# lvxianwei/DeepMerge

Measured on AMD Instinct MI355X. Metric: superpixel-pairs/sec (train step), higher is better.
Workload: dtype bf16; 1 GPU; ShfitScaleFormer_v3 depth [3, 2, 1], scales [32, 64, 128, 256] x 4ch (256x256x4 patches), 32 pairs/GPU/step, fwd+loss+bwd+allreduce+Adam (BASELINE configs[1]); pairs_per_gpu=32, global_batch=32, parallelism=dp1

## Files before the change

deepmerge_amd/_lib.py:

```python
from __future__ import annotations

import ctypes as C
import os
import re
import threading

HERE = os.path.dirname(os.path.abspath(__file__))
ROOT = os.path.dirname(HERE)
LIB_PATH = os.path.join(HERE, "libdeepmerge_hip.so")
HEADER_PATH = os.path.join(ROOT, "include", "deepmerge_hip.h")

DM_F32, DM_BF16 = 0, 1
DM_NT, DM_NN, DM_TN = 0, 1, 2
DM_BF16_PAIR = 2
DM_F64 = 3
DM_EPI_NONE, DM_EPI_GELU, DM_EPI_DGELU, DM_EPI_GELU_GRAD, DM_EPI_MUL = 0, 1, 2, 3, 4

_STATUS = {-1: "bad shape", -2: "bad dtype", -3: "bad alignment", -4: "workspace", -5: "HIP error", -6: "unsupported"}


class DeepMergeLibraryError(RuntimeError):
    pass


class DmGemmArgs(C.Structure):
    _fields_ = [
        ("layout", C.c_int32), ("ab_dtype", C.c_int32), ("c_dtype", C.c_int32), ("aux_dtype", C.c_int32),
        ("M", C.c_int32), ("N", C.c_int32), ("K", C.c_int32),
        ("epilogue", C.c_int32), ("accumulate", C.c_int32), ("split_k", C.c_int32),
        ("A", C.c_void_p), ("lda", C.c_int64),
        ("B", C.c_void_p), ("ldb", C.c_int64),
        ("C", C.c_void_p), ("ldc", C.c_int64),
        ("bias", C.c_void_p),
        ("residual", C.c_void_p), ("ldr", C.c_int64),
        ("aux", C.c_void_p), ("ldaux", C.c_int64),
        ("rows_per_group", C.c_int32), ("group_stride", C.c_int64),
        ("workspace", C.c_void_p), ("workspace_bytes", C.c_int64),
        ("colsum_a", C.c_void_p), ("colsum_accumulate", C.c_int32),
        ("k_fold", C.c_int32), ("a_fold", C.c_int64 * 3), ("b_fold", C.c_int64 * 3),
        ("c_plane", C.c_int64),
    ]


class DmReduceItem(C.Structure):
    _fields_ = [("partial", C.c_void_p), ("out0", C.c_void_p), ("out1", C.c_void_p),
                ("nrows", C.c_int32), ("width", C.c_int32), ("split", C.c_int32), ("accumulate", C.c_int32)]


class DmPairDraw(C.Structure):
    _fields_ = [("pairs", C.c_void_p), ("pair_flag", C.c_void_p), ("poly_off", C.c_void_p), ("poly_pts", C.c_void_p),
                ("pt_tile", C.c_void_p), ("pt_xy", C.c_void_p), ("pt_inner", C.c_void_p), ("pt_obj", C.c_void_p),
                ("pt_region", C.c_void_p),
                ("tile_id", C.c_void_p), ("xy", C.c_void_p), ("inner", C.c_void_p), ("obj", C.c_void_p),
                ("region", C.c_void_p), ("flag", C.c_void_p),
                ("point_id", C.c_void_p),
                ("seed", C.c_uint64),
                ("n_pairs", C.c_int32), ("n_poly", C.c_int32), ("n_poly_pts", C.c_int32), ("n_pts", C.c_int32),
                ("epoch", C.c_int32), ("batch", C.c_int32)]


class DmMergeFold(C.Structure):
    _fields_ = [("ptr", C.c_void_p), ("idx", C.c_void_p), ("edges", C.c_void_p), ("root", C.c_void_p), ("pick", C.c_void_p),
                ("rep", C.c_void_p), ("region_of", C.c_void_p),
                ("simi", C.c_void_p), ("weights", C.c_void_p),
                ("count", C.c_void_p), ("sum", C.c_void_p), ("sumsq", C.c_void_p), ("bbox", C.c_void_p), ("peri", C.c_void_p),
                ("new_id", C.c_void_p), ("hist_rank", C.c_void_p), ("new_ptr", C.c_void_p), ("new_idx", C.c_void_p),
                ("new_rep", C.c_void_p), ("new_region_of", C.c_void_p), ("n_regions", C.c_void_p),
                ("new_count", C.c_void_p), ("new_sum", C.c_void_p), ("new_sumsq", C.c_void_p), ("new_bbox", C.c_void_p),
                ("new_peri", C.c_void_p),
                ("history", C.c_void_p), ("history_simi", C.c_void_p),
                ("C", C.c_int32), ("P", C.c_int32), ("E", C.c_int32), ("S0", C.c_int32), ("bands", C.c_int32), ("round", C.c_int32),
                ("hist_base", C.c_int32), ("hist_cap", C.c_int32)]


class DmVectorTrace(C.Structure):
    _fields_ = [("dart", C.c_void_p), ("next", C.c_void_p), ("lab", C.c_void_p), ("other", C.c_void_p), ("flags", C.c_void_p),
                ("key", C.c_void_p), ("sum", C.c_void_p), ("ring_of_slot", C.c_void_p), ("ring_ptr", C.c_void_p),
                ("arc_base", C.c_void_p), ("xy", C.c_void_p), ("area2", C.c_void_p),
                ("arc_first", C.c_void_p), ("arc_left", C.c_void_p), ("arc_right", C.c_void_p), ("arc_vstart", C.c_void_p),
                ("arc_count", C.c_void_p), ("arc_pos", C.c_void_p), ("arc_ptr", C.c_void_p), ("arc_xy", C.c_void_p),
                ("W", C.c_int32), ("D", C.c_int32), ("R", C.c_int32), ("n_arcs", C.c_int32)]


class DmSceneVectorTrace(C.Structure):
    _fields_ = [("dart", C.c_void_p), ("next", C.c_void_p), ("lab", C.c_void_p), ("other", C.c_void_p), ("flags", C.c_void_p),
                ("key", C.c_void_p), ("sum", C.c_void_p), ("ring_of_slot", C.c_void_p), ("ring_ptr", C.c_void_p),
                ("arc_base", C.c_void_p), ("xy", C.c_void_p), ("area2", C.c_void_p),
                ("arc_first", C.c_void_p), ("arc_left", C.c_void_p), ("arc_right", C.c_void_p), ("arc_vstart", C.c_void_p),
                ("arc_count", C.c_void_p), ("arc_pos", C.c_void_p), ("arc_ptr", C.c_void_p), ("arc_xy", C.c_void_p),
                ("W", C.c_int64), ("D", C.c_int32), ("R", C.c_int32), ("n_arcs", C.c_int32)]


class DmProfRow(C.Structure):
    _fields_ = [("name", C.c_char * 64), ("launches", C.c_int64), ("total_ms", C.c_double),
                ("total_flops", C.c_double), ("total_bytes", C.c_double)]


_P, _I, _L, _F, _D = C.c_void_p, C.c_int32, C.c_int64, C.c_float, C.c_double

SIGNATURES = {
    "dm_abi_version": (_I, []),
    "dm_last_error": (C.c_char_p, []),
    "dm_arch": (C.c_char_p, []),
    "dm_gemm": (_I, [C.POINTER(DmGemmArgs), _P]),
    "dm_gemm_workspace_bytes": (_L, [_I, _I, _I, _I]),
    "dm_gemm_grouped": (_I, [C.POINTER(DmGemmArgs), _I, _P]),
    "dm_attention_fwd": (_I, [_P, _P, _P, _P, _I, _I, _I, _I, _F, _I, _P]),
    "dm_attention_relpos_inkernel": (_I, [_I, _I, _I, _I, _I, _I, _I, _I]),
    "dm_attention_fwd_relpos": (_I, [_P, _P, _I, _I, _I, _P, _P, _I, _I, _I, _I, _F, _I, _P]),
    "dm_attention_split_ok": (_I, [_I, _I, _I, _I, _I, _I, _I, _I]),
    "dm_attention_split_fwd": (_I, [_P, _P, _P, _P, _I, _I, _I, _P, _P, _I, _I, _I, _I, _F, _P]),
    "dm_attention_split_fwd_pair": (_I, [_P, _P, _P, _P, _I, _I, _I, _P, _P, _P, _I, _I, _I, _I, _F, _P]),
    "dm_attention_split_bwd_chunks": (_I, [_I, _I, _I]),
    "dm_attention_split_bwd": (_I, [_P, _P, _P, _I, _I, _I, _P, _P, _P, _P, _P, _P, _P, _P, _I, _I, _I, _I, _F, _P]),
    "dm_attention_split_bwd_pair": (_I, [_P, _P, _P, _I, _I, _I, _P, _P, _P, _P, _P, _P, _P, _P, _I, _I, _I, _I, _F, _P]),
    "dm_attention_bwd_relpos": (_I, [_P, _P, _I, _I, _I, _P, _P, _P, _P, _P, _P, _P, _P, _I, _I, _I, _I, _F, _I, _P]),
    "dm_attention_bwd": (_I, [_P, _P, _P, _P, _P, _P, _P, _P, _P, _I, _I, _I, _I, _F, _I, _P]),
    "dm_attention_bwd_batch_chunks": (_I, [_I, _I, _I, _I]),
    "dm_relpos_bias_gather": (_I, [_P, _P, _P, _P, _I, _I, _I, _P]),
    "dm_relpos_bias_reduce": (_I, [_P, _P, _P, _P, _I, _I, _I, _I, _I, _P]),
    "dm_layernorm_fwd": (_I, [_P, _P, _P, _P, _I, _P, _P, _I, _I, _F, _P]),
    "dm_layernorm_bwd": (_I, [_P, _I, _P, _P, _P, _P, _P, _P, _P, _P, _P, _I, _P, _I, _I, _P]),
    "dm_layernorm_bwd_partials": (_I, [_P, _I, _P, _P, _P, _P, _P, _P, _P, _P, _I, _I, C.POINTER(C.c_int32), _P]),
    "dm_layernorm_bwd_partials_pair": (_I, [_P, _I, _P, _P, _P, _P, _P, _P, _P, _P, _I, _I, C.POINTER(C.c_int32), _P]),
    "dm_partial_reduce_batch": (_I, [C.POINTER(DmReduceItem), _I, _P]),
    "dm_layernorm_bwd_partial_floats": (_L, [_I]),
    "dm_token_pool_fwd": (_I, [_P, _P, _I, _I, _I, _I, _P]),
    "dm_token_pool_bwd": (_I, [_P, _P, _I, _I, _I, _I, _P]),
    "dm_group_mean_fwd": (_I, [_P, _P, _I, _I, _I, _P]),
    "dm_group_mean_bwd": (_I, [_P, _P, _I, _I, _I, _P]),
    "dm_colsum": (_I, [_P, _I, _L, _P, _I, _I, _I, _P, _P]),
    "dm_colsum_partial_floats": (_L, [_I]),
    "dm_cast": (_I, [_P, _P, _I, _L, _P]),
    "dm_split_bf16": (_I, [_P, _L, _L, _L, _P, _I, _I, _P]),
    "dm_split_colsum_partial_floats": (_L, [_L, _L]),
    "dm_split_bf16_colsum": (_I, [_P, _L, _L, _L, _P, _I, _I, _P, _P, _P]),
    "dm_split_bf16_planes": (_I, [_P, _L, _L, _L, _P, _P, _P, _P]),
    "dm_patchify": (_I, [_P, _P, _I, _I, _I, _I, _I, _P]),
    "dm_contrastive_loss": (_I, [_P, _P, _P, _F, _F, _P, _P, _P, _I, _I, _P]),
    "dm_cross_entropy": (_I, [_P, _P, _P, _F, _P, _P, _I, _I, _P]),
    "dm_batchnorm_workspace_bytes": (_L, [_I, _I]),
    "dm_batchnorm_fwd": (_I, [_P, _P, _P, _P, _P, _P, _I, _P, _P, _P, _I, _I, _F, _F, _I, _I, _P, _P]),
    "dm_batchnorm_bwd": (_I, [_P, _P, _P, _P, _P, _I, _P, _P, _P, _P, _P, _I, _I, _I, _I, _I, _P, _P]),
    "dm_adam_step": (_I, [_P, _P, _P, _P, _P, _L, _I, _D, _D, _D, _D, _D, _P]),
    "dm_adam_hyper": (_I, [_I, _D, _D, _D, _P]),
    "dm_adam_step_dev": (_I, [_P, _P, _P, _P, _P, _L, _P, _D, _D, _D, _D, _P]),
    "dm_adam_step_dev_pair": (_I, [_P, _P, _P, _P, _P, _P, _L, _P, _D, _D, _D, _D, _P]),
    "dm_segment_mean": (_I, [_P, _P, _P, _P, _I, _I, _P]),
    "dm_edge_similarity": (_I, [_P, _P, _P, _P, _I, _I, _F, _P]),
    "dm_pairwise_distance": (_I, [_P, _P, _P, _I, _I, _I, _I, _P]),
    "dm_patch_pyramid": (_I, [_P, _I, _I, _I, _P, _P, _I, _I, _I, _I, _P, _P]),
    "dm_patch_pyramid_cols": (_I, [_P, _I, _I, _I, _P, _P, _I, _I, _I, _I, _I, _P, _I, _P]),
    "dm_pair_batch_gather": (_I, [_P, _I, _I, _I, _I, _P, _P, _P, _P, _I, _I, _I, _I, _I, _I, _P, _I, _P, _P, _P, _P]),
    "dm_pair_epoch_draw": (_I, [C.POINTER(DmPairDraw), _P]),
    "dm_contrastive_terms": (_I, [_P, _P, _P, _F, _P, _P, _I, _I, _P]),
    "dm_pair_eval_workspace_bytes": (_L, [_L, _I]),
    "dm_pair_eval_summary": (_I, [_P, _P, _P, _L, _P, _I, _P, _P, _P, _P, _P]),
    "dm_label_stats": (_I, [_P, _P, _I, _I, _I, _I, _P, _P, _P, _P, _P, _P]),
    "dm_label_features": (_I, [_P, _P, _P, _P, _P, _I, _I, _P, _P]),
    "dm_rag_edges": (_I, [_P, _I, _I, _I, _P, _P, _I, _P, _P, _I, _P, _P, _P]),
    "dm_seam_stitch": (_I, [_P, _P, _L, _L, _P, _P, _P, _I, _P, _P, _I, _P, _P, _P]),
    "dm_merge_round": (_I, [_P, _P, _I, _I, _P, _P, _I, _P]),
    "dm_merge_best": (_I, [_P, _P, _I, _I, _F, _P, _P]),
    "dm_merge_match": (_I, [_P, _P, _I, _I, _P, _P, _P, _P, _P]),
    "dm_merge_fold_regions": (_I, [C.POINTER(DmMergeFold), _P]),
    "dm_merge_edge_keys": (_I, [_P, _P, _P, _I, _I, _P, _P]),
    "dm_merge_fold_edges": (_I, [_P, _P, _P, _I, _P, _P, _P, _P]),
    "dm_relabel_raster": (_I, [_P, _P, _P, _L, _I, _P]),
    "dm_region_merge_cost": (_I, [_P, _P, _P, _P, _P, _P, _P, _I, _I, _I, _D, _D, _D, _D, _D, _P, _P]),
    "dm_pixel_regions": (_I, [_P, _I, _I, _I, _P, _P, _P, _P, _P, _P, _P, _P]),
    "dm_label_clearance": (_I, [_P, _I, _I, _I, _P, _P, _P, _P]),
    "dm_point_select_round": (_I, [_P, _P, _I, _I, _I, _I, _I, _P, _P, _P, _P, _P, _P]),
    "dm_point_emit": (_I, [_P, _P, _P, _P, _I, _I, _I, _I, _P, _P, _P, _P, _P, _P, _P]),
    "dm_label_overlap": (_I, [_P, _P, _I, _I, _L, _L, _P, _P, _I, _P, _P, _I, _P, _P, _P]),
    "dm_overlap_reduce": (_I, [_P, _P, _I, _L, _L, _P, _P, _P, _P, _P, _P, _P, _P, _P]),
    "dm_pair_flags": (_I, [_P, _I, _P, _P, _P, _I, _I, _P, _P]),
    "dm_slic_iterate": (_I, [_P, _I, _I, _I, _I, _I, _I, _P, _P, _P, _P]),
    "dm_connected_labels": (_I, [_P, _I, _I, _I, _I, _P, _P, _P, _P, _P]),
    "dm_label_area": (_I, [_P, _I, _I, _I, _P, _P]),
    "dm_slic_absorb_pick": (_I, [_P, _P, _I, _P, _I, _I, _P, _P, _P, _P]),
    "dm_vector_count": (_I, [_P, _I, _I, _P, _P, _P, _P]),
    "dm_vector_emit": (_I, [_P, _P, _I, _I, _P, _P, _P]),
    "dm_vector_link": (_I, [_P, _P, _P, _P, _I, _I, _I, _P, _P, _P, _P, _P, _P]),
    "dm_vector_head_round": (_I, [_P, _P, _P, _P, _I, _P, _P]),
    "dm_vector_rank_init": (_I, [_P, _P, _P, _P, _I, _P, _P, _P, _P, _P, _I, _P]),
    "dm_vector_rank_round": (_I, [_P, _P, _P, _P, _I, _P, _P]),
    "dm_vector_ring_emit": (_I, [C.POINTER(DmVectorTrace), _P]),
    "dm_vector_arc_emit": (_I, [C.POINTER(DmVectorTrace), _P]),
    "dm_scene_vector_count": (_I, [_P, _I, _I, _I, _I, _I, _I, _P, _P, _P, _P, _P]),
    "dm_scene_vector_link": (_I, [_P, _P, _P, _I, _I, _I, _L, _L, _L, _L, _P, _P, _P, _P, _P, _P]),
    "dm_scene_vector_ring_emit": (_I, [C.POINTER(DmSceneVectorTrace), _P]),
    "dm_scene_vector_arc_emit": (_I, [C.POINTER(DmSceneVectorTrace), _P]),
    "dm_rasterize_count": (_I, [_P, _P, _P, _I, _I, _I, _I, _P, _P]),
    "dm_rasterize_emit": (_I, [_P, _P, _P, _P, _P, _I, _I, _L, _I, _I, _L, _P, _P]),
    "dm_rasterize_fill": (_I, [_P, _L, _I, _I, _I, _P, _P, _P]),
    "dm_simplify_nodes": (_I, [_P, _I, _I, _P, _P]),
    "dm_simplify_chains": (_I, [_P, _P, _I, _L, _I, _I, _I, _P, _P, _P]),
    "dm_simplify_arc_count": (_I, [_P, _P, _I, _L, _I, _I, _P, _P, _P]),
    "dm_simplify_arc_emit": (_I, [_P, _P, _P, _I, _L, _L, _I, _I, _P, _P, _P]),
    "dm_simplify_ring_count": (_I, [_P, _P, _P, _I, _I, _I, _I, _P, _P, _P]),
    "dm_simplify_ring_emit": (_I, [_P, _P, _P, _P, _P, _I, _I, _L, _I, _I, _P, _P, _P, _P]),
    "dm_gru_cell_fwd": (_I, [_P, _L, _P, _P, _P, _P, _I, _I, _P]),
    "dm_gru_cell_bwd": (_I, [_P, _P, _P, _P, _P, _P, _I, _I, _P]),
    "dm_prof_enable": (_I, [_I]),
    "dm_prof_collect": (_I, [C.POINTER(DmProfRow), _I]),
}

_lock = threading.Lock()
_lib = None


def declared_symbols(header_path: str = HEADER_PATH):
    text = open(header_path).read()
    text = re.sub(r"/\*.*?\*/", "", text, flags=re.S)
    return sorted(set(re.findall(r"\b(dm_[a-z0-9_]+)\s*\(", text)))


def lib() -> C.CDLL:
    global _lib
    if _lib is not None:
        return _lib
    with _lock:
        if _lib is not None:
            return _lib
        if not os.path.exists(LIB_PATH):
            raise DeepMergeLibraryError(
                f"{LIB_PATH} not found: build the HIP kernels first "
                f"(`python -c 'import __graft_entry__ as g; g.build()'` or `make -C deepmerge_amd/csrc`). "
                f"deepmerge_amd has no CPU fallback.")
        try:
            handle = C.CDLL(LIB_PATH)
        except OSError as e:
            raise DeepMergeLibraryError(f"cannot load {LIB_PATH}: {e}") from e
        for name, (res, args) in SIGNATURES.items():
            try:
                fn = getattr(handle, name)
            except AttributeError as e:
                raise DeepMergeLibraryError(f"{LIB_PATH} does not export {name}") from e
            fn.restype = res
            fn.argtypes = args
        if handle.dm_abi_version() != 7:
            raise DeepMergeLibraryError(f"ABI version mismatch: library {handle.dm_abi_version()} != 7")
        _lib = handle
        return _lib


def check(rc: int, what: str):
    if rc == 0:
        return
    msg = lib().dm_last_error().decode("utf-8", "replace")
    text = f"{what} failed ({_STATUS.get(rc, rc)}): {msg}"
    if rc in (-1, -2, -3, -6):
        raise ValueError(text)
    raise RuntimeError(text)
```

deepmerge_amd/csrc/dm_attention.hip:

```cpp
#include "dm_common.h"
#include "dm_mfma.h"
#include "dm_attention_pipe.h"
#include "dm_attention_x3.h"
#include "dm_prof.h"

namespace {

constexpr int HD = 64;
constexpr int QB = 64;

template <typename T> struct AL {
  static constexpr int RB = HD * (int)sizeof(T);
  static constexpr int CPRW = RB / 16;
  static constexpr int KBD = RB / 64;
  static constexpr int EPC = 16 / (int)sizeof(T);
  static constexpr int TPB = (sizeof(T) == 2) ? 2 : 1;
};

template <typename T> __device__ __forceinline__ int swz(int row);
template <> __device__ __forceinline__ int swz<bf16_t>(int row) {
  const int t0 = (row >> 1) & 1, t1 = (row >> 2) & 1, t2 = (row >> 3) & 1;
  return ((t1 ^ t2) << 2) | (t0 << 1) | t1;
}
template <> __device__ __forceinline__ int swz<float>(int row) { return row & 15; }

template <typename T> __device__ __forceinline__ int img_off(int row, int chunk) {
  return row * AL<T>::RB + ((chunk ^ swz<T>(row)) << 4);
}

template <typename T>
__device__ __forceinline__ void tile_to_lds(char *lds, const T *g, long long ld, int nvalid, int nrows, int t) {
  using L = AL<T>;
  const int c = t % L::CPRW;
  constexpr int RPI = 256 / L::CPRW;
  for (int row = t / L::CPRW; row < nrows; row += RPI) {
    u32x4 v = {0u, 0u, 0u, 0u};
    if (row < nvalid) v = *reinterpret_cast<const u32x4 *>(g + (long long)row * ld + c * L::EPC);
    *reinterpret_cast<u32x4 *>(lds + img_off<T>(row, c)) = v;
  }
}

template <typename T> __device__ __forceinline__ u32x4 frag_row(const char *lds, int row, int kb, int lane) {
  return *reinterpret_cast<const u32x4 *>(lds + img_off<T>(row, kb * 4 + (lane >> 4)));
}
template <typename T> __device__ __forceinline__ u32x4 frag_tr(const char *lds, int d0, int m, int lane);
template <> __device__ __forceinline__ u32x4 frag_tr<bf16_t>(const char *lds, int d0, int m, int lane) {
  const int g = lane >> 4, q = (lane >> 2) & 3, p = lane & 3;
  const int d = d0 + 4 * p;
  u32x4 out;
#pragma unroll
  for (int half = 0; half < 2; ++half) {
    const int k = 32 * m + 4 * g + 16 * half + q;
    const u32x2 w = dm_ds_read_tr16(lds + img_off<bf16_t>(k, d >> 3) + ((d & 7) << 1));
    out[2 * half] = w[0];
    out[2 * half + 1] = w[1];
  }
  return out;
}
template <> __device__ __forceinline__ u32x4 frag_tr<float>(const char *lds, int d0, int m, int lane) {
  const int g = lane >> 4, d = d0 + (lane & 15);
  u32x4 out;
#pragma unroll
  for (int j = 0; j < 4; ++j) {
    const int k = 16 * m + 4 * g + j;
    out[j] = *reinterpret_cast<const unsigned int *>(lds + img_off<float>(k, d >> 2) + ((d & 3) << 2));
  }
  return out;
}
template <typename T> __device__ __forceinline__ u32x4 gl_frag(const T *rowp, bool valid, int kb, int lane) {
  u32x4 v = {0u, 0u, 0u, 0u};
  if (valid) v = *reinterpret_cast<const u32x4 *>(rowp + (kb * 4 + (lane >> 4)) * AL<T>::EPC);
  return v;
}

template <typename T, int NKT> __device__ __forceinline__ u32x4 acc_frag(const f32x4 (&s)[NKT], int m) {
  if constexpr (sizeof(T) == 2) {
    const f32x4 lo = s[2 * m], hi = s[2 * m + 1];
    bf16x8 r = {(bf16_t)lo[0], (bf16_t)lo[1], (bf16_t)lo[2], (bf16_t)lo[3], (bf16_t)hi[0], (bf16_t)hi[1], (bf16_t)hi[2], (bf16_t)hi[3]};
    return __builtin_bit_cast(u32x4, r);
  } else {
    return __builtin_bit_cast(u32x4, s[m]);
  }
}

template <typename T, int NKT>
__device__ __forceinline__ void contract_tokens(f32x4 (&o)[4], const f32x4 (&s)[NKT], const char *img, int lane) {
#pragma unroll
  for (int m = 0; m < NKT / AL<T>::TPB; ++m) {
    const u32x4 fp = acc_frag<T, NKT>(s, m);
#pragma unroll
    for (int dt = 0; dt < 4; ++dt) mma<T>(o[dt], fp, frag_tr<T>(img, dt * 16, m, lane));
    if ((m & 1) == 1) __builtin_amdgcn_sched_barrier(0);
  }
}

__device__ __forceinline__ float row_max(float v) {
  v = fmaxf(v, __shfl_xor(v, 16, 64));
  return fmaxf(v, __shfl_xor(v, 32, 64));
}
__device__ __forceinline__ float row_sum(float v) {
  v += __shfl_xor(v, 16, 64);
  return v + __shfl_xor(v, 32, 64);
}

template <typename T> __device__ __forceinline__ float fast_exp(float x);
template <> __device__ __forceinline__ float fast_exp<float>(float x) { return expf(x); }
template <> __device__ __forceinline__ float fast_exp<bf16_t>(float x) { return __expf(x); }

__device__ __forceinline__ f32x4 load4_guard(const float *p, int i, int n, bool vec) {
  if (vec) return (i < n) ? dm_load4(p + i) : (f32x4){0.f, 0.f, 0.f, 0.f};
  f32x4 r;
#pragma unroll
  for (int e = 0; e < 4; ++e) r[e] = (i + e < n) ? p[i + e] : 0.f;
  return r;
}

struct AttnParams {
  const void *qkv;
  const float *bias;
  const float *bias_t;
  const void *out;
  const void *dout;
  float *lse;
  float *delta;
  void *dqkv;
  float *slab;
  int B, N, H, bchunk;
  float scale;
};

template <bool FAST, bool STRIDED>
__device__ __forceinline__ f32x4 bias_tile(const float *bias_rows, int N, int row, int lane, int kt) {
  const int col = kt * 16 + 4 * (lane >> 4);
  f32x4 bv = {0.f, 0.f, 0.f, 0.f};
  if (bias_rows && row < N) {
    if constexpr (!STRIDED) {
      bv = load4_guard(bias_rows + (long long)row * N, col, N, FAST);
    } else {
#pragma unroll
      for (int r = 0; r < 4; ++r) bv[r] = (col + r < N) ? bias_rows[(long long)(col + r) * N + row] : 0.f;
    }
  }
  return bv;
}
template <typename T>
__device__ __forceinline__ f32x4 score_tile(const u32x4 (&fa)[AL<T>::KBD], const char *img, const f32x4 bv,
                                            int N, int row, float scale, int lane, int kt) {
  using L = AL<T>;
  const int g = lane >> 4, li = lane & 15;
  f32x4 a = {0.f, 0.f, 0.f, 0.f};
#pragma unroll
  for (int kb = 0; kb < L::KBD; ++kb) mma<T>(a, fa[kb], frag_row<T>(img, kt * 16 + li, kb, lane));
  const int col = kt * 16 + 4 * g;
#pragma unroll
  for (int r = 0; r < 4; ++r) a[r] = (row < N && col + r < N) ? a[r] * scale + bv[r] : -INFINITY;
  return a;
}

template <typename T> __device__ __forceinline__ u32x4 pack_tiles(const f32x4 (&tl)[AL<T>::TPB]) {
  if constexpr (sizeof(T) == 2) {
    bf16x8 r = {(bf16_t)tl[0][0], (bf16_t)tl[0][1], (bf16_t)tl[0][2], (bf16_t)tl[0][3],
                (bf16_t)tl[1][0], (bf16_t)tl[1][1], (bf16_t)tl[1][2], (bf16_t)tl[1][3]};
    return __builtin_bit_cast(u32x4, r);
  } else {
    return __builtin_bit_cast(u32x4, tl[0]);
  }
}

template <typename T, int NB>
__device__ __forceinline__ void contract_frags(f32x4 (&o)[4], const u32x4 (&f)[NB], const char *img, int lane) {
#pragma unroll
  for (int m = 0; m < NB; ++m) {
#pragma unroll
    for (int dt = 0; dt < 4; ++dt) mma<T>(o[dt], f[m], frag_tr<T>(img, dt * 16, m, lane));
    if ((m & 1) == 1) __builtin_amdgcn_sched_barrier(0);
  }
}

template <typename T, int NKT, bool FAST>
__global__ __launch_bounds__(256, 2) void attn_fwd_kernel(const AttnParams p) {
  using L = AL<T>;
  constexpr int NK = NKT * 16;
  constexpr int IMG = NK * L::RB;
  __shared__ __attribute__((aligned(16))) char smem[2 * IMG];
  char *kimg = smem, *vimg = smem + IMG;
  const int t = threadIdx.x, lane = t & 63, wave = t >> 6, g = lane >> 4, li = lane & 15;
  const int qblk = blockIdx.x, h = blockIdx.y, b = blockIdx.z;
  const int N = p.N, H = p.H;

  const long long tok_stride = 3LL * H * HD;
  const T *base = reinterpret_cast<const T *>(p.qkv) + (long long)b * N * tok_stride + (long long)h * HD;
  const int q = qblk * QB + wave * 16 + li;

  tile_to_lds<T>(kimg, base + (long long)H * HD, tok_stride, N, NK, t);
  tile_to_lds<T>(vimg, base + 2LL * H * HD, tok_stride, N, NK, t);
  u32x4 fq[L::KBD];
#pragma unroll
  for (int kb = 0; kb < L::KBD; ++kb) fq[kb] = gl_frag<T>(base + (long long)q * tok_stride, q < N, kb, lane);
  __syncthreads();

  f32x4 s[NKT];
  const float *brows = p.bias ? p.bias + (long long)h * N * N : nullptr;
#pragma unroll
  for (int kt = 0; kt < NKT; ++kt) s[kt] = score_tile<T>(fq, kimg, bias_tile<FAST, false>(brows, N, q, lane, kt), N, q, p.scale, lane, kt);

  float m = -INFINITY;
#pragma unroll
  for (int kt = 0; kt < NKT; ++kt)
#pragma unroll
    for (int r = 0; r < 4; ++r) m = fmaxf(m, s[kt][r]);
  m = row_max(m);
  const float msafe = (m == -INFINITY) ? 0.f : m;
  float l = 0.f;
#pragma unroll
  for (int kt = 0; kt < NKT; ++kt)
#pragma unroll
    for (int r = 0; r < 4; ++r) {
      const float e = fast_exp<T>(s[kt][r] - msafe);
      s[kt][r] = e;
      l += e;
    }
  l = row_sum(l);
  const float inv = (l > 0.f) ? 1.f / l : 0.f;
  if (g == 0 && q < N) p.lse[((long long)b * H + h) * N + q] = msafe + logf(l);
#pragma unroll
  for (int kt = 0; kt < NKT; ++kt) s[kt] *= inv;

  f32x4 o[4];
#pragma unroll
  for (int dt = 0; dt < 4; ++dt) o[dt] = (f32x4){0.f, 0.f, 0.f, 0.f};
  contract_tokens<T, NKT>(o, s, vimg, lane);
  if (q < N) {
    T *orow = reinterpret_cast<T *>(const_cast<void *>(p.out)) + ((long long)b * N + q) * H * HD + (long long)h * HD;
#pragma unroll
    for (int dt = 0; dt < 4; ++dt) dm_store4(orow + dt * 16 + 4 * g, o[dt]);
  }
}

template <typename T, int NKT, bool FAST>
__global__ __launch_bounds__(256, 2) void attn_bwd_dq_kernel(const AttnParams p) {
  using L = AL<T>;
  constexpr int NK = NKT * 16;
  constexpr int IMG = NK * L::RB;
  constexpr int NB = NKT / L::TPB;
  __shared__ __attribute__((aligned(16))) char smem[2 * IMG];
  char *kimg = smem, *vimg = smem + IMG;
  const int t = threadIdx.x, lane = t & 63, wave = t >> 6, g = lane >> 4, li = lane & 15;
  const int qblk = blockIdx.x, h = blockIdx.y, chunk = blockIdx.z;
  const int N = p.N, H = p.H;
  const long long tok_stride = 3LL * H * HD;
  const int q = qblk * QB + wave * 16 + li;
  const bool qok = q < N;
  const float *brows = p.bias ? p.bias + (long long)h * N * N : nullptr;
  const bool want_bins = p.slab != nullptr;
  f32x4 hacc[NKT];
#pragma unroll
  for (int kt = 0; kt < NKT; ++kt) hacc[kt] = (f32x4){0.f, 0.f, 0.f, 0.f};

  const int b_end = min(p.B, (chunk + 1) * p.bchunk);
  for (int b = chunk * p.bchunk; b < b_end; ++b) {
    const T *base = reinterpret_cast<const T *>(p.qkv) + (long long)b * N * tok_stride + (long long)h * HD;
    const long long orow = ((long long)b * N + q) * H * HD + (long long)h * HD;
    const T *Og = reinterpret_cast<const T *>(p.out) + orow;
    const T *dOg = reinterpret_cast<const T *>(p.dout) + orow;
    __syncthreads();
    tile_to_lds<T>(kimg, base + (long long)H * HD, tok_stride, N, NK, t);
    tile_to_lds<T>(vimg, base + 2LL * H * HD, tok_stride, N, NK, t);
    u32x4 fq[L::KBD], fdo[L::KBD];
#pragma unroll
    for (int kb = 0; kb < L::KBD; ++kb) {
      fq[kb] = gl_frag<T>(base + (long long)q * tok_stride, qok, kb, lane);
      fdo[kb] = gl_frag<T>(dOg, qok, kb, lane);
    }
    float dl = 0.f;
    if (qok) {
#pragma unroll
      for (int c = 0; c < 4; ++c) {
        const f32x4 a = dm_load4(Og + 16 * g + 4 * c), d = dm_load4(dOg + 16 * g + 4 * c);
        dl += (a[0] * d[0] + a[1] * d[1]) + (a[2] * d[2] + a[3] * d[3]);
      }
    }
    dl = row_sum(dl);
    const long long rowid = ((long long)b * H + h) * N + q;
    if (g == 0 && qok) p.delta[rowid] = dl;
    const float lse = qok ? p.lse[rowid] : 0.f;
    __syncthreads();

    u32x4 fds[NB];
    f32x4 bnext[L::TPB];
#pragma unroll
    for (int u = 0; u < L::TPB; ++u) bnext[u] = bias_tile<FAST, false>(brows, N, q, lane, u);
#pragma unroll
    for (int m = 0; m < NB; ++m) {
      f32x4 bcur[L::TPB];
#pragma unroll
      for (int u = 0; u < L::TPB; ++u) bcur[u] = bnext[u];
      if (m + 1 < NB) {
#pragma unroll
        for (int u = 0; u < L::TPB; ++u) bnext[u] = bias_tile<FAST, false>(brows, N, q, lane, (m + 1) * L::TPB + u);
      }
      f32x4 tl[L::TPB];
#pragma unroll
      for (int u = 0; u < L::TPB; ++u) {
        const int kt = m * L::TPB + u;
        const f32x4 sc = score_tile<T>(fq, kimg, bcur[u], N, q, p.scale, lane, kt);
        f32x4 a = {0.f, 0.f, 0.f, 0.f};
#pragma unroll
        for (int kb = 0; kb < L::KBD; ++kb) mma<T>(a, fdo[kb], frag_row<T>(vimg, kt * 16 + li, kb, lane));
        f32x4 dsv;
#pragma unroll
        for (int r = 0; r < 4; ++r) dsv[r] = fast_exp<T>(sc[r] - lse) * (a[r] - dl);
        if (want_bins) hacc[kt] += dsv;
        tl[u] = dsv;
      }
      fds[m] = pack_tiles<T>(tl);
      asm volatile("" : "+v"(fds[m]));
      __builtin_amdgcn_sched_barrier(0);
    }

    f32x4 o[4];
#pragma unroll
    for (int dt = 0; dt < 4; ++dt) o[dt] = (f32x4){0.f, 0.f, 0.f, 0.f};
    contract_frags<T, NB>(o, fds, kimg, lane);
    if (qok) {
      T *dq = reinterpret_cast<T *>(p.dqkv) + ((long long)b * N + q) * tok_stride + (long long)h * HD;
#pragma unroll
      for (int dt = 0; dt < 4; ++dt) dm_store4(dq + dt * 16 + 4 * g, o[dt] * p.scale);
    }
  }

  if (want_bins && qok) {
    float *srow = p.slab + (((long long)chunk * H + h) * N + q) * N;
#pragma unroll
    for (int kt = 0; kt < NKT; ++kt) {
      const int key = kt * 16 + 4 * g;
      if constexpr (FAST) {
        if (key < N) dm_store4(srow + key, hacc[kt]);
      } else {
#pragma unroll
        for (int r = 0; r < 4; ++r)
          if (key + r < N) srow[key + r] = hacc[kt][r];
      }
    }
  }
}

template <typename T, int NKT, bool FAST>
__global__ __launch_bounds__(256, 2) void attn_bwd_dkv_kernel(const AttnParams p) {
  using L = AL<T>;
  constexpr int NK = NKT * 16;
  constexpr int IMG = NK * L::RB;
  __shared__ __attribute__((aligned(16))) char smem[2 * IMG];
  char *qimg = smem, *doimg = smem + IMG;
  const int t = threadIdx.x, lane = t & 63, wave = t >> 6, g = lane >> 4, li = lane & 15;
  const int kblk = blockIdx.x, h = blockIdx.y, b = blockIdx.z;
  const int N = p.N, H = p.H;

  const long long tok_stride = 3LL * H * HD;
  const T *base = reinterpret_cast<const T *>(p.qkv) + (long long)b * N * tok_stride + (long long)h * HD;
  const long long o_stride = (long long)H * HD;
  const T *dOg = reinterpret_cast<const T *>(p.dout) + (long long)b * N * o_stride + (long long)h * HD;
  const int key = kblk * QB + wave * 16 + li;
  const bool kok = key < N;
  const T *krow = base + (long long)key * tok_stride + (long long)H * HD;
  const T *vrow = krow + (long long)H * HD;
  const float *lse = p.lse + ((long long)b * H + h) * N;
  const float *delta = p.delta + ((long long)b * H + h) * N;

  tile_to_lds<T>(qimg, base, tok_stride, N, NK, t);
  tile_to_lds<T>(doimg, dOg, o_stride, N, NK, t);
  u32x4 fk[L::KBD], fvv[L::KBD];
#pragma unroll
  for (int kb = 0; kb < L::KBD; ++kb) {
    fk[kb] = gl_frag<T>(krow, kok, kb, lane);
    fvv[kb] = gl_frag<T>(vrow, kok, kb, lane);
  }
  __syncthreads();

  constexpr int NB = NKT / L::TPB;
  u32x4 fpt[NB], fds[NB];
  const float *bsrc = FAST ? p.bias_t : p.bias;
  const float *brows = bsrc ? bsrc + (long long)h * N * N : nullptr;
  f32x4 bnext[L::TPB], lnext[L::TPB], dnext[L::TPB];
  auto fetch = [&](int m) {
#pragma unroll
    for (int u = 0; u < L::TPB; ++u) {
      const int qt = m * L::TPB + u;
      bnext[u] = bias_tile<FAST, !FAST>(brows, N, key, lane, qt);
      lnext[u] = load4_guard(lse, qt * 16 + 4 * g, N, FAST);
      dnext[u] = load4_guard(delta, qt * 16 + 4 * g, N, FAST);
    }
  };
  fetch(0);
#pragma unroll
  for (int m = 0; m < NB; ++m) {
    f32x4 bcur[L::TPB], lcur[L::TPB], dcur[L::TPB];
#pragma unroll
    for (int u = 0; u < L::TPB; ++u) { bcur[u] = bnext[u]; lcur[u] = lnext[u]; dcur[u] = dnext[u]; }
    if (m + 1 < NB) fetch(m + 1);
    f32x4 tp[L::TPB], td[L::TPB];
#pragma unroll
    for (int u = 0; u < L::TPB; ++u) {
      const int qt = m * L::TPB + u;
      const int q0 = qt * 16 + 4 * g;
      const f32x4 sc = score_tile<T>(fk, qimg, bcur[u], N, key, p.scale, lane, qt);
      f32x4 a = {0.f, 0.f, 0.f, 0.f};
#pragma unroll
      for (int kb = 0; kb < L::KBD; ++kb) mma<T>(a, fvv[kb], frag_row<T>(doimg, qt * 16 + li, kb, lane));
#pragma unroll
      for (int r = 0; r < 4; ++r) {
        const float pv = (q0 + r < N) ? fast_exp<T>(sc[r] - lcur[u][r]) : 0.f;
        tp[u][r] = pv;
        td[u][r] = pv * (a[r] - dcur[u][r]);
      }
    }
    fpt[m] = pack_tiles<T>(tp);
    fds[m] = pack_tiles<T>(td);
    asm volatile("" : "+v"(fpt[m]), "+v"(fds[m]));
    __builtin_amdgcn_sched_barrier(0);
  }
  f32x4 o[4];
  T *dk = reinterpret_cast<T *>(p.dqkv) + ((long long)b * N + key) * tok_stride + (long long)H * HD + (long long)h * HD;
  T *dvp = dk + (long long)H * HD;
#pragma unroll
  for (int dt = 0; dt < 4; ++dt) o[dt] = (f32x4){0.f, 0.f, 0.f, 0.f};
  contract_frags<T, NB>(o, fpt, doimg, lane);
  if (kok) {
#pragma unroll
    for (int dt = 0; dt < 4; ++dt) dm_store4(dvp + dt * 16 + 4 * g, o[dt]);
  }
#pragma unroll
  for (int dt = 0; dt < 4; ++dt) o[dt] = (f32x4){0.f, 0.f, 0.f, 0.f};
  contract_frags<T, NB>(o, fds, qimg, lane);
  if (kok) {
#pragma unroll
    for (int dt = 0; dt < 4; ++dt) dm_store4(dk + dt * 16 + 4 * g, o[dt] * p.scale);
  }
}

template <typename T, int NKT, bool FAST> void launch3(int which, const AttnParams &p, dim3 grid, hipStream_t s) {
  if (which == 0) hipLaunchKernelGGL((attn_fwd_kernel<T, NKT, FAST>), grid, dim3(256), 0, s, p);
  else if (which == 1) hipLaunchKernelGGL((attn_bwd_dq_kernel<T, NKT, FAST>), grid, dim3(256), 0, s, p);
  else hipLaunchKernelGGL((attn_bwd_dkv_kernel<T, NKT, FAST>), grid, dim3(256), 0, s, p);
}
template <typename T, bool FAST> void dispatch_nkt(int which, const AttnParams &p, hipStream_t s) {
  const dim3 grid((p.N + QB - 1) / QB, p.H, which == 1 ? (p.B + p.bchunk - 1) / p.bchunk : p.B);
  const int nkt = (p.N + 15) / 16;
  if (nkt <= 2) launch3<T, 2, FAST>(which, p, grid, s);
  else if (nkt <= 4) launch3<T, 4, FAST>(which, p, grid, s);
  else if (nkt <= 8) launch3<T, 8, FAST>(which, p, grid, s);
  else if (nkt <= 12) launch3<T, 12, FAST>(which, p, grid, s);
  else if (nkt <= 14) launch3<T, 14, FAST>(which, p, grid, s);
  else launch3<T, 16, FAST>(which, p, grid, s);
}
template <typename T> int dispatch(int which, const AttnParams &p, hipStream_t s) {
  const bool fast = (p.N % 4 == 0) && (which != 2 || p.bias == nullptr || p.bias_t != nullptr);
  if (fast) dispatch_nkt<T, true>(which, p, s);
  else dispatch_nkt<T, false>(which, p, s);
  return 0;
}

int check_common(const char *who, int B, int N, int H, int D, int dtype) {
  DM_REQUIRE(B > 0 && H > 0 && N > 0 && N <= 256, DM_ERR_BAD_SHAPE, "%s: need 0 < N <= 4096 tokens and head dim <= 256 (got N=%d, D=%d, B=%d, H=%d)", who, N, D, B, H);
  DM_REQUIRE(D == HD, DM_ERR_BAD_SHAPE, "%s: head dim must be in 1..256 (got %d)", who, D);
  DM_REQUIRE(dtype == DM_F32 || dtype == DM_BF16, DM_ERR_BAD_DTYPE, "%s: bad dtype %d", who, dtype);
  DM_REQUIRE(H <= 65535 && B <= 65535, DM_ERR_BAD_SHAPE, "%s: grid too large", who);
  return DM_OK;
}

}

static int batch_chunk(int B, int N, int H) {
  const int per_sample = ((N + QB - 1) / QB) * H;
  for (int c = 8; c > 1; c >>= 1)
    if ((long long)per_sample * ((B + c - 1) / c) >= 300) return c;
  return 1;
}

const AttnSwitches &attn_switches() {
  static const AttnSwitches sw = [] {
    AttnSwitches v;
    if (const char *e = getenv("DM_ATTN_PIPE")) v.pipe = atoi(e);
    if (const char *e = getenv("DM_ATTN_Q32")) v.q32 = atoi(e);
    if (const char *e = getenv("DM_ATTN_Q32_BWD")) v.q32_bwd = atoi(e);
    if (const char *e = getenv("DM_ATTN_Q32_TABKV")) v.q32_tabkv = atoi(e) != 0;
    if (const char *e = getenv("DM_ATTN_Q32_W8")) v.q32_w8 = atoi(e) != 0;
    if (const char *e = getenv("DM_ATTN_Q32_TABW")) v.q32_tabw = atoi(e);
    if (const char *e = getenv("DM_ATTN_PF")) v.pf = atoi(e) != 0;
    if (const char *e = getenv("DM_ATTN_XCD")) v.xcd = atoi(e) != 0;
    if (const char *e = getenv("DM_ATTN_X3")) v.x3 = atoi(e) != 0;
    if (const char *e = getenv("DM_ATTN_X3_W8")) v.x3_w8 = atoi(e) != 0;
    return v;
  }();
  return sw;
}

namespace {

bool tokens32(const AttnCall &c) { return c.N > 128 && c.N <= 256; }
bool cube_fits(const AttnCall &c) { return c.N == 64 * c.cube_s && (c.cube_s == 3 || c.cube_s == 4); }
bool persistent_gate(const AttnCall &c, int mode) {
  return mode != 0 && (long long)c.N * 3 * c.H * 64 * 2 < (1LL << 31) && (mode == 2 || c.B * c.H >= 96);
}

AttnPass pass32(const AttnCall &c, AttnFamily f, AttnBias bias, int waves, int rows) {
  AttnPass g{f, (c.N + 31) / 32, c.N % 32 != 0, bias, waves, 0, 0, 0};
  attn_chunks(c.B, c.N, c.H, rows, g.nblk, g.chunks, g.bchunk);
  return g;
}
bool ragged16(const AttnCall &c) { return !(c.N == 128 || c.N == 192 || c.N == 256); }
AttnPass pass_pipe16(const AttnCall &c, AttnBias bias) {
  const int nkt = (c.N + 15) / 16;
  AttnPass g{ATTN_PIPE16, ragged16(c) ? (nkt + 1) / 2 * 2 : nkt, ragged16(c), bias, 8, 0, 0, 0};
  attn_chunks(c.B, c.N, c.H, 128, g.nblk, g.chunks, g.bchunk);
  return g;
}
AttnPass pass_reg16(const AttnCall &c, int bchunk) {
  return AttnPass{ATTN_REG16, (c.N + 15) / 16, c.N % 16 != 0, c.dense ? ATTN_BIAS_DENSE : ATTN_BIAS_NONE, 4, (c.N + QB - 1) / QB, (c.B + bchunk - 1) / bchunk, bchunk};
}
int waves32(const AttnCall &c, const AttnSwitches &sw) { return (c.N + 31) / 32 <= 7 && sw.q32_w8 ? 8 : 4; }

bool split_shape(const AttnCall &c, const AttnSwitches &sw) {
  return sw.x3 && c.D == HD && tokens32(c) && c.B > 0 && c.H > 0 && persistent_gate(c, 2) && (!c.table || cube_fits(c));
}

}

AttnFwdPlan attn_plan_fwd(const AttnCall &c, const AttnSwitches &sw) {
  AttnFwdPlan pl{};
  pl.pf = sw.pf;
  pl.xcd = sw.xcd;
  if (c.split) {
    if (!split_shape(c, sw)) pl.refused = ATTN_SHAPE_NOT_TAKEN;
    else pl.pass = pass32(c, ATTN_X3, c.table ? ATTN_BIAS_TABLE : ATTN_BIAS_NONE, sw.x3_w8 ? 8 : 4, 128);
    return pl;
  }
  pl.pass = pass_reg16(c, 1);
  if (c.D != HD || c.N > 256) {
    pl.pass.family = ATTN_GENERIC;
  } else if (c.dtype == DM_BF16) {
    if (tokens32(c) && persistent_gate(c, sw.q32) && !(c.table && (c.dense || !cube_fits(c)))) {
      if (c.table) pl.pass = pass32(c, ATTN_Q32, ATTN_BIAS_TABLE, sw.q32_tabw == 4 ? 4 : 8, sw.q32_tabw == 4 ? 128 : 256);
      else if (c.dense) pl.pass = pass32(c, ATTN_Q32, ATTN_BIAS_DENSE, 4, 128);
      else pl.pass = pass32(c, ATTN_Q32, ATTN_BIAS_NONE, waves32(c, sw), 32 * waves32(c, sw));
    } else if (c.N >= 128 && persistent_gate(c, sw.pipe)) {
      pl.pass = pass_pipe16(c, c.dense ? ATTN_BIAS_DENSE : ATTN_BIAS_NONE);
    }
  }
  if (c.table && !c.dense && !(pl.pass.family == ATTN_Q32 && pl.pass.bias == ATTN_BIAS_TABLE)) pl.refused = ATTN_SHAPE_NOT_TAKEN;
  return pl;
}

AttnBwdPlan attn_plan_bwd(const AttnCall &c, const AttnSwitches &sw) {
  AttnBwdPlan pl{};
  pl.xcd = sw.xcd;
  if (c.split) {
    if (c.B > 0 && c.H > 0) {
      const AttnBias bias = c.table ? ATTN_BIAS_TABLE : ATTN_BIAS_NONE;
      pl.dq = pass32(c, ATTN_X3, bias, sw.x3_w8 ? 8 : 4, 128);
      pl.dkv = pass32(c, ATTN_X3, bias, 4, 128);
      pl.slab_chunks = pl.dkv.chunks;
    }
    if (!split_shape(c, sw)) pl.refused = ATTN_SHAPE_NOT_TAKEN;
    return pl;
  }
  pl.dq = pass_reg16(c, batch_chunk(c.B, c.N, c.H));
  pl.dkv = pass_reg16(c, 1);
  pl.slab_chunks = pl.dq.chunks;
  if (c.D != HD || c.N > 256) {
    pl.dq.family = pl.dkv.family = ATTN_GENERIC;
    return pl;
  }
  const bool table_only = c.table && !c.dense;
  if (c.dtype != DM_BF16) {
    if (table_only) pl.refused = ATTN_TABLE_NEEDS_BF16;
    return pl;
  }
  if (c.N >= 128 && persistent_gate(c, sw.pipe) && !(ragged16(c) && (c.dense || c.slab))) {
    pl.dq = pass_pipe16(c, c.dense ? ATTN_BIAS_DENSE : ATTN_BIAS_NONE);
    pl.dkv = pass_pipe16(c, c.dense || c.slab ? ATTN_BIAS_DENSE : ATTN_BIAS_NONE);
    if (tokens32(c) && persistent_gate(c, sw.q32_bwd) && !(c.table && !cube_fits(c))) {
      if (c.table) pl.dq = pass32(c, ATTN_Q32, ATTN_BIAS_TABLE, 8, 256);
      else if (c.dense) pl.dq = pass32(c, ATTN_Q32, ATTN_BIAS_DENSE, 4, 128);
      else pl.dq = pass32(c, ATTN_Q32, ATTN_BIAS_NONE, waves32(c, sw), 32 * waves32(c, sw));
      const int w = (c.N + 31) / 32 <= 7 ? 8 : 4;
      if (sw.q32_bwd != 3 && c.table && sw.q32_tabkv) pl.dkv = pass32(c, ATTN_Q32_TABKV, ATTN_BIAS_TABLE, 4, 128);
      else if (sw.q32_bwd != 3 && !c.dense && !c.slab) pl.dkv = pass32(c, ATTN_Q32, ATTN_BIAS_NONE, w, 32 * w);
    }
    pl.slab_chunks = pl.dkv.chunks;
  }
  if (table_only && pl.dkv.family != ATTN_Q32_TABKV) pl.refused = ATTN_TABLE_NOT_TAKEN;
  return pl;
}

extern "C" int32_t dm_attention_bwd_batch_chunks(int32_t B, int32_t N, int32_t H, int32_t dtype) {
  return attn_plan_bwd(AttnCall{B, N, H, HD, dtype == DM_BF16 ? DM_BF16 : DM_F32, true, false, 0, true, false}, attn_switches()).slab_chunks;
}

bool dm_attn_generic_shape(int N, int D);
int dm_attn_generic_fwd(const void *qkv, const float *bias, void *out, float *lse, int B, int N, int H, int D, float scale, int dtype, hipStream_t s);
int dm_attn_generic_bwd(const void *qkv, const float *bias, const void *out, const void *dout, const float *lse, void *dqkv, float *delta,
                        int B, int N, int H, int D, float scale, int dtype, hipStream_t s);

extern "C" int dm_attention_fwd(const void *qkv, const float *bias, void *out, float *lse, int32_t B, int32_t N, int32_t H,
                                int32_t D, float scale, int32_t dtype, void *stream) {
  if (dm_attn_generic_shape(N, D)) {
    DM_REQUIRE(B > 0 && H > 0 && H <= 65535 && B <= 65535 && (dtype == DM_F32 || dtype == DM_BF16) && qkv && out && lse, DM_ERR_BAD_SHAPE,
               "dm_attention_fwd: bad arguments (B=%d H=%d dtype=%d)", B, H, dtype);
    const int rc = dm_attn_generic_fwd(qkv, bias, out, lse, B, N, H, D, scale, dtype, reinterpret_cast<hipStream_t>(stream));
    DM_REQUIRE(rc == DM_OK, rc, "dm_attention_fwd: generic kernel could not be configured");
    DM_LAUNCH_CHECK("dm_attention_fwd(generic)");
    return DM_OK;
  }
  if (int rc = check_common("dm_attention_fwd", B, N, H, D, dtype)) return rc;
  DM_REQUIRE(qkv && out && lse, DM_ERR_BAD_SHAPE, "dm_attention_fwd: null pointer");
  DM_REQUIRE(dm_aligned16(qkv) && dm_aligned16(out) && dm_aligned16(bias), DM_ERR_BAD_ALIGN, "dm_attention_fwd: qkv/out/bias must be 16-byte aligned");
  const AttnFwdPlan pl = attn_plan_fwd(AttnCall{B, N, H, D, dtype, bias != nullptr, false, 0, false, false}, attn_switches());
  hipStream_t s = reinterpret_cast<hipStream_t>(stream);
  {
    const double esz = (dtype == DM_BF16) ? 2.0 : 4.0;
    DmProfScope prof(dtype == DM_BF16 ? "attn_fwd_bf16" : "attn_fwd_f32", s, 4.0 * B * H * (double)N * N * HD,
                     esz * 4.0 * B * H * (double)N * HD);
    const AttnPipeParams pp{qkv, bias, out, lse, B, N, H, scale};
    if (pl.pass.family == ATTN_Q32) {
      DM_REQUIRE(dm_attn_fwd_q32(pl, pp, s), DM_ERR_HIP, "dm_attention_fwd: kernel could not be configured");
    } else if (pl.pass.family == ATTN_PIPE16) {
      dm_attn_fwd_pipe(pl, pp, s);
    } else {
      AttnParams p{};
      p.qkv = qkv; p.bias = bias; p.out = out; p.lse = lse; p.B = B; p.N = N; p.H = H; p.scale = scale; p.bchunk = 1;
      if (dtype == DM_BF16) dispatch<bf16_t>(0, p, s); else dispatch<float>(0, p, s);
    }
  }
  DM_LAUNCH_CHECK("dm_attention_fwd");
  return DM_OK;
}

static AttnCall table_call(int32_t B, int32_t N, int32_t H, int32_t D, int32_t cube_s, int32_t cube_h, int32_t cube_w, int32_t dtype, bool split) {
  return AttnCall{B, N, H, D, dtype, false, true, cube_h == 8 && cube_w == 8 ? cube_s : 0, false, split};
}

extern "C" int32_t dm_attention_relpos_inkernel(int32_t B, int32_t N, int32_t H, int32_t D, int32_t cube_s, int32_t cube_h, int32_t cube_w,
                                                int32_t dtype) {
  if (B <= 0 || H <= 0) return 0;
  const AttnCall c = table_call(B, N, H, D, cube_s, cube_h, cube_w, dtype, false);
  return !attn_plan_fwd(c, attn_switches()).refused && !attn_plan_bwd(c, attn_switches()).refused ? 1 : 0;
}

extern "C" int dm_attention_fwd_relpos(const void *qkv, const float *table, int32_t cube_s, int32_t cube_h, int32_t cube_w, void *out,
                                       float *lse, int32_t B, int32_t N, int32_t H, int32_t D, float scale, int32_t dtype, void *stream) {
  DM_REQUIRE(dm_attention_relpos_inkernel(B, N, H, D, cube_s, cube_h, cube_w, dtype), DM_ERR_UNSUPPORTED,
             "dm_attention_fwd_relpos: shape not taken (B=%d N=%d H=%d D=%d cube=%dx%dx%d dtype=%d); gather the bias and call dm_attention_fwd",
             B, N, H, D, cube_s, cube_h, cube_w, dtype);
  DM_REQUIRE(qkv && table && out && lse, DM_ERR_BAD_SHAPE, "dm_attention_fwd_relpos: null pointer");
  DM_REQUIRE(dm_aligned16(qkv) && dm_aligned16(out), DM_ERR_BAD_ALIGN, "dm_attention_fwd_relpos: qkv/out must be 16-byte aligned");
  const AttnFwdPlan pl = attn_plan_fwd(table_call(B, N, H, D, cube_s, cube_h, cube_w, dtype, false), attn_switches());
  hipStream_t s = reinterpret_cast<hipStream_t>(stream);
  {
    DmProfScope prof("attn_fwd_bf16", s, 4.0 * B * H * (double)N * N * HD, 2.0 * 4.0 * B * H * (double)N * HD);
    AttnPipeParams pp{qkv, nullptr, out, lse, B, N, H, scale};
    pp.table = table;
    pp.cube_s = cube_s;
    DM_REQUIRE(dm_attn_fwd_q32(pl, pp, s), DM_ERR_UNSUPPORTED, "dm_attention_fwd_relpos: kernel could not be configured");
  }
  DM_LAUNCH_CHECK("dm_attention_fwd_relpos");
  return DM_OK;
}

static int attention_bwd(const void *qkv, const float *bias, const float *bias_t, const float *table, int32_t cube_s, const void *out,
                         const void *dout, const float *lse, void *dqkv, float *delta, float *dbias_slab, int32_t B, int32_t N, int32_t H,
                         int32_t D, float scale, int32_t dtype, void *stream) {
  if (dm_attn_generic_shape(N, D)) {
    DM_REQUIRE(B > 0 && H > 0 && H <= 65535 && B <= 65535 && (dtype == DM_F32 || dtype == DM_BF16) && qkv && out && dout && lse && dqkv && delta,
               DM_ERR_BAD_SHAPE, "dm_attention_bwd: bad arguments (B=%d H=%d dtype=%d)", B, H, dtype);
    DM_REQUIRE(dbias_slab == nullptr, DM_ERR_UNSUPPORTED, "dm_attention_bwd: the bias-table gradient needs head dim 64 and N <= 256 (got D=%d N=%d)", D, N);
    const int rc = dm_attn_generic_bwd(qkv, bias, out, dout, lse, dqkv, delta, B, N, H, D, scale, dtype, reinterpret_cast<hipStream_t>(stream));
    DM_REQUIRE(rc == DM_OK, rc, "dm_attention_bwd: generic kernel could not be configured");
    DM_LAUNCH_CHECK("dm_attention_bwd(generic)");
    return DM_OK;
  }
  if (int rc = check_common("dm_attention_bwd", B, N, H, D, dtype)) return rc;
  DM_REQUIRE(qkv && out && dout && lse && dqkv && delta, DM_ERR_BAD_SHAPE, "dm_attention_bwd: null pointer");
  DM_REQUIRE(dm_aligned16(qkv) && dm_aligned16(out) && dm_aligned16(dout) && dm_aligned16(dqkv) && dm_aligned16(bias) &&
             dm_aligned16(bias_t) && dm_aligned16(lse) && dm_aligned16(delta) && dm_aligned16(dbias_slab), DM_ERR_BAD_ALIGN,
             "dm_attention_bwd: tensors must be 16-byte aligned");
  const AttnBwdPlan pl = attn_plan_bwd(AttnCall{B, N, H, D, dtype, bias != nullptr, table != nullptr, cube_s, dbias_slab != nullptr, false}, attn_switches());
  DM_REQUIRE(pl.refused != ATTN_TABLE_NEEDS_BF16, DM_ERR_UNSUPPORTED, "dm_attention_bwd_relpos: the table-reading kernels are bf16 only");
  DM_REQUIRE(!pl.refused, DM_ERR_UNSUPPORTED,
             "dm_attention_bwd_relpos: the table-reading backward kernels do not take this call (B=%d N=%d H=%d, switches "
             "DM_ATTN_PIPE / DM_ATTN_Q32_BWD / DM_ATTN_Q32_TABKV) and no dense bias rows were given", B, N, H);
  hipStream_t s = reinterpret_cast<hipStream_t>(stream);
  {
    const double esz = (dtype == DM_BF16) ? 2.0 : 4.0;
    DmProfScope prof(dtype == DM_BF16 ? "attn_bwd_bf16" : "attn_bwd_f32", s, 10.0 * B * H * (double)N * N * HD,
                     esz * 8.0 * B * H * (double)N * HD);
    if (pl.dkv.family == ATTN_REG16) {
      AttnParams p{};
      p.qkv = qkv; p.bias = bias; p.bias_t = bias ? bias_t : nullptr; p.out = out; p.dout = dout; p.lse = const_cast<float *>(lse);
      p.delta = delta; p.dqkv = dqkv; p.slab = dbias_slab;
      p.B = B; p.N = N; p.H = H; p.scale = scale; p.bchunk = pl.dq.bchunk;
      if (dtype == DM_BF16) { dispatch<bf16_t>(1, p, s); dispatch<bf16_t>(2, p, s); }
      else { dispatch<float>(1, p, s); dispatch<float>(2, p, s); }
    } else {
      AttnPipeBwdParams pp{qkv, bias, out, dout, lse, delta, dqkv, dbias_slab, B, N, H, scale};
      pp.table = table;
      pp.cube_s = cube_s;
      DM_REQUIRE(pl.dq.family != ATTN_Q32 || dm_attn_bwd_dq_q32(pl, pp, s), DM_ERR_HIP, "dm_attention_bwd: the dQ kernel could not be configured");
      if (pl.dkv.family == ATTN_PIPE16) dm_attn_bwd_pipe(pl, pp, s);
      else DM_REQUIRE(dm_attn_bwd_dkv_q32(pl, pp, s), DM_ERR_HIP, "dm_attention_bwd: the dK / dV kernel could not be configured");
    }
  }
  DM_LAUNCH_CHECK("dm_attention_bwd");
  return DM_OK;
}

extern "C" int dm_attention_bwd(const void *qkv, const float *bias, const float *bias_t, const void *out, const void *dout,
                                const float *lse, void *dqkv, float *delta, float *dbias_slab, int32_t B, int32_t N, int32_t H, int32_t D, float scale, int32_t dtype,
                                void *stream) {
  return attention_bwd(qkv, bias, bias_t, nullptr, 0, out, dout, lse, dqkv, delta, dbias_slab, B, N, H, D, scale, dtype, stream);
}

extern "C" int dm_attention_bwd_relpos(const void *qkv, const float *table, int32_t cube_s, int32_t cube_h, int32_t cube_w, const float *bias,
                                       const float *bias_t, const void *out, const void *dout, const float *lse, void *dqkv, float *delta,
                                       float *dbias_slab, int32_t B, int32_t N, int32_t H, int32_t D, float scale, int32_t dtype, void *stream) {
  DM_REQUIRE(table, DM_ERR_BAD_SHAPE, "dm_attention_bwd_relpos: null table");
  DM_REQUIRE(bias || dm_attention_relpos_inkernel(B, N, H, D, cube_s, cube_h, cube_w, dtype), DM_ERR_UNSUPPORTED,
             "dm_attention_bwd_relpos: shape not taken (B=%d N=%d H=%d D=%d cube=%dx%dx%d dtype=%d); call dm_attention_bwd", B, N, H, D, cube_s,
             cube_h, cube_w, dtype);
  return attention_bwd(qkv, bias, bias_t, table, cube_s, out, dout, lse, dqkv, delta, dbias_slab, B, N, H, D, scale, dtype, stream);
}

static AttnCall split_call(int32_t B, int32_t N, int32_t H, int32_t D, bool has_table, int32_t cube_s, int32_t cube_h, int32_t cube_w, bool slab) {
  AttnCall c = table_call(B, N, H, D, cube_s, cube_h, cube_w, DM_F32, true);
  c.table = has_table;
  c.slab = slab;
  return c;
}

extern "C" int32_t dm_attention_split_ok(int32_t B, int32_t N, int32_t H, int32_t D, int32_t has_table, int32_t cube_s, int32_t cube_h,
                                         int32_t cube_w) {
  return attn_plan_fwd(split_call(B, N, H, D, has_table != 0, cube_s, cube_h, cube_w, false), attn_switches()).refused ? 0 : 1;
}

static int split_fwd_impl(const float *qkv, void *qkv_hi, void *qkv_lo, const float *table, int32_t cube_s, int32_t cube_h, int32_t cube_w, float *out,
                          void *out_pair, float *lse, int32_t B, int32_t N, int32_t H, int32_t D, float scale, void *stream);
extern "C" int dm_attention_split_fwd(const float *qkv, void *qkv_hi, void *qkv_lo, const float *table, int32_t cube_s, int32_t cube_h,
                                      int32_t cube_w, float *out, float *lse, int32_t B, int32_t N, int32_t H, int32_t D, float scale,
                                      void *stream) {
  return split_fwd_impl(qkv, qkv_hi, qkv_lo, table, cube_s, cube_h, cube_w, out, nullptr, lse, B, N, H, D, scale, stream);
}
extern "C" int dm_attention_split_fwd_pair(const float *qkv, void *qkv_hi, void *qkv_lo, const float *table, int32_t cube_s, int32_t cube_h,
                                           int32_t cube_w, float *out, void *out_pair, float *lse, int32_t B, int32_t N, int32_t H, int32_t D,
                                           float scale, void *stream) {
  DM_REQUIRE(out_pair && dm_aligned16(out_pair), DM_ERR_BAD_SHAPE, "dm_attention_split_fwd_pair: out_pair must be a 16-byte aligned pointer");
  return split_fwd_impl(qkv, qkv_hi, qkv_lo, table, cube_s, cube_h, cube_w, out, out_pair, lse, B, N, H, D, scale, stream);
}
static int split_fwd_impl(const float *qkv, void *qkv_hi, void *qkv_lo, const float *table, int32_t cube_s, int32_t cube_h, int32_t cube_w, float *out,
                          void *out_pair, float *lse, int32_t B, int32_t N, int32_t H, int32_t D, float scale, void *stream) {
  const AttnFwdPlan pl = attn_plan_fwd(split_call(B, N, H, D, table != nullptr, cube_s, cube_h, cube_w, false), attn_switches());
  DM_REQUIRE(!pl.refused, DM_ERR_UNSUPPORTED,
             "dm_attention_split_fwd: shape not taken (B=%d N=%d H=%d D=%d cube=%dx%dx%d); use dm_attention_fwd", B, N, H, D, cube_s, cube_h, cube_w);
  DM_REQUIRE(qkv_hi && qkv_lo && out && lse, DM_ERR_BAD_SHAPE, "dm_attention_split_fwd: null pointer");
  DM_REQUIRE(dm_aligned16(qkv) && dm_aligned16(qkv_hi) && dm_aligned16(qkv_lo) && dm_aligned16(out), DM_ERR_BAD_ALIGN,
             "dm_attention_split_fwd: tensors must be 16-byte aligned");
  hipStream_t s = reinterpret_cast<hipStream_t>(stream);
  {
    DmProfScope prof("attn_fwd_x3", s, 3.0 * 4.0 * B * H * (double)N * N * HD, 4.0 * 4.0 * B * H * (double)N * HD);
    if (qkv) dm_attn_x3_split(qkv, qkv_hi, qkv_lo, (long long)B * N * 3 * H * HD, s);
    AttnX3Params p{reinterpret_cast<const bf16_t *>(qkv_hi), reinterpret_cast<const bf16_t *>(qkv_lo), table, cube_s, out, lse, B, N, H, scale,
                   reinterpret_cast<bf16_t *>(out_pair)};
    DM_REQUIRE(dm_attn_fwd_x3(pl, p, s), DM_ERR_UNSUPPORTED, "dm_attention_split_fwd: kernel could not be configured");
  }
  DM_LAUNCH_CHECK("dm_attention_split_fwd");
  return DM_OK;
}

extern "C" int32_t dm_attention_split_bwd_chunks(int32_t B, int32_t N, int32_t H) {
  return attn_plan_bwd(split_call(B, N, H, HD, false, 0, 0, 0, false), attn_switches()).slab_chunks;
}

static int split_bwd_impl(const void *qkv_hi, const void *qkv_lo, const float *table, int32_t cube_s, int32_t cube_h, int32_t cube_w,
                          const float *out, const float *dout, void *dout_hi, void *dout_lo, const float *lse, float *dqkv, void *dqkv_pair,
                          float *delta, float *dbias_slab, int32_t B, int32_t N, int32_t H, int32_t D, float scale, void *stream);
extern "C" int dm_attention_split_bwd(const void *qkv_hi, const void *qkv_lo, const float *table, int32_t cube_s, int32_t cube_h, int32_t cube_w,
                                      const float *out, const float *dout, void *dout_hi, void *dout_lo, const float *lse, float *dqkv,
                                      float *delta, float *dbias_slab, int32_t B, int32_t N, int32_t H, int32_t D, float scale, void *stream) {
  DM_REQUIRE(dqkv, DM_ERR_BAD_SHAPE, "dm_attention_split_bwd: null pointer");
  return split_bwd_impl(qkv_hi, qkv_lo, table, cube_s, cube_h, cube_w, out, dout, dout_hi, dout_lo, lse, dqkv, nullptr, delta, dbias_slab, B, N, H, D, scale, stream);
}
extern "C" int dm_attention_split_bwd_pair(const void *qkv_hi, const void *qkv_lo, const float *table, int32_t cube_s, int32_t cube_h, int32_t cube_w,
                                           const float *out, const float *dout, void *dout_hi, void *dout_lo, const float *lse, void *dqkv_pair,
                                           float *delta, float *dbias_slab, int32_t B, int32_t N, int32_t H, int32_t D, float scale, void *stream) {
  DM_REQUIRE(dqkv_pair, DM_ERR_BAD_SHAPE, "dm_attention_split_bwd_pair: null pointer");
  return split_bwd_impl(qkv_hi, qkv_lo, table, cube_s, cube_h, cube_w, out, dout, dout_hi, dout_lo, lse, nullptr, dqkv_pair, delta, dbias_slab, B, N, H, D, scale, stream);
// ... 25 lines not shown
```

deepmerge_amd/csrc/dm_attention_plan.h:

```cpp
#pragma once

struct AttnSwitches {
  int pipe = 1;
  int q32 = 1;
  int q32_bwd = 1;
  bool q32_tabkv = true;
  bool q32_w8 = true;
  int q32_tabw = 8;
  bool pf = true;
  bool xcd = true;
  bool x3 = true;
  bool x3_w8 = true;
};
const AttnSwitches &attn_switches();

struct AttnCall {
  int B, N, H, D, dtype;
  bool dense;
  bool table;
  int cube_s;
  bool slab;
  bool split;
};

enum AttnFamily {
  ATTN_GENERIC,
  ATTN_REG16,
  ATTN_PIPE16,
  ATTN_Q32,
  ATTN_Q32_TABKV,
  ATTN_X3,
};
enum AttnBias { ATTN_BIAS_NONE, ATTN_BIAS_DENSE, ATTN_BIAS_TABLE };
enum AttnRefusal { ATTN_TAKEN = 0, ATTN_SHAPE_NOT_TAKEN, ATTN_TABLE_NEEDS_BF16, ATTN_TABLE_NOT_TAKEN };

struct AttnPass {
  AttnFamily family;
  int nkt;
  bool ragged;
  AttnBias bias;
  int waves;
  int nblk, chunks, bchunk;
};
struct AttnFwdPlan {
  AttnRefusal refused;
  AttnPass pass;
  bool pf, xcd;
};
struct AttnBwdPlan {
  AttnRefusal refused;
  AttnPass dq, dkv;
  bool xcd;
  int slab_chunks;
};
AttnFwdPlan attn_plan_fwd(const AttnCall &c, const AttnSwitches &sw);
AttnBwdPlan attn_plan_bwd(const AttnCall &c, const AttnSwitches &sw);

inline void attn_chunks(int B, int N, int H, int rows, int &nblk, int &chunks, int &bchunk) {
  nblk = (N + rows - 1) / rows;
  chunks = 256 / (H * nblk);
  if (chunks < 1) chunks = 1;
  if (chunks > B) chunks = B;
  bchunk = (B + chunks - 1) / chunks;
  chunks = (B + bchunk - 1) / bchunk;
}
```

deepmerge_amd/ops.py:

```python
from __future__ import annotations

import os

import ctypes as C
from typing import Optional

import torch

from . import _lib
from ._lib import DM_BF16, DM_EPI_DGELU, DM_EPI_GELU, DM_EPI_GELU_GRAD, DM_EPI_MUL, DM_EPI_NONE, DM_F32, DM_NN, DM_NT, DM_TN, DmGemmArgs, check

_NUMERICS = "bf16"


NUMERICS_MODES = ("bf16", "fp32", "bf16x3")
_FP32_PRODUCTS = "mfma_f32"
_SPLIT_MIN_WORK = 1 << 24
_PAIR_LN_MAX_COLS = 1024


def set_numerics(mode: str) -> None:
    global _NUMERICS
    _NUMERICS = check_numerics(mode)

# ... 284 lines not shown
            b_rows, b_cols = (N, K) if layout == DM_NT else (K, N)
            if (A.rows, A.cols) != (a_rows, a_cols) or (B.rows, B.cols) != (b_rows, b_cols):
                raise ValueError(f"plane pair shapes {(A.rows, A.cols)} / {(B.rows, B.cols)} do not match the product {(a_rows, a_cols)} / {(b_rows, b_cols)}")
            fold = (K, A.t.stride(0), B.t.stride(0))
            A, B, lda, ldb, K = A.t, B.t, a_cols, b_cols, 3 * K
        _need_cuda(A, B, C_out, kw.get("colsum_out"))
        if A.dtype != B.dtype:
            raise ValueError(f"A/B dtype mismatch: {A.dtype} vs {B.dtype}")
        lda = lda if lda is not None else (A.stride(-2) if A.dim() >= 2 else K)
        ldb = ldb if ldb is not None else (B.stride(-2) if B.dim() >= 2 else K)
        arr[i] = _gemm_args(layout, A, B, C_out, M, N, K, lda, ldb, kw.get("ldc"), kw.get("bias"), kw.get("residual"), kw.get("ldr"),
                            kw.get("epilogue", DM_EPI_NONE), kw.get("aux"), kw.get("ldaux"), kw.get("accumulate", False), kw.get("split_k", 0),
                            kw.get("rows_per_group", 0), kw.get("group_stride", 0), kw.get("colsum_out"), kw.get("colsum_accumulate", False),
                            f"{kw.get('ws_slot', 'gemm')}.g{i}", None, fold, min_slabs=16 if layout == DM_TN else 0)
    check(_lib.lib().dm_gemm_grouped(arr, len(calls), _stream()), "dm_gemm_grouped")


def cast(src: torch.Tensor, dtype: torch.dtype) -> torch.Tensor:
    if src.dtype == dtype:
        return src
    _need_cuda(src)
    if src.dtype != torch.float32:
        raise ValueError("dm_cast source must be fp32")
    src = src.contiguous()
    dst = torch.empty(src.shape, dtype=dtype, device=src.device)
    check(_lib.lib().dm_cast(src.data_ptr(), dst.data_ptr(), _dt(dst), src.numel(), _stream()), "dm_cast")
    return dst


def colsum(X: torch.Tensor, out: torch.Tensor, accumulate: bool = False, ws_slot: str = "partial") -> torch.Tensor:
    _need_cuda(X, out)
    M, N = X.shape
    part = workspace(_lib.lib().dm_colsum_partial_floats(N) * 4, X.device, ws_slot)
    check(_lib.lib().dm_colsum(X.data_ptr(), _dt(X), X.stride(0), out.data_ptr(), M, N, int(accumulate), part.data_ptr(), _stream()), "dm_colsum")
    return out


def layernorm_fwd(x: torch.Tensor, gamma, beta, eps: float, out_dtype: torch.dtype, pair: bool = False):
    _need_cuda(x, gamma, beta)
    rows, cols = x.numel() // x.shape[-1], x.shape[-1]
    mean = torch.empty(rows, dtype=torch.float32, device=x.device)
    rstd = torch.empty(rows, dtype=torch.float32, device=x.device)
    if pair:
        yp = torch.empty((2, rows, cols), dtype=torch.bfloat16, device=x.device)
        check(_lib.lib().dm_layernorm_fwd(x.data_ptr(), gamma.data_ptr(), beta.data_ptr(), yp.data_ptr(), _lib.DM_BF16_PAIR, mean.data_ptr(),
                                          rstd.data_ptr(), rows, cols, eps, _stream()), "dm_layernorm_fwd")
        return Planes(yp), mean, rstd
    y = torch.empty(x.shape, dtype=out_dtype, device=x.device)
    check(_lib.lib().dm_layernorm_fwd(x.data_ptr(), gamma.data_ptr(), beta.data_ptr(), y.data_ptr(), _dt(y), mean.data_ptr(),
                                      rstd.data_ptr(), rows, cols, eps, _stream()), "dm_layernorm_fwd")
    return y, mean, rstd


_pending_reduce = []
_pending_out = set()
_flush_queued = False
_flush_task = -1


def _in_backward() -> bool:
    return torch._C._current_graph_task_id() != -1


def flush_reductions() -> None:
    global _flush_queued
    _flush_queued = False
    if not _pending_reduce:
        return
    items = (_lib.DmReduceItem * len(_pending_reduce))()
    for i, (f, _keep) in enumerate(_pending_reduce):
        items[i].partial, items[i].out0, items[i].out1, items[i].nrows, items[i].width, items[i].split, items[i].accumulate = f
    n = len(_pending_reduce)
    keep = list(_pending_reduce)
    _pending_reduce.clear()
    _pending_out.clear()
    check(_lib.lib().dm_partial_reduce_batch(items, n, _stream()), "dm_partial_reduce_batch")
    del keep


def _queue_reduce(part, out0, out1, nrows, width, split, accumulate) -> None:
    global _flush_queued, _flush_task
    task = torch._C._current_graph_task_id()
    if task != _flush_task:
        _pending_reduce.clear()
        _pending_out.clear()
        _flush_queued = False
        _flush_task = task
    keys = (out0.data_ptr(), out1.data_ptr())
    if keys[0] in _pending_out or keys[1] in _pending_out:
        flush_reductions()
    _pending_reduce.append(((part.data_ptr(), keys[0], keys[1], int(nrows), int(width), int(split), int(bool(accumulate))), (part, out0, out1)))
    _pending_out.update(keys)
    if not _flush_queued:
        torch.autograd.Variable._execution_engine.queue_callback(flush_reductions)
        _flush_queued = True


def layernorm_bwd(dy, x, gamma, mean, rstd, dres=None, dgamma=None, dbeta=None, accumulate=False, want_lp=False, defer=False, want_pair=False):
    _need_cuda(dy, x)
    if not (dy.is_contiguous() and x.is_contiguous()) or dy.numel() != x.numel():
        raise ValueError("layernorm_bwd: dy and x must be contiguous and of the same size (an expanded gradient has no rows to read)")
    rows, cols = x.numel() // x.shape[-1], x.shape[-1]
    dx = torch.empty(x.shape, dtype=torch.float32, device=x.device)
    dx_lp = torch.empty(x.shape, dtype=torch.bfloat16, device=x.device) if want_lp else None
    if dgamma is None:
        dgamma = torch.empty(cols, dtype=torch.float32, device=x.device)
        dbeta = torch.empty(cols, dtype=torch.float32, device=x.device)
        accumulate = False
        defer = False
    if want_pair:
        pair = torch.empty((2, rows, cols), dtype=torch.bfloat16, device=x.device)
        deferred = defer and _DEFER_REDUCTIONS and _in_backward()
        part = (torch.empty(_lib.lib().dm_layernorm_bwd_partial_floats(cols), dtype=torch.float32, device=x.device) if deferred
                else workspace(_lib.lib().dm_layernorm_bwd_partial_floats(cols) * 4, x.device, "partial").view(torch.float32))
        n_part = C.c_int32(0)
        check(_lib.lib().dm_layernorm_bwd_partials_pair(dy.data_ptr(), _dt(dy), x.data_ptr(), gamma.data_ptr(), mean.data_ptr(), rstd.data_ptr(),
                                                        _ptr(dres), dx.data_ptr(), pair.data_ptr(), part.data_ptr(), rows, cols, C.byref(n_part),
                                                        _stream()), "dm_layernorm_bwd_partials_pair")
        if deferred:
            _queue_reduce(part, dgamma, dbeta, n_part.value, 2 * cols, cols, accumulate)
        else:
            item = (_lib.DmReduceItem * 1)()
            item[0].partial, item[0].out0, item[0].out1 = part.data_ptr(), dgamma.data_ptr(), dbeta.data_ptr()
            item[0].nrows, item[0].width, item[0].split, item[0].accumulate = n_part.value, 2 * cols, cols, int(bool(accumulate))
            check(_lib.lib().dm_partial_reduce_batch(item, 1, _stream()), "dm_partial_reduce_batch")
        return dx, Planes(pair), dgamma, dbeta
    if defer and _DEFER_REDUCTIONS and _in_backward():
        part = torch.empty(_lib.lib().dm_layernorm_bwd_partial_floats(cols), dtype=torch.float32, device=x.device)
        n_part = C.c_int32(0)
        check(_lib.lib().dm_layernorm_bwd_partials(dy.data_ptr(), _dt(dy), x.data_ptr(), gamma.data_ptr(), mean.data_ptr(), rstd.data_ptr(),
                                                   _ptr(dres), dx.data_ptr(), _ptr(dx_lp), part.data_ptr(), rows, cols, C.byref(n_part),
                                                   _stream()), "dm_layernorm_bwd_partials")
        _queue_reduce(part, dgamma, dbeta, n_part.value, 2 * cols, cols, accumulate)
        return (dx, dx_lp, dgamma, dbeta) if want_lp else (dx, dgamma, dbeta)
    part = workspace(_lib.lib().dm_layernorm_bwd_partial_floats(cols) * 4, x.device, "partial")
    check(_lib.lib().dm_layernorm_bwd(dy.data_ptr(), _dt(dy), x.data_ptr(), gamma.data_ptr(), mean.data_ptr(), rstd.data_ptr(),
                                      _ptr(dres), dx.data_ptr(), _ptr(dx_lp), dgamma.data_ptr(), dbeta.data_ptr(), int(accumulate),
                                      part.data_ptr(), rows, cols, _stream()), "dm_layernorm_bwd")
    return (dx, dx_lp, dgamma, dbeta) if want_lp else (dx, dgamma, dbeta)


_DEFER_REDUCTIONS = os.environ.get("DM_DEFER_REDUCTIONS", "1") != "0"


def relpos_bias_gather(table: torch.Tensor, index32: torch.Tensor, N: int, transposed: bool = False):
    _need_cuda(table, index32)
    n_bins, H = table.shape
    bias = torch.empty((H, N, N), dtype=torch.float32, device=table.device)
    bias_t = torch.empty_like(bias) if transposed else None
    check(_lib.lib().dm_relpos_bias_gather(table.data_ptr(), index32.data_ptr(), bias.data_ptr(), _ptr(bias_t), N, H, n_bins, _stream()),
          "dm_relpos_bias_gather")
    return (bias, bias_t) if transposed else bias


def attention_fwd(qkv: torch.Tensor, bias: Optional[torch.Tensor], B: int, N: int, H: int, D: int, scale: float):
    _need_cuda(qkv, bias)
    out = torch.empty((B, N, H * D), dtype=qkv.dtype, device=qkv.device)
    lse = torch.empty((B, H, N), dtype=torch.float32, device=qkv.device)
    check(_lib.lib().dm_attention_fwd(qkv.data_ptr(), _ptr(bias), out.data_ptr(), lse.data_ptr(), B, N, H, D, scale, _dt(qkv), _stream()),
          "dm_attention_fwd")
    return out, lse


def _split_attention(table, index32, qkv, B, N, H, D):
    if (qkv if isinstance(qkv, torch.dtype) else qkv.dtype) != torch.float32 or _FP32_PRODUCTS != "bf16x3" or not _SPLIT_ATTENTION:
        return False, None
    cube = None if table is None else getattr(index32, "_dm_cube", None)
    if table is not None and cube is None:
        return False, None
    return attention_split_ok(B, N, H, D, cube), cube


_SPLIT_ATTENTION = os.environ.get("DM_ATTN_X3", "1") != "0"


def _inkernel_cube(table, index32, B, N, H, D, dtype):
    cube = None if table is None else getattr(index32, "_dm_cube", None)
    if cube is None or _INKERNEL_TABLE is False or not relpos_inkernel(B, N, H, D, cube, dtype):
        return None
    return cube


_INKERNEL_TABLE = os.environ.get("DM_ATTN_TABLE_IN_KERNEL", "1") != "0"


def relpos_inkernel(B: int, N: int, H: int, D: int, cube, dtype: torch.dtype) -> bool:
    if cube is None or len(cube) != 3:
        return False
    return bool(_lib.lib().dm_attention_relpos_inkernel(B, N, H, D, int(cube[0]), int(cube[1]), int(cube[2]),
                                                        DM_BF16 if dtype == torch.bfloat16 else DM_F32))


def attention_fwd_relpos(qkv: torch.Tensor, table: torch.Tensor, cube, B: int, N: int, H: int, D: int, scale: float):
    _need_cuda(qkv, table)
    if table.dtype != torch.float32 or not table.is_contiguous() or tuple(table.shape) != ((2 * cube[0] - 1) * (2 * cube[1] - 1) * (2 * cube[2] - 1), H):
        raise ValueError(f"attention_fwd_relpos: table must be contiguous fp32 [(2s-1)(2h-1)(2w-1), H], got {tuple(table.shape)} {table.dtype}")
    out = torch.empty((B, N, H * D), dtype=qkv.dtype, device=qkv.device)
    lse = torch.empty((B, H, N), dtype=torch.float32, device=qkv.device)
    check(_lib.lib().dm_attention_fwd_relpos(qkv.data_ptr(), table.data_ptr(), int(cube[0]), int(cube[1]), int(cube[2]), out.data_ptr(),
                                             lse.data_ptr(), B, N, H, D, scale, _dt(qkv), _stream()), "dm_attention_fwd_relpos")
    return out, lse


def attention_split_ok(B: int, N: int, H: int, D: int, cube=None) -> bool:
    c = (0, 0, 0) if cube is None else tuple(int(v) for v in cube)
    return bool(_lib.lib().dm_attention_split_ok(B, N, H, D, int(cube is not None), c[0], c[1], c[2]))


def attention_fwd_split(qkv: torch.Tensor, table: Optional[torch.Tensor], cube, B: int, N: int, H: int, D: int, scale: float, out_pair: bool = False):
    if table is not None and (table.dtype != torch.float32 or not table.is_contiguous()):
        raise ValueError("attention_fwd_split: table must be contiguous fp32")
    if isinstance(qkv, Planes):
        _need_cuda(qkv.t, table)
        hi, lo, src, dev = qkv.t[0], qkv.t[1], None, qkv.t.device
    else:
        _need_cuda(qkv, table)
        if qkv.dtype != torch.float32 or not qkv.is_contiguous():
            raise ValueError("attention_fwd_split: qkv must be a contiguous fp32 tensor")
        hi = torch.empty(qkv.shape, dtype=torch.bfloat16, device=qkv.device)
        lo = torch.empty(qkv.shape, dtype=torch.bfloat16, device=qkv.device)
        src, dev = qkv.data_ptr(), qkv.device
    out = torch.empty((B, N, H * D), dtype=torch.float32, device=dev)
    lse = torch.empty((B, H, N), dtype=torch.float32, device=dev)
    c = (0, 0, 0) if cube is None else tuple(int(v) for v in cube)
    if out_pair:
        op = torch.empty((2, B * N, H * D), dtype=torch.bfloat16, device=dev)
        check(_lib.lib().dm_attention_split_fwd_pair(src, hi.data_ptr(), lo.data_ptr(), _ptr(table), c[0], c[1], c[2], out.data_ptr(), op.data_ptr(),
                                                     lse.data_ptr(), B, N, H, D, scale, _stream()), "dm_attention_split_fwd_pair")
        return out, lse, hi, lo, Planes(op)
    check(_lib.lib().dm_attention_split_fwd(src, hi.data_ptr(), lo.data_ptr(), _ptr(table), c[0], c[1], c[2], out.data_ptr(),
                                            lse.data_ptr(), B, N, H, D, scale, _stream()), "dm_attention_split_fwd")
    return out, lse, hi, lo


def attention_bwd_split(hi, lo, table, cube, out, dout, lse, B, N, H, D, scale, index32=None, n_bins=0, pair=False):
    _need_cuda(hi, lo, table, out, dout, lse, index32)
    if out.dtype != torch.float32 or dout.dtype != torch.float32 or not (out.is_contiguous() and dout.is_contiguous()):
        raise ValueError("attention_bwd_split: out / dout must be contiguous fp32")
    dqkv = (torch.empty((2, B * N, 3 * H * D), dtype=torch.bfloat16, device=hi.device) if pair
            else torch.empty(hi.shape, dtype=torch.float32, device=hi.device))
    delta = torch.empty((B, H, N), dtype=torch.float32, device=hi.device)
    dhi = torch.empty(dout.shape, dtype=torch.bfloat16, device=hi.device)
    dlo = torch.empty(dout.shape, dtype=torch.bfloat16, device=hi.device)
    slab, info = None, None
    if index32 is not None and table is not None:
        chunks = _lib.lib().dm_attention_split_bwd_chunks(B, N, H)
        slab = torch.empty((chunks, H, N, N), dtype=torch.float32, device=hi.device)
        info = (chunks, N, relpos_index_csr(index32, n_bins))
    c = (0, 0, 0) if cube is None else tuple(int(v) for v in cube)
    fn = _lib.lib().dm_attention_split_bwd_pair if pair else _lib.lib().dm_attention_split_bwd
    check(fn(hi.data_ptr(), lo.data_ptr(), _ptr(table), c[0], c[1], c[2], out.data_ptr(), dout.data_ptr(),
             dhi.data_ptr(), dlo.data_ptr(), lse.data_ptr(), dqkv.data_ptr(), delta.data_ptr(), _ptr(slab),
             B, N, H, D, scale, _stream()), "dm_attention_split_bwd")
    return (Planes(dqkv) if pair else dqkv), slab, info


def relpos_index_csr(index32: torch.Tensor, n_bins: int):
    key = (index32._version, n_bins)
    hit = getattr(index32, "_dm_csr", None)
    if hit is None or hit[0] != key:
        flat = index32.reshape(-1).to(torch.int64)
        ok = (flat >= 0) & (flat < n_bins)
        where = torch.nonzero(ok).reshape(-1)
        order = torch.argsort(flat[where], stable=True)
        positions = where[order].to(torch.int32).contiguous()
        counts = torch.bincount(flat[where], minlength=n_bins)
        offsets = torch.zeros(n_bins + 1, dtype=torch.int64, device=index32.device)
        offsets[1:] = torch.cumsum(counts, 0)
        hit = index32._dm_csr = (key, positions, offsets.to(torch.int32).contiguous())
    return hit[1], hit[2]


def attention_bwd(qkv, bias, out, dout, lse, B, N, H, D, scale, index32=None, n_bins=0, bias_t=None, table=None, cube=None):
    _need_cuda(qkv, bias, out, dout, lse, index32, bias_t, table)
    dqkv = torch.empty_like(qkv)
    delta = torch.empty((B, H, N), dtype=torch.float32, device=qkv.device)
    slab, info = None, None
    if index32 is not None:
        if D != 64 or N > 256:
            raise ValueError(f"the relative-position bias gradient needs head dim 64 and N <= 256 (got D={D}, N={N})")
        chunks = _lib.lib().dm_attention_bwd_batch_chunks(B, N, H, _dt(qkv))
        slab = torch.empty((chunks, H, N, N), dtype=torch.float32, device=qkv.device)
        info = (chunks, N, relpos_index_csr(index32, n_bins))
    if table is not None and cube is not None:
        check(_lib.lib().dm_attention_bwd_relpos(qkv.data_ptr(), table.data_ptr(), int(cube[0]), int(cube[1]), int(cube[2]), _ptr(bias),
                                                 _ptr(bias_t), out.data_ptr(), dout.data_ptr(), lse.data_ptr(), dqkv.data_ptr(),
                                                 delta.data_ptr(), _ptr(slab), B, N, H, D, scale, _dt(qkv), _stream()),
              "dm_attention_bwd_relpos")
        return dqkv, slab, info
    check(_lib.lib().dm_attention_bwd(qkv.data_ptr(), _ptr(bias), _ptr(bias_t), out.data_ptr(), dout.data_ptr(), lse.data_ptr(), dqkv.data_ptr(),
                                      delta.data_ptr(), _ptr(slab), B, N, H, D, scale, _dt(qkv), _stream()),
          "dm_attention_bwd")
    return dqkv, slab, info


def relpos_bias_scatter(slab, dtable, B, H, info, n_bins, accumulate=False):
    _need_cuda(slab, dtable)
    chunks, N, (positions, offsets) = info
    check(_lib.lib().dm_relpos_bias_reduce(slab.data_ptr(), positions.data_ptr(), offsets.data_ptr(), dtable.data_ptr(), chunks, H, N,
                                           n_bins, int(accumulate), _stream()), "dm_relpos_bias_reduce")
    return dtable


def patchify(x: torch.Tensor, patch: int, dtype: torch.dtype) -> torch.Tensor:
    _need_cuda(x)
    B, Cc, H, W = x.shape
    if H != W:
        raise ValueError("square images only")
    x = x.contiguous()
    g = H // patch
    cols = torch.empty((B * g * g, Cc * patch * patch), dtype=dtype, device=x.device)
    check(_lib.lib().dm_patchify(x.data_ptr(), cols.data_ptr(), _dt(cols), B, Cc, H, patch, _stream()), "dm_patchify")
    return cols


RESIZE_RULES = {"opencv": 0, "exact_area": 1}


def _resize_rule(resize: str) -> int:
    if resize not in RESIZE_RULES:
        raise ValueError(f"resize must be one of {tuple(RESIZE_RULES)}, got {resize!r}")
    return RESIZE_RULES[resize]


def patch_pyramid(tile: torch.Tensor, xy: torch.Tensor, windows: torch.Tensor, target: int, max_window: Optional[int] = None,
                  resize: str = "opencv") -> torch.Tensor:
    _need_cuda(tile, xy, windows)
    if tile.dtype != torch.uint8:
        raise ValueError("tile must be uint8")
    bands, H, W = tile.shape
    P = xy.shape[0]
    if max_window is None:
        max_window = int(windows.max().item())
    out = torch.empty((P, bands, target, target), dtype=torch.float32, device=tile.device)
    check(_lib.lib().dm_patch_pyramid(tile.contiguous().data_ptr(), bands, H, W, xy.to(torch.int32).contiguous().data_ptr(),
                                      windows.to(torch.int32).contiguous().data_ptr(), max_window, P, target, _resize_rule(resize),
                                      out.data_ptr(), _stream()), "dm_patch_pyramid")
    return out


class PatchCols:

    def __init__(self, cols: torch.Tensor, batch: int, side: int, patch: int, bands: int):
        self.cols, self.batch, self.side, self.patch, self.bands = cols, batch, side, patch, bands

    @property
    def shape(self):
        return (self.batch, self.bands, self.side, self.side)

    def __getitem__(self, sl):
        g2 = (self.side // self.patch) ** 2
        if not isinstance(sl, slice) or sl.step not in (None, 1):
            raise TypeError("PatchCols supports contiguous batch slices only")
        a, b, _ = sl.indices(self.batch)
        return PatchCols(self.cols[a * g2:b * g2], b - a, self.side, self.patch, self.bands)

    def to(self, *_a, **_k):
        return self

    @staticmethod
    def cat(a: "PatchCols", b: "PatchCols") -> "PatchCols":
        if (a.side, a.patch, a.bands, a.cols.dtype) != (b.side, b.patch, b.bands, b.cols.dtype):
            raise ValueError("PatchCols.cat: the two sides were built for different scales / dtypes")
        ca, cb = a.cols, b.cols
        if (ca.is_contiguous() and cb.is_contiguous() and ca.untyped_storage().data_ptr() == cb.untyped_storage().data_ptr()
                and cb.data_ptr() == ca.data_ptr() + ca.numel() * ca.element_size()):
            both = ca.as_strided((ca.shape[0] + cb.shape[0], ca.shape[1]), (ca.shape[1], 1), ca.storage_offset())
        else:
            both = torch.cat((ca, cb), 0)
        return PatchCols(both, a.batch + b.batch, a.side, a.patch, a.bands)


def cat_batch(a, b):
    if isinstance(a, PatchCols) or isinstance(b, PatchCols):
        return PatchCols.cat(a, b)
    return torch.cat((a, b), 0)


def pair_batch_gather(tiles: torch.Tensor, tile_id: Optional[torch.Tensor], xy: torch.Tensor, inner: torch.Tensor, obj: torch.Tensor,
                      scale_index: int, target: int, max_window: int, out: torch.Tensor, grid: int = 0, resize: str = "opencv",
                      region_features: Optional[torch.Tensor] = None, designed: Optional[torch.Tensor] = None,
                      error_flag: Optional[torch.Tensor] = None) -> None:
    _need_cuda(tiles, tile_id, xy, inner, obj, out, region_features, designed, error_flag)
    if tiles.dtype != torch.uint8 or tiles.dim() != 4 or not tiles.is_contiguous():
        raise ValueError("tiles must be a contiguous uint8 [T, bands, H, W] tensor")
    for name, t in (("tile_id", tile_id), ("xy", xy), ("inner", inner), ("obj", obj), ("error_flag", error_flag)):
        if t is not None and (t.dtype != torch.int32 or not t.is_contiguous()):
            raise ValueError(f"{name} must be a contiguous int32 tensor (a per-step cast would be a launch of its own)")
    T, bands, H, W = tiles.shape
    P = xy.shape[0]
    if not out.is_contiguous() or out.numel() != P * bands * target * target:
        raise ValueError(f"out must be contiguous with {P * bands * target * target} elements, got {tuple(out.shape)}")
    if (region_features is None) != (designed is None):
        raise ValueError("designed rows need the region features (and vice versa)")
    if designed is not None and (designed.dtype != torch.float32 or designed.numel() != P * 19 or not designed.is_contiguous()
                                 or region_features.dtype != torch.float32 or region_features.numel() != P * 15 or not region_features.is_contiguous()):
        raise ValueError("region_features must be contiguous float32 [P, 15] and designed contiguous float32 [P, 1, 19]")
    check(_lib.lib().dm_pair_batch_gather(tiles.data_ptr(), T, bands, H, W, _ptr(tile_id), xy.data_ptr(), inner.data_ptr(), obj.data_ptr(),
                                          scale_index, max_window, P, target, grid, _resize_rule(resize), out.data_ptr(), _dt(out),
                                          _ptr(region_features), _ptr(designed), _ptr(error_flag), _stream()), "dm_pair_batch_gather")


def pair_epoch_draw(pairs: torch.Tensor, pair_flag: torch.Tensor, poly_off: torch.Tensor, poly_pts: torch.Tensor, pt_tile: torch.Tensor,
                    pt_xy: torch.Tensor, pt_inner: torch.Tensor, pt_obj: torch.Tensor, pt_region: torch.Tensor, seed: int, epoch: int, batch: int,
                    tile_id: torch.Tensor, xy: torch.Tensor, inner: torch.Tensor, obj: torch.Tensor, region: torch.Tensor, flag: torch.Tensor,
                    point_id: Optional[torch.Tensor] = None) -> None:
    if pairs.dim() != 2 or pairs.shape[1] != 2:
        raise ValueError(f"pair_epoch_draw: pairs must be [N, 2], got {tuple(pairs.shape)}")
    N, n_pts = pairs.shape[0], pt_tile.numel()
    cols = {"pairs": (pairs, torch.int32, 2 * N), "pair_flag": (pair_flag, torch.int32, N), "poly_off": (poly_off, torch.int32, poly_off.numel()),
            "poly_pts": (poly_pts, torch.int32, poly_pts.numel()), "pt_tile": (pt_tile, torch.int32, n_pts), "pt_xy": (pt_xy, torch.int32, 2 * n_pts),
            "pt_inner": (pt_inner, torch.int32, n_pts), "pt_obj": (pt_obj, torch.int32, n_pts), "pt_region": (pt_region, torch.float32, 15 * n_pts),
            "tile_id": (tile_id, torch.int32, 2 * N), "xy": (xy, torch.int32, 4 * N), "inner": (inner, torch.int32, 2 * N),
            "obj": (obj, torch.int32, 2 * N), "region": (region, torch.float32, 30 * N), "flag": (flag, torch.float32, N),
            "point_id": (point_id, torch.int32, 2 * N)}
    _need_cuda(*(t for t, _, _ in cols.values()))
    for name, (t, dtype, numel) in cols.items():
        if t is not None and (t.dtype != dtype or not t.is_contiguous() or t.numel() != numel):
            raise ValueError(f"pair_epoch_draw: {name} must be a contiguous {dtype} tensor of {numel} elements, got {t.dtype} {tuple(t.shape)}")
    a = _lib.DmPairDraw()
    for name, (t, _, _) in cols.items():
        setattr(a, name, _ptr(t))
    a.seed = int(seed) & 0xFFFFFFFFFFFFFFFF
    a.n_pairs, a.n_poly, a.n_poly_pts, a.n_pts = N, poly_off.numel() - 1, poly_pts.numel(), n_pts
    a.epoch, a.batch = int(epoch), int(batch)
    with torch.cuda.device(pairs.device):
        check(_lib.lib().dm_pair_epoch_draw(C.byref(a), _stream()), "dm_pair_epoch_draw")


def patch_pyramid_cols(tile: torch.Tensor, xy: torch.Tensor, windows: torch.Tensor, target: int, grid: int = 8,
                       dtype: torch.dtype = torch.bfloat16, max_window: Optional[int] = None, resize: str = "opencv") -> PatchCols:
    _need_cuda(tile, xy, windows)
    if tile.dtype != torch.uint8:
        raise ValueError("tile must be uint8")
    bands, H, W = tile.shape
    P = xy.shape[0]
    if target % grid:
        raise ValueError(f"target {target} is not a multiple of the token grid {grid}")
    ps = target // grid
    if max_window is None:
        max_window = int(windows.max().item())
    cols = torch.empty((P * grid * grid, bands * ps * ps), dtype=dtype, device=tile.device)
    check(_lib.lib().dm_patch_pyramid_cols(tile.contiguous().data_ptr(), bands, H, W, xy.to(torch.int32).contiguous().data_ptr(),
                                           windows.to(torch.int32).contiguous().data_ptr(), max_window, P, target, grid, _resize_rule(resize),
                                           cols.data_ptr(), _dt(cols), _stream()), "dm_patch_pyramid_cols")
    return PatchCols(cols, P, target, ps, bands)


def adam_step(param, grad, m, v, step, lr=1e-4, beta1=0.9, beta2=0.999, eps=1e-8, grad_scale=1.0, param_lp=None):
    _need_cuda(param, grad, m, v)
    check(_lib.lib().dm_adam_step(param.data_ptr(), grad.data_ptr(), m.data_ptr(), v.data_ptr(), _ptr(param_lp), param.numel(), step,
                                  lr, beta1, beta2, eps, grad_scale, _stream()), "dm_adam_step")


def adam_hyper(step: int, lr: float, beta1: float = 0.9, beta2: float = 0.999) -> torch.Tensor:
    h = torch.empty(2, dtype=torch.float32).pin_memory() if torch.cuda.is_available() else torch.empty(2, dtype=torch.float32)
    check(_lib.lib().dm_adam_hyper(step, lr, beta1, beta2, h.data_ptr()), "dm_adam_hyper")
    return h


def adam_step_dev(param, grad, m, v, hyper_dev, beta1=0.9, beta2=0.999, eps=1e-8, grad_scale=1.0, param_lp=None, param_lo=None):
    _need_cuda(param, grad, m, v, hyper_dev)
    if param_lo is not None:
        check(_lib.lib().dm_adam_step_dev_pair(param.data_ptr(), grad.data_ptr(), m.data_ptr(), v.data_ptr(), param_lp.data_ptr(), param_lo.data_ptr(),
                                               param.numel(), hyper_dev.data_ptr(), beta1, beta2, eps, grad_scale, _stream()), "dm_adam_step_dev_pair")
        return
    check(_lib.lib().dm_adam_step_dev(param.data_ptr(), grad.data_ptr(), m.data_ptr(), v.data_ptr(), _ptr(param_lp), param.numel(),
                                      hyper_dev.data_ptr(), beta1, beta2, eps, grad_scale, _stream()), "dm_adam_step_dev")


def segment_mean(F: torch.Tensor, ptr: torch.Tensor, idx: torch.Tensor, validate: bool = True) -> torch.Tensor:
    _need_cuda(F, ptr, idx)
    S, D = ptr.numel() - 1, F.shape[1]
    if validate and S > 0:
        bad = (ptr[1:] < ptr[:-1]).any() | (ptr[0] != 0) | (ptr[-1] > idx.numel())
        if idx.numel():
            bad = bad | (idx.min() < 0) | (idx.max() >= F.shape[0])
        if bool(bad):
            raise ValueError("segment_mean: ptr must be non-decreasing from 0 to <= len(idx) and idx must index rows of F")
    pooled = torch.empty((S, D), dtype=torch.float32, device=F.device)
    check(_lib.lib().dm_segment_mean(F.data_ptr(), ptr.data_ptr(), idx.data_ptr(), pooled.data_ptr(), S, D, _stream()), "dm_segment_mean")
    return pooled


def edge_similarity(pooled: torch.Tensor, edges: torch.Tensor, margin: float = 1.0, validate: bool = True):
    _need_cuda(pooled, edges)
    E, D = edges.shape[0], pooled.shape[1]
    if validate and E > 0 and int(edges.max()) >= pooled.shape[0]:
        raise ValueError(f"edge_similarity: edge endpoint {int(edges.max())} is not a row of pooled (S = {pooled.shape[0]}); negative ids mean 'no polygon'")
    simi = torch.empty(E, dtype=torch.float32, device=pooled.device)
    merge = torch.empty(E, dtype=torch.uint8, device=pooled.device)
    check(_lib.lib().dm_edge_similarity(pooled.data_ptr(), edges.data_ptr(), simi.data_ptr(), merge.data_ptr(), E, D, margin, _stream()),
          "dm_edge_similarity")
    return simi, merge


def contrastive_terms(a: torch.Tensor, b: torch.Tensor, flag: torch.Tensor, margin: float = 1.0,
                      d2: Optional[torch.Tensor] = None, term: Optional[torch.Tensor] = None):
    _need_cuda(a, b, flag, d2, term)
    if a.dim() != 2 or tuple(a.shape) != tuple(b.shape) or a.shape[0] < 1 or a.shape[1] < 1:
        raise ValueError(f"contrastive_terms: a and b must be the same non-empty [B, D], got {tuple(a.shape)} and {tuple(b.shape)}")
    B = a.shape[0]
    for name, t, shape in (("a", a, tuple(a.shape)), ("b", b, tuple(a.shape)), ("flag", flag, (B,)), ("d2", d2, (B,)), ("term", term, (B,))):
        if t is not None and (t.dtype != torch.float32 or not t.is_contiguous() or tuple(t.shape) != shape):
            raise ValueError(f"contrastive_terms: {name} must be a contiguous float32 tensor of shape {shape}, got {t.dtype} {tuple(t.shape)}")
    d2 = torch.empty(B, dtype=torch.float32, device=a.device) if d2 is None else d2
    term = torch.empty(B, dtype=torch.float32, device=a.device) if term is None else term
    with torch.cuda.device(a.device):
        check(_lib.lib().dm_contrastive_terms(a.data_ptr(), b.data_ptr(), flag.data_ptr(), float(margin), d2.data_ptr(), term.data_ptr(),
                                              B, a.shape[1], _stream()), "dm_contrastive_terms")
    return d2, term


PAIR_EVAL_MAX_THRESHOLDS = 1024


def pair_eval_summary(term: torch.Tensor, simi: torch.Tensor, flag: torch.Tensor, thresholds: torch.Tensor, validate: bool = True,
                      out: Optional[torch.Tensor] = None) -> torch.Tensor:
    _need_cuda(term, simi, flag, thresholds, out)
    N = term.numel()
    for name, t in (("term", term), ("simi", simi), ("flag", flag)):
        if t.dtype != torch.float32 or not t.is_contiguous() or t.dim() != 1 or t.numel() != N:
            raise ValueError(f"pair_eval_summary: {name} must be a contiguous float32 [N] tensor (N = {N}), got {t.dtype} {tuple(t.shape)}")
    if not 1 <= N <= 2 ** 31 - 1:
        raise ValueError(f"pair_eval_summary: N = {N} pairs (1 .. 2^31 - 1)")
    T = thresholds.numel()
    if thresholds.dtype != torch.float32 or not thresholds.is_contiguous() or thresholds.dim() != 1 or not 1 <= T <= PAIR_EVAL_MAX_THRESHOLDS:
        raise ValueError(f"pair_eval_summary: thresholds must be a contiguous float32 [T] tensor with 1 <= T <= {PAIR_EVAL_MAX_THRESHOLDS}, "
                         f"got {thresholds.dtype} {tuple(thresholds.shape)}")
    if validate:
        th = thresholds.cpu()
        if not bool(torch.isfinite(th).all()) or (T > 1 and not bool((th[1:] > th[:-1]).all())):
            raise ValueError("pair_eval_summary: thresholds must be finite and strictly ascending")
    if out is None:
        out = torch.empty(2 * T + 2, dtype=torch.int64, device=term.device)
    elif out.dtype != torch.int64 or not out.is_contiguous() or out.numel() != 2 * T + 2:
        raise ValueError(f"pair_eval_summary: out must be a contiguous int64 tensor of {2 * T + 2} elements")
    lib = _lib.lib()
    ws = workspace(lib.dm_pair_eval_workspace_bytes(N, T), term.device, slot="eval")
    with torch.cuda.device(term.device):
        check(lib.dm_pair_eval_summary(term.data_ptr(), simi.data_ptr(), flag.data_ptr(), N, thresholds.data_ptr(), T, ws.data_ptr(),
                                       out.data_ptr(), out.data_ptr() + 16, out.data_ptr() + 8, _stream()), "dm_pair_eval_summary")
    return out


_DIST_DTYPES = {torch.float32: DM_F32, torch.float64: _lib.DM_F64}


def pairwise_distance(X: torch.Tensor, Y: torch.Tensor) -> torch.Tensor:
    _need_cuda(X, Y)
    if X.dim() != 2 or Y.dim() != 2:
        raise ValueError(f"pairwise_distance: X and Y must be 2-D, got {tuple(X.shape)} and {tuple(Y.shape)}")
    if X.shape[1] != Y.shape[1]:
        raise ValueError(f"pairwise_distance: feature widths differ ({X.shape[1]} != {Y.shape[1]})")
    if X.dtype != Y.dtype or X.dtype not in _DIST_DTYPES:
        raise ValueError(f"pairwise_distance: X and Y must both be float32 or float64, got {X.dtype} and {Y.dtype}")
    if X.device != Y.device:
        raise ValueError(f"pairwise_distance: X on {X.device}, Y on {Y.device}")
    n, m, p = X.shape[0], Y.shape[0], X.shape[1]
    if n == 0 or m == 0:
        return torch.empty((n, m), dtype=X.dtype, device=X.device)
    if p == 0:
        return torch.zeros((n, m), dtype=X.dtype, device=X.device)
    X, Y = X.detach().contiguous(), Y.detach().contiguous()
    D = torch.empty((n, m), dtype=X.dtype, device=X.device)
    with torch.cuda.device(X.device):
        check(_lib.lib().dm_pairwise_distance(X.data_ptr(), Y.data_ptr(), D.data_ptr(), n, m, p, _DIST_DTYPES[X.dtype], _stream()),
              "dm_pairwise_distance")
    return D


def _as_operand(t: torch.Tensor, dtype: torch.dtype) -> torch.Tensor:
    t = t.contiguous()
    if t.dtype == dtype:
        return t
    if t.dtype == torch.float32:
        return cast(t, dtype)
    raise ValueError(f"cannot use a {t.dtype} gradient with {dtype} operands")


def _linear_backward(x, w, dy, need_dx, need_dw, need_db, wshape, wparam=None, bparam=None):
    M, K = x.shape
    N = w.shape[0]
    dx = dw = db = None
    if need_dx:
        dx = torch.empty((M, K), dtype=x.dtype, device=x.device)
        gemm(DM_NN, dy, w, dx, M, K, N, lda=N, ldb=K, ldc=K)
    wsink = _multi_use_sink(wparam, (N, K)) if need_dw else None
    bsink = _multi_use_sink(bparam, (N,)) if need_db else None
    if need_db:
        db = bsink if bsink is not None else torch.empty(N, dtype=torch.float32, device=x.device)
    if need_dw:
        dw = wsink if wsink is not None else torch.empty((N, K), dtype=torch.float32, device=x.device)
        gemm(DM_TN, dy, x, dw, N, K, M, lda=N, ldb=K, ldc=K, accumulate=_acc(wparam, wsink is not None),
             colsum_out=db, colsum_accumulate=_acc(bparam, bsink is not None))
        dw = None if wsink is not None else dw.reshape(wshape)
    elif need_db:
        colsum(dy, db, accumulate=_acc(bparam, bsink is not None))
    if bsink is not None:
        db = None
    return dx, dw, db


class LinearFn(torch.autograd.Function):

    @staticmethod
    def forward(ctx, x, weight, bias, residual, out_dtype):
        _save_products(ctx)
        x = x.contiguous()
        M, K = x.shape
        N = weight.shape[0]
        w = lp_weight(weight, x.dtype, (N, K))
        y = torch.empty((M, N), dtype=out_dtype, device=x.device)
        gemm(DM_NT, x, w, y, M, N, K, lda=K, ldb=K, ldc=N, bias=bias,
             residual=None if residual is None else residual.contiguous())
        ctx.save_for_backward(x, w)
        ctx.has_bias, ctx.wshape = bias is not None, weight.shape
        ctx.params = (weight, bias)
        return y

    @staticmethod
    @_replay_products
    def backward(ctx, dy):
        x, w = ctx.saved_tensors
        dres = dy if ctx.needs_input_grad[3] else None
        dyo = _as_operand(dy, x.dtype)
        dx, dw, db = _linear_backward(x, w, dyo, ctx.needs_input_grad[0], ctx.needs_input_grad[1],
                                      ctx.has_bias and ctx.needs_input_grad[2], ctx.wshape, *ctx.params)
        return dx, dw, db, dres, None


class PatchEmbedCatFn(torch.autograd.Function):

    @staticmethod
    def forward(ctx, S, T, *args):
        _save_products(ctx)
        cols, weights, biases = args[:S], args[S:2 * S], args[2 * S:3 * S]
        B = cols[0].shape[0] // T
        Cc = weights[0].shape[0]
        cube = torch.empty((B, S * T, Cc), dtype=torch.float32, device=cols[0].device)
        flat = cube.view(-1)
        ws = []
        for i in range(S):
            c = cols[i].contiguous()
            K = c.shape[1]
            w = lp_weight(weights[i], c.dtype, (Cc, K))
            ws.append(w)
            gemm(DM_NT, c, w, flat[i * T * Cc:], B * T, Cc, K, lda=K, ldb=K, ldc=Cc, bias=biases[i], rows_per_group=T, group_stride=S * T * Cc)
        ctx.save_for_backward(*cols, *ws)
        ctx.cfg = (S, T, B, Cc)
        ctx.params = (weights, biases)
        return cube

    @staticmethod
    @_replay_products
    def backward(ctx, dcube):
        S, T, B, Cc = ctx.cfg
        saved = ctx.saved_tensors
        cols, ws = saved[:S], saved[S:]
        weights, biases = ctx.params
        grads_w, grads_b = [], []
        same = all(c.dtype == cols[0].dtype for c in cols)
        dys = torch.empty((S, B, T, Cc), dtype=cols[0].dtype, device=dcube.device).copy_(dcube.contiguous().view(B, S, T, Cc).transpose(0, 1)) if same else None
        for i in range(S):
            c = cols[i]
            K = c.shape[1]
            dy = dys[i].view(B * T, Cc) if same else dcube[:, i * T:(i + 1) * T, :].to(c.dtype).reshape(B * T, Cc)
            need_w, need_b = ctx.needs_input_grad[2 + S + i], ctx.needs_input_grad[2 + 2 * S + i]
            _, dw, db = _linear_backward(c, ws[i], dy, False, need_w, need_b and biases[i] is not None, weights[i].shape, weights[i], biases[i])
            grads_w.append(dw)
            grads_b.append(db)
        return (None, None) + (None,) * S + tuple(grads_w) + tuple(grads_b)


class MlpFn(torch.autograd.Function):

    @staticmethod
    def forward(ctx, x, w1, b1, w2, b2, residual, out_dtype):
        _save_products(ctx)
        x = x.contiguous()
        M, K = x.shape
        Hd, N = w1.shape[0], w2.shape[0]
        w1c = cast(w1.reshape(Hd, K), x.dtype)
        w2c = cast(w2.reshape(N, Hd), x.dtype)
        pre = torch.empty((M, Hd), dtype=x.dtype, device=x.device)
        h = torch.empty((M, Hd), dtype=x.dtype, device=x.device)
        gemm(DM_NT, x, w1c, h, M, Hd, K, lda=K, ldb=K, ldc=Hd, bias=b1, epilogue=DM_EPI_GELU_GRAD, aux=pre, ldaux=Hd)
        y = torch.empty((M, N), dtype=out_dtype, device=x.device)
        gemm(DM_NT, h, w2c, y, M, N, Hd, lda=Hd, ldb=Hd, ldc=N, bias=b2,
             residual=None if residual is None else residual.contiguous())
        ctx.save_for_backward(x, w1c, w2c, pre, h)
        ctx.shapes = (w1.shape, w2.shape)
        ctx.params = (w1, b1, w2, b2)
        return y

    @staticmethod
    @_replay_products
    def backward(ctx, dy):
        x, w1c, w2c, pre, h = ctx.saved_tensors
        M, K = x.shape
        Hd, N = w1c.shape[0], w2c.shape[0]
        need = ctx.needs_input_grad
        dres = dy if need[5] else None
        dyo = _as_operand(dy, x.dtype)
        w1, b1, w2, b2 = ctx.params
        _, dw2, db2 = _linear_backward(h, w2c, dyo, False, need[3], need[4], ctx.shapes[1], w2, b2)
        dpre = torch.empty((M, Hd), dtype=x.dtype, device=x.device)
        gemm(DM_NN, dyo, w2c, dpre, M, Hd, N, lda=N, ldb=Hd, ldc=Hd, epilogue=DM_EPI_MUL, aux=pre, ldaux=Hd)
        dx, dw1, db1 = _linear_backward(x, w1c, dpre, need[0], need[1], need[2], ctx.shapes[0], w1, b1)
        return dx, dw1, db1, dw2, db2, dres, None


class LayerNormFn(torch.autograd.Function):

    @staticmethod
    def forward(ctx, x, gamma, beta, eps, out_dtype):
        x = x.contiguous()
        y, mean, rstd = layernorm_fwd(x, gamma, beta, eps, out_dtype)
        ctx.save_for_backward(x, gamma, mean, rstd)
        ctx.params = (gamma, beta)
        return y

    @staticmethod
    def backward(ctx, dy):
        x, gamma, mean, rstd = ctx.saved_tensors
        C = gamma.numel()
        gs, bs = _multi_use_sink(ctx.params[0], (C,)), _multi_use_sink(ctx.params[1], (C,))
        if gs is not None and bs is not None and ctx.needs_input_grad[1] and ctx.needs_input_grad[2]:
            acc = _acc(ctx.params[0], True)
            _acc(ctx.params[1], True)
            r = layernorm_bwd(dy.contiguous(), x, gamma, mean, rstd, dgamma=gs, dbeta=bs, accumulate=acc)
            return r[0], None, None, None, None
        dx, dg, db = layernorm_bwd(dy.contiguous(), x, gamma, mean, rstd)
        return dx, dg, db, None, None


class AttentionFn(torch.autograd.Function):

    @staticmethod
    def forward(ctx, qkv, table, index32, B, N, H, D, scale):
        qkv = qkv.contiguous()
        bias = bias_t = None
        cube = _inkernel_cube(table, index32, B, N, H, D, qkv.dtype)
        split, scube = _split_attention(table, index32, qkv, B, N, H, D)
        if split:
            out, lse, hi, lo = attention_fwd_split(qkv, None if table is None else table.contiguous(), scube, B, N, H, D, scale)
            ctx.save_for_backward(hi, lo, out, lse, index32, table)
            ctx.dims = (B, N, H, D, scale, None if table is None else table.shape[0])
            ctx.split_cube = (scube,)
            return out
        elif cube is not None:
            out, lse = attention_fwd_relpos(qkv, table.contiguous(), cube, B, N, H, D, scale)
        else:
            if table is not None:
                bias, bias_t = relpos_bias_gather(table.contiguous(), index32, N, transposed=True)
            out, lse = attention_fwd(qkv, bias, B, N, H, D, scale)
        ctx.save_for_backward(qkv, out, lse, bias, bias_t, index32, table if cube is not None else None)
        ctx.dims = (B, N, H, D, scale, None if table is None else table.shape[0])
        return out

    @staticmethod
    def backward(ctx, dout):
        B, N, H, D, scale, n_bins = ctx.dims
        if getattr(ctx, "split_cube", None) is not None:
            hi, lo, out, lse, index32, table = ctx.saved_tensors
            want_table = table is not None and ctx.needs_input_grad[1]
            dqkv, slab, rows = attention_bwd_split(hi, lo, None if table is None else table.contiguous(), ctx.split_cube[0], out,
                                                   dout.contiguous().float(), lse, B, N, H, D, scale, index32 if want_table else None, n_bins or 0)
            dtable = None
            if want_table:
                dtable = torch.empty((n_bins, H), dtype=torch.float32, device=hi.device)
                relpos_bias_scatter(slab, dtable, B, H, rows, n_bins)
            return dqkv, dtable, None, None, None, None, None, None
        qkv, out, lse, bias, bias_t, index32, table = ctx.saved_tensors
        cube = None
        if table is not None:
            table, cube = table.contiguous(), index32._dm_cube
        want_table = (bias is not None or table is not None) and ctx.needs_input_grad[1]
        dqkv, slab, rows = attention_bwd(qkv, bias, out, _as_operand(dout, qkv.dtype), lse, B, N, H, D, scale,
                                         index32 if want_table else None, n_bins or 0, bias_t=bias_t, table=table, cube=cube)
        dtable = None
        if want_table:
            dtable = torch.empty((n_bins, H), dtype=torch.float32, device=qkv.device)
            relpos_bias_scatter(slab, dtable, B, H, rows, n_bins)
        return dqkv, dtable, None, None, None, None, None, None


class GRUCellFn(torch.autograd.Function):

    @staticmethod
    def forward(ctx, gi, gh, h):
        _need_cuda(gi, gh, h)
        B, H = h.shape
        if gi.shape != (B, 3 * H) or gh.shape != (B, 3 * H) or gi.stride(1) != 1:
            raise ValueError(f"GRUCellFn: gi {tuple(gi.shape)} / gh {tuple(gh.shape)} do not fit h {tuple(h.shape)}")
        gh, h = gh.contiguous(), h.contiguous()
        h_new = torch.empty_like(h)
        saved = torch.empty((B, 4 * H), dtype=torch.float32, device=h.device)
        check(_lib.lib().dm_gru_cell_fwd(gi.data_ptr(), gi.stride(0), gh.data_ptr(), h.data_ptr(), h_new.data_ptr(), saved.data_ptr(), B, H,
                                         _stream()), "dm_gru_cell_fwd")
        ctx.save_for_backward(saved, h)
        return h_new

    @staticmethod
    def backward(ctx, dh_new):
        saved, h = ctx.saved_tensors
        B, H = h.shape
        dh_new = dh_new.contiguous()
        dgi = torch.empty((B, 3 * H), dtype=torch.float32, device=h.device)
        dgh, dh = torch.empty_like(dgi), torch.empty_like(h)
        check(_lib.lib().dm_gru_cell_bwd(dh_new.data_ptr(), saved.data_ptr(), h.data_ptr(), dgi.data_ptr(), dgh.data_ptr(), dh.data_ptr(), B, H,
                                         _stream()), "dm_gru_cell_bwd")
        return dgi, dgh, dh


class BatchNormReluFn(torch.autograd.Function):

    @staticmethod
    def forward(ctx, x, gamma, beta, running_mean, running_var, mask, rows_per_sample, eps, momentum, training, relu):
        _need_cuda(x, gamma, beta, running_mean, running_var, mask)
        x = x.float().contiguous()
        M, Cc = x.shape
        if training and M <= 1:
            raise ValueError(f"Expected more than 1 value per channel when training, got input size {tuple(x.shape)}")
        y = torch.empty_like(x)
        mean = torch.empty(Cc, dtype=torch.float32, device=x.device)
        rstd = torch.empty(Cc, dtype=torch.float32, device=x.device)
        if mask is not None:
            mask = mask.float().contiguous()
            if mask.shape != (M // rows_per_sample, Cc):
                raise ValueError(f"mask must be [samples, C] = {(M // rows_per_sample, Cc)}, got {tuple(mask.shape)}")
        ws = workspace(_lib.lib().dm_batchnorm_workspace_bytes(M, Cc), x.device, "bn")
        check(_lib.lib().dm_batchnorm_fwd(x.data_ptr(), gamma.data_ptr(), beta.data_ptr(), _ptr(running_mean), _ptr(running_var), _ptr(mask),
                                          rows_per_sample, y.data_ptr(), mean.data_ptr(), rstd.data_ptr(), M, Cc, eps, momentum, int(training),
                                          int(relu), ws.data_ptr(), _stream()), "dm_batchnorm_fwd")
        ctx.save_for_backward(x, y, gamma, mask, mean, rstd)
        ctx.cfg = (rows_per_sample, bool(training), bool(relu))
        ctx.params = (gamma, beta)
        return y

    @staticmethod
    def backward(ctx, dy):
        x, y, gamma, mask, mean, rstd = ctx.saved_tensors
        rows_per_sample, training, relu = ctx.cfg
        M, Cc = x.shape
        dx = torch.empty_like(x)
        gs, bs = _multi_use_sink(ctx.params[0], (Cc,)), _multi_use_sink(ctx.params[1], (Cc,))
        direct = gs is not None and bs is not None
        dg = gs if direct else torch.empty(Cc, dtype=torch.float32, device=x.device)
        db = bs if direct else torch.empty(Cc, dtype=torch.float32, device=x.device)
        ws = workspace(_lib.lib().dm_batchnorm_workspace_bytes(M, Cc), x.device, "bn")
        acc = _acc(ctx.params[0], direct)
        _acc(ctx.params[1], direct)
        check(_lib.lib().dm_batchnorm_bwd(dy.float().contiguous().data_ptr(), x.data_ptr(), y.data_ptr(), gamma.data_ptr(), _ptr(mask), rows_per_sample,
                                          mean.data_ptr(), rstd.data_ptr(), dx.data_ptr(), dg.data_ptr(), db.data_ptr(), int(acc), M, Cc,
                                          int(training), int(relu), ws.data_ptr(), _stream()), "dm_batchnorm_bwd")
        return dx, (None if direct else dg), (None if direct else db), None, None, None, None, None, None, None, None


class TokenPoolFn(torch.autograd.Function):

    @staticmethod
    def forward(ctx, x, S, side):
        x = x.contiguous()
        B, N, Cc = x.shape
        y = torch.empty((B, S * (side // 2) ** 2, Cc), dtype=torch.float32, device=x.device)
        check(_lib.lib().dm_token_pool_fwd(x.data_ptr(), y.data_ptr(), B, S, side, Cc, _stream()), "dm_token_pool_fwd")
        ctx.dims = (B, S, side, Cc)
        return y

    @staticmethod
    def backward(ctx, dy):
        B, S, side, Cc = ctx.dims
        dy = dy.contiguous()
        dx = torch.empty((B, S * side * side, Cc), dtype=torch.float32, device=dy.device)
        check(_lib.lib().dm_token_pool_bwd(dy.data_ptr(), dx.data_ptr(), B, S, side, Cc, _stream()), "dm_token_pool_bwd")
        return dx, None, None


class GroupMeanFn(torch.autograd.Function):

    @staticmethod
    def forward(ctx, x, g):
        x = x.contiguous()
        rows, Cc = x.numel() // (x.shape[-1] * g), x.shape[-1]
        y = torch.empty((rows, Cc), dtype=torch.float32, device=x.device)
        check(_lib.lib().dm_group_mean_fwd(x.data_ptr(), y.data_ptr(), rows, g, Cc, _stream()), "dm_group_mean_fwd")
        ctx.dims = (rows, g, Cc, x.shape)
        return y

    @staticmethod
    def backward(ctx, dy):
        rows, g, Cc, xshape = ctx.dims
        dy = dy.contiguous()
        dx = torch.empty(xshape, dtype=torch.float32, device=dy.device)
        check(_lib.lib().dm_group_mean_bwd(dy.data_ptr(), dx.data_ptr(), rows, g, Cc, _stream()), "dm_group_mean_bwd")
        return dx, None


class ContrastiveLossFn(torch.autograd.Function):

    @staticmethod
    def forward(ctx, a, b, flag, margin):
        a, b = a.contiguous(), b.contiguous()
        B, D = a.shape
        flag = flag.to(torch.float32).contiguous()
        loss = torch.empty(1, dtype=torch.float32, device=a.device)
        da, db = torch.empty_like(a), torch.empty_like(b)
        check(_lib.lib().dm_contrastive_loss(a.data_ptr(), b.data_ptr(), flag.data_ptr(), margin, 1.0, loss.data_ptr(),
                                             da.data_ptr(), db.data_ptr(), B, D, _stream()), "dm_contrastive_loss")
        ctx.save_for_backward(da, db)
        return loss.reshape(())

    @staticmethod
    def backward(ctx, g):
        da, db = ctx.saved_tensors
        if is_unit_grad(g):
            return da, db, None, None
        return da * g, db * g, None, None


_unit_grads = {}


def unit_grad(device) -> torch.Tensor:
    key = torch.device(device)
    t = _unit_grads.get(key)
    if t is None:
        t = _unit_grads[key] = torch.ones((), dtype=torch.float32, device=key)
    return t


def is_unit_grad(g: torch.Tensor) -> bool:
    t = _unit_grads.get(g.device)
    return t is not None and g.data_ptr() == t.data_ptr() and g.dim() == 0


def split_halves(f: torch.Tensor):
    B = f.shape[0] // 2
    a, b = f[:B], f[B:]
    a._dm_pair, b._dm_pair = f, f
    return a, b


def stacked_halves(a: torch.Tensor, b: torch.Tensor):
    f = getattr(a, "_dm_pair", None)
    if f is None or f is not getattr(b, "_dm_pair", None) or f.dim() != 2 or not f.is_contiguous() or a.shape != b.shape:
        return None
    B, D = a.shape
    if tuple(f.shape) != (2 * B, D) or a.data_ptr() != f.data_ptr() or b.data_ptr() != f.data_ptr() + B * D * f.element_size():
        return None
    return f


class ContrastivePairLossFn(torch.autograd.Function):

    @staticmethod
    def forward(ctx, both, flag, margin):
        B, D = both.shape[0] // 2, both.shape[1]
        flag = flag.to(torch.float32).contiguous()
        loss = torch.empty(1, dtype=torch.float32, device=both.device)
        d = torch.empty_like(both)
        check(_lib.lib().dm_contrastive_loss(both.data_ptr(), both[B:].data_ptr(), flag.data_ptr(), margin, 1.0, loss.data_ptr(),
                                             d.data_ptr(), d[B:].data_ptr(), B, D, _stream()), "dm_contrastive_loss")
        ctx.save_for_backward(d)
        return loss.reshape(())

    @staticmethod
    def backward(ctx, g):
        d, = ctx.saved_tensors
        return (d if is_unit_grad(g) else d * g), None, None


def contrastive_loss(a: torch.Tensor, b: torch.Tensor, flag: torch.Tensor, margin: float) -> torch.Tensor:
    both = stacked_halves(a, b) if (a.dtype == torch.float32 and b.dtype == torch.float32) else None
    if both is not None:
        return ContrastivePairLossFn.apply(both, flag, margin)
    return ContrastiveLossFn.apply(a, b, flag, margin)


class CrossEntropyFn(torch.autograd.Function):

    @staticmethod
    def forward(ctx, logits, target):
        _need_cuda(logits, target)
        x = logits.float().contiguous()
        B, K = x.shape
        loss = torch.empty(1, dtype=torch.float32, device=x.device)
        dl = torch.empty_like(x)
        if target.dtype.is_floating_point:
            if target.shape != x.shape:
                raise ValueError(f"probability targets must be [B,K] = {tuple(x.shape)}, got {tuple(target.shape)}")
            t = target.float().contiguous()
            ti, tp = 0, t.data_ptr()
        else:
            if target.shape != (B,):
                raise ValueError(f"index targets must be [B] = ({B},), got {tuple(target.shape)}")
            t = target.to(torch.int64).contiguous()
            if B and (int(t.min()) < 0 or int(t.max()) >= K):
                raise IndexError(f"Target {int(t.max())} is out of bounds.")
            ti, tp = t.data_ptr(), 0
        check(_lib.lib().dm_cross_entropy(x.data_ptr(), ti, tp, 1.0, loss.data_ptr(), dl.data_ptr(), B, K, _stream()), "dm_cross_entropy")
        ctx.save_for_backward(dl)
        return loss.reshape(())

    @staticmethod
    def backward(ctx, g):
        (dl,) = ctx.saved_tensors
        return dl * g, None




def lp_weight(weight: torch.Tensor, dtype: torch.dtype, shape2d) -> torch.Tensor:
    if dtype == torch.float32:
        return weight.reshape(shape2d)
    lp = getattr(weight, "_dm_lp", None)
    if lp is not None and lp.dtype == dtype:
        return lp.reshape(shape2d)
    return cast(weight.reshape(shape2d), dtype)


def pair_weight(weight: torch.Tensor, w2d: torch.Tensor) -> Planes:
    src = getattr(weight, "_dm_pair_src", None)
    if src is not None and _PLANES:
        flat, off = src
        rows, cols = w2d.shape
        if rows * cols == weight.numel() and off % 8 == 0 and flat.shape[1] % 8 == 0:
            return Planes(torch.as_strided(flat, (2, rows, cols), (flat.shape[1], cols, 1), off))
    return split_planes(w2d)


def _operand_grad(dy: torch.Tensor, dtype: torch.dtype) -> torch.Tensor:
    if dy.dtype == dtype and dy.is_contiguous():
        return dy
    lp = getattr(dy, "_dm_lp_copy", None)
    if lp is not None and lp.dtype == dtype and lp.numel() == dy.numel():
        return lp.reshape(dy.shape)
    return _as_operand(dy, dtype)


def _grad_out(param: torch.Tensor, shape, device):
    sink = getattr(param, "_dm_grad_sink", None)
    if sink is not None:
        return sink.view(shape), True
    return torch.empty(shape, dtype=torch.float32, device=device), False


def _acc(param, direct) -> bool:
    if not direct:
        return False
    st = getattr(param, "_dm_gw", None)
    if st is None or st[0]:
        return True
    st[0] = True
    return False


def _multi_use_sink(param, shape):
    if param is None:
        return None
    sink = getattr(param, "_dm_grad_sink", None)
    return None if sink is None else sink.view(shape)


def _grad_done(param: torch.Tensor, g: torch.Tensor, direct: bool):
    if not direct:
        return g.view(param.shape) if g.shape != param.shape else g
    return None


_WGRAD_SIDE_TOKENS = int(os.environ.get("DM_WGRAD_STREAM", "0"))
_WGRAD_GROUP_TOKENS = int(os.environ.get("DM_WGRAD_GROUP", "12288"))
_WGRAD_PAIR = os.environ.get("DM_WGRAD_PAIR", "1") != "0"
_side_streams = {}


def _side_stream(device):
    key = torch.device(device).index
    st = _side_streams.get(key)
    if st is None:
        st = _side_streams[key] = torch.cuda.Stream(device=device)
    return st


class BlockFn(torch.autograd.Function):

    @staticmethod
    def forward(ctx, x, n1w, n1b, table, index32, qkv_w, qkv_b, proj_w, proj_b, n2w, n2b, fc1_w, fc1_b, fc2_w, fc2_b,
                heads, eps, scale, dtype):
        _save_products(ctx)
        x = x.contiguous()
        B, N, Cc = x.shape
        M, Hd, D = B * N, fc1_w.shape[0], Cc // heads
        dev = x.device
        wq, wp = lp_weight(qkv_w, dtype, (3 * Cc, Cc)), lp_weight(proj_w, dtype, (Cc, Cc))
        w1, w2 = lp_weight(fc1_w, dtype, (Hd, Cc)), lp_weight(fc2_w, dtype, (Cc, Hd))
        x2d = x.view(M, Cc)
        planes = (dtype == torch.float32 and _FP32_PRODUCTS == "bf16x3" and planes_ok(M, Cc) and planes_ok(M, Hd) and planes_ok(Hd, Cc)
                  and Cc <= _PAIR_LN_MAX_COLS and M * Cc * Cc >= _SPLIT_MIN_WORK)
        if planes:
            wq, wp, w1, w2 = (pair_weight(P, w) for P, w in ((qkv_w, wq), (proj_w, wp), (fc1_w, w1), (fc2_w, w2)))
        y1, mean1, rstd1 = layernorm_fwd(x2d, n1w, n1b, eps, dtype, pair=planes)
        split, scube = _split_attention(table, index32, dtype, B, N, heads, D)
        qkv = (Planes(torch.empty((2, M, 3 * Cc), dtype=torch.bfloat16, device=dev)) if (planes and split)
               else torch.empty((M, 3 * Cc), dtype=dtype, device=dev))
        gemm(DM_NT, y1, wq, qkv, M, 3 * Cc, Cc, lda=Cc, ldb=Cc, ldc=3 * Cc, bias=qkv_b)
        bias = bias_t = None
        cube = _inkernel_cube(table, index32, B, N, heads, D, dtype)
        split_imgs = None
        if split:
            o_op = None
            if planes:
                o, lse, hi, lo, o_op = attention_fwd_split(qkv, None if table is None else table.contiguous(), scube, B, N, heads, D, scale, out_pair=True)
            else:
                o, lse, hi, lo = attention_fwd_split(qkv, None if table is None else table.contiguous(), scube, B, N, heads, D, scale)
            split_imgs = (hi, lo, scube)
        elif cube is not None:
            o, lse = attention_fwd_relpos(qkv, table.contiguous(), cube, B, N, heads, D, scale)
        else:
            if table is not None:
                bias, bias_t = relpos_bias_gather(table.contiguous(), index32, N, transposed=True)
            o, lse = attention_fwd(qkv, bias, B, N, heads, D, scale)
        x1 = torch.empty((M, Cc), dtype=torch.float32, device=dev)
        if not (planes and split):
            o_op = split_planes(o.view(M, Cc)) if planes else o.view(M, Cc)
        gemm(DM_NT, o_op, wp, x1, M, Cc, Cc, lda=Cc, ldb=Cc, ldc=Cc, bias=proj_b, residual=x2d)
        y2, mean2, rstd2 = layernorm_fwd(x1, n2w, n2b, eps, dtype, pair=planes)
        h = Planes(torch.empty((2, M, Hd), dtype=torch.bfloat16, device=dev)) if planes else torch.empty((M, Hd), dtype=dtype, device=dev)
        if any(ctx.needs_input_grad):
            pre = torch.empty((M, Hd), dtype=dtype, device=dev)
            gemm(DM_NT, y2, w1, h, M, Hd, Cc, lda=Cc, ldb=Cc, ldc=Hd, bias=fc1_b, epilogue=DM_EPI_GELU_GRAD, aux=pre, ldaux=Hd)
        else:
            pre = None
            gemm(DM_NT, y2, w1, h, M, Hd, Cc, lda=Cc, ldb=Cc, ldc=Hd, bias=fc1_b, epilogue=DM_EPI_GELU)
        x2 = torch.empty((M, Cc), dtype=torch.float32, device=dev)
        gemm(DM_NT, h, w2, x2, M, Cc, Hd, lda=Hd, ldb=Hd, ldc=Cc, bias=fc2_b, residual=x1)
        if planes:
            y1, y2, h, wq, wp, w1, w2, o_op = y1.t, y2.t, h.t, wq.t, wp.t, w1.t, w2.t, o_op.t
            if isinstance(qkv, Planes):
                qkv = qkv.t
        ctx.planes = planes
        ctx.save_for_backward(x2d, mean1, rstd1, y1, qkv, o, lse, bias, bias_t, index32, x1, mean2, rstd2, y2, pre, h,
                              wq, wp, w1, w2, n1w, n2w, o_op if planes else None)
        ctx.dims = (B, N, Cc, heads, D, Hd, scale, None if table is None else table.shape[0])
        ctx.table_in_kernel = cube is not None
        ctx.split_imgs = split_imgs
        ctx.params = (n1w, n1b, table, qkv_w, qkv_b, proj_w, proj_b, n2w, n2b, fc1_w, fc1_b, fc2_w, fc2_b)
        return x2.view(B, N, Cc)

    @staticmethod
    @_replay_products
    def backward(ctx, dx2):
        (x, mean1, rstd1, y1, qkv, o, lse, bias, bias_t, index32, x1, mean2, rstd2, y2, pre, h,
         wq, wp, w1, w2, n1w, n2w, o_op) = ctx.saved_tensors
        planes = ctx.planes
        if planes:
            y1, y2, h, wq, wp, w1, w2, o_op = (Planes(t_) for t_ in (y1, y2, h, wq, wp, w1, w2, o_op))
        (P_n1w, P_n1b, P_table, P_qkv_w, P_qkv_b, P_proj_w, P_proj_b, P_n2w, P_n2b, P_fc1_w, P_fc1_b, P_fc2_w, P_fc2_b) = ctx.params
        B, N, Cc, heads, D, Hd, scale, n_bins = ctx.dims
        M = B * N
        dtype, dev = (torch.float32 if planes else y1.dtype), x.device
        lp = dtype != torch.float32
        lp_copy = getattr(dx2, "_dm_lp_copy", None)
        dy_pair = getattr(dx2, "_dm_planes", None)
        if dy_pair is not None and dy_pair[1] != (dx2.data_ptr(), dx2._version):
            dy_pair = None
        elif dy_pair is not None:
            dy_pair = dy_pair[0]
        dx2 = dx2.contiguous().view(M, Cc)
        if lp_copy is not None:
            dx2._dm_lp_copy = lp_copy
        dy = _operand_grad(dx2, dtype)
        if planes and isinstance(dy_pair, Planes) and (dy_pair.rows, dy_pair.cols) == (M, Cc):
            dy = dy_pair
        dw2, k_w2 = _grad_out(P_fc2_w, (Cc, Hd), dev)
        db2, k_b2 = _grad_out(P_fc2_b, (Cc,), dev)
        side = _side_stream(dev) if 0 < M <= _WGRAD_SIDE_TOKENS else None

        pending = [] if (side is None and (lp or planes) and 0 < M <= _WGRAD_GROUP_TOKENS) else None
        late = [] if (pending is None and side is None and (lp or planes) and _WGRAD_PAIR) else None

        def wgrad(*a, pair=False, **kw):
            if pending is not None:
                pending.append((a, kw))
                return None
            if late is not None and pair:
                late.append((a, kw))
                return None
            if side is None:
                return gemm(*a, **kw)
            side.wait_stream(torch.cuda.current_stream())
            with torch.cuda.stream(side):
                return gemm(*a, ws_slot="gemm_side", **kw)

        def bias_grad(g2d, db, acc_b, direct):
            if planes and not isinstance(g2d, Planes):
                g2d = split_planes(g2d)
            return g2d, dict(colsum_out=db, colsum_accumulate=acc_b)
        dy, cs = bias_grad(dy, db2, _acc(P_fc2_b, k_b2), k_b2)
        wgrad(DM_TN, dy, h, dw2, Cc, Hd, M, lda=Cc, ldb=Hd, ldc=Hd, accumulate=_acc(P_fc2_w, k_w2), **cs)
        dpre = Planes(torch.empty((2, M, Hd), dtype=torch.bfloat16, device=dev)) if planes else torch.empty((M, Hd), dtype=dtype, device=dev)
        gemm(DM_NN, dy, w2, dpre, M, Hd, Cc, lda=Cc, ldb=Hd, ldc=None if planes else Hd, epilogue=DM_EPI_MUL, aux=pre, ldaux=Hd)
        dw1, k_w1 = _grad_out(P_fc1_w, (Hd, Cc), dev)
        db1, k_b1 = _grad_out(P_fc1_b, (Hd,), dev)
        dpre, cs = bias_grad(dpre, db1, _acc(P_fc1_b, k_b1), k_b1)
        wgrad(DM_TN, dpre, y2, dw1, Hd, Cc, M, lda=Hd, ldb=Cc, ldc=Cc, accumulate=_acc(P_fc1_w, k_w1), **cs)
        dy2 = torch.empty((M, Cc), dtype=dtype, device=dev)
        gemm(DM_NN, dpre, w1, dy2, M, Cc, Hd, lda=Hd, ldb=Cc, ldc=Cc)
        dg2, k_n2 = _grad_out(P_n2w, (Cc,), dev)
        dbt2, k_n2b = _grad_out(P_n2b, (Cc,), dev)
        if k_n2 != k_n2b:
            dg2, dbt2, k_n2, k_n2b = torch.empty(Cc, device=dev), torch.empty(Cc, device=dev), False, False
        a_n2 = _acc(P_n2w, k_n2)
        _acc(P_n2b, k_n2b)
        r = layernorm_bwd(dy2, x1, n2w, mean2, rstd2, dres=dx2, dgamma=dg2, dbeta=dbt2, accumulate=a_n2, want_lp=lp, defer=bool(k_n2 and k_n2b),
                          want_pair=planes)
        dx1, dx1_lp = (r[0], r[1]) if (lp or planes) else (r[0], r[0])
        dwp, k_wp = _grad_out(P_proj_w, (Cc, Cc), dev)
        dbp, k_bp = _grad_out(P_proj_b, (Cc,), dev)
        dx1_op, cs = bias_grad(dx1_lp, dbp, _acc(P_proj_b, k_bp), k_bp)
        wgrad(DM_TN, dx1_op, o_op if planes else o.view(M, Cc), dwp, Cc, Cc, M, lda=Cc, ldb=Cc, ldc=Cc, accumulate=_acc(P_proj_w, k_wp), pair=True, **cs)
        do = torch.empty((M, Cc), dtype=dtype, device=dev)
        gemm(DM_NN, dx1_op, wp, do, M, Cc, Cc, lda=Cc, ldb=Cc, ldc=Cc)
        tab, cube = None, None
        if ctx.split_imgs is not None:
            hi, lo, scube = ctx.split_imgs
            ctx.split_imgs = None
            want_table = P_table is not None
            dqkv, slab, rows = attention_bwd_split(hi, lo, None if P_table is None else P_table.detach().contiguous(), scube, o.view(B, N, Cc),
                                                   do.view(B, N, Cc), lse, B, N, heads, D, scale, index32 if want_table else None, n_bins or 0,
                                                   pair=planes)
        else:
            if ctx.table_in_kernel:
                tab, cube = P_table.detach().contiguous(), index32._dm_cube
            want_table = bias is not None or tab is not None
            dqkv, slab, rows = attention_bwd(qkv, bias, o, do, lse, B, N, heads, D, scale,
                                             index32 if want_table else None, n_bins or 0, bias_t=bias_t, table=tab, cube=cube)
        dtable, k_t = None, False
        if want_table:
            dtable, k_t = _grad_out(P_table, (n_bins, heads), dev)
            relpos_bias_scatter(slab, dtable, B, heads, rows, n_bins, accumulate=_acc(P_table, k_t))
        dqkv2 = dqkv if isinstance(dqkv, Planes) else dqkv.view(M, 3 * Cc)
        dwq, k_wq = _grad_out(P_qkv_w, (3 * Cc, Cc), dev)
        dbq, k_bq = _grad_out(P_qkv_b, (3 * Cc,), dev)
        dqkv_op, cs = bias_grad(dqkv2, dbq, _acc(P_qkv_b, k_bq), k_bq)
        wgrad(DM_TN, dqkv_op, y1, dwq, 3 * Cc, Cc, M, lda=3 * Cc, ldb=Cc, ldc=Cc, accumulate=_acc(P_qkv_w, k_wq), pair=True, **cs)
        dy1 = torch.empty((M, Cc), dtype=dtype, device=dev)
        gemm(DM_NN, dqkv_op, wq, dy1, M, Cc, 3 * Cc, lda=3 * Cc, ldb=Cc, ldc=Cc)
        dg1, k_n1 = _grad_out(P_n1w, (Cc,), dev)
        dbt1, k_n1b = _grad_out(P_n1b, (Cc,), dev)
        if k_n1 != k_n1b:
            dg1, dbt1, k_n1, k_n1b = torch.empty(Cc, device=dev), torch.empty(Cc, device=dev), False, False
        a_n1 = _acc(P_n1w, k_n1)
        _acc(P_n1b, k_n1b)
        r = layernorm_bwd(dy1, x, n1w, mean1, rstd1, dres=dx1, dgamma=dg1, dbeta=dbt1, accumulate=a_n1, want_lp=lp, defer=bool(k_n1 and k_n1b),
                          want_pair=planes)
        if side is not None:
            torch.cuda.current_stream().wait_stream(side)
        if pending:
            gemm_grouped(pending)
        if late:
            gemm_grouped(late)
        dx = r[0].view(B, N, Cc)
        if lp:
            dx._dm_lp_copy = r[1]
        if planes:
            dx._dm_planes = (r[1], (dx.data_ptr(), dx._version))
        return (dx, _grad_done(P_n1w, dg1, k_n1), _grad_done(P_n1b, dbt1, k_n1b),
                _grad_done(P_table, dtable, k_t) if want_table else None, None,
                _grad_done(P_qkv_w, dwq, k_wq), _grad_done(P_qkv_b, dbq, k_bq),
                _grad_done(P_proj_w, dwp, k_wp), _grad_done(P_proj_b, dbp, k_bp),
                _grad_done(P_n2w, dg2, k_n2), _grad_done(P_n2b, dbt2, k_n2b),
                _grad_done(P_fc1_w, dw1, k_w1), _grad_done(P_fc1_b, db1, k_b1),
                _grad_done(P_fc2_w, dw2, k_w2), _grad_done(P_fc2_b, db2, k_b2), None, None, None, None)
```

include/deepmerge_hip.h:

```cpp
#ifndef DEEPMERGE_HIP_H
#define DEEPMERGE_HIP_H

#include <stdint.h>

#ifdef __cplusplus
extern "C" {
#endif

typedef enum { DM_F32 = 0, DM_BF16 = 1,
               DM_BF16_PAIR = 2,
               DM_F64 = 3
} DmDtype;

typedef enum {
  DM_OK = 0,
  DM_ERR_BAD_SHAPE = -1,
  DM_ERR_BAD_DTYPE = -2,
  DM_ERR_BAD_ALIGN = -3,
  DM_ERR_WORKSPACE = -4,
  DM_ERR_HIP = -5,
  DM_ERR_UNSUPPORTED = -6
} DmStatus;

int dm_abi_version(void);
const char *dm_last_error(void);
const char *dm_arch(void);

typedef enum { DM_NT = 0, DM_NN = 1, DM_TN = 2 } DmGemmLayout;
typedef enum { DM_EPI_NONE = 0, DM_EPI_GELU = 1, DM_EPI_DGELU = 2, DM_EPI_GELU_GRAD = 3, DM_EPI_MUL = 4 } DmEpilogue;

typedef struct {
  int32_t layout;
  int32_t ab_dtype;
  int32_t c_dtype;
  int32_t aux_dtype;
  int32_t M, N, K;
  int32_t epilogue;
  int32_t accumulate;
  int32_t split_k;
  const void *A; int64_t lda;
  const void *B; int64_t ldb;
  void *C; int64_t ldc;
  const float *bias;
  const float *residual; int64_t ldr;
  void *aux; int64_t ldaux;
  int32_t rows_per_group; int64_t group_stride;
  void *workspace; int64_t workspace_bytes;
  float *colsum_a; int32_t colsum_accumulate;
  int32_t k_fold;
  int64_t a_fold[3], b_fold[3];
  int64_t c_plane;
} DmGemmArgs;

int dm_gemm(const DmGemmArgs *args, void *stream);
int64_t dm_gemm_workspace_bytes(int32_t layout, int32_t M, int32_t N, int32_t K);
int dm_gemm_grouped(const DmGemmArgs *args, int32_t n, void *stream);

int dm_attention_fwd(const void *qkv, const float *bias, void *out, float *lse,
                     int32_t B, int32_t N, int32_t H, int32_t D, float scale, int32_t dtype, void *stream);
int32_t dm_attention_relpos_inkernel(int32_t B, int32_t N, int32_t H, int32_t D, int32_t cube_s, int32_t cube_h,
                                     int32_t cube_w, int32_t dtype);
int dm_attention_fwd_relpos(const void *qkv, const float *table, int32_t cube_s, int32_t cube_h, int32_t cube_w,
                            void *out, float *lse, int32_t B, int32_t N, int32_t H, int32_t D, float scale,
                            int32_t dtype, void *stream);
int dm_attention_bwd(const void *qkv, const float *bias, const float *bias_t, const void *out, const void *dout,
                     const float *lse, void *dqkv, float *delta, float *dbias_slab, int32_t B, int32_t N, int32_t H,
                     int32_t D, float scale, int32_t dtype, void *stream);
int dm_attention_bwd_relpos(const void *qkv, const float *table, int32_t cube_s, int32_t cube_h, int32_t cube_w,
                            const float *bias, const float *bias_t, const void *out, const void *dout, const float *lse,
                            void *dqkv, float *delta, float *dbias_slab, int32_t B, int32_t N, int32_t H, int32_t D,
                            float scale, int32_t dtype, void *stream);
int32_t dm_attention_split_ok(int32_t B, int32_t N, int32_t H, int32_t D, int32_t has_table, int32_t cube_s, int32_t cube_h,
                              int32_t cube_w);
int dm_attention_split_fwd(const float *qkv, void *qkv_hi, void *qkv_lo, const float *table, int32_t cube_s, int32_t cube_h,
                           int32_t cube_w, float *out, float *lse, int32_t B, int32_t N, int32_t H, int32_t D, float scale,
                           void *stream);
int dm_attention_split_fwd_pair(const float *qkv, void *qkv_hi, void *qkv_lo, const float *table, int32_t cube_s, int32_t cube_h,
                                int32_t cube_w, float *out, void *out_pair, float *lse, int32_t B, int32_t N, int32_t H, int32_t D,
                                float scale, void *stream);
int32_t dm_attention_split_bwd_chunks(int32_t B, int32_t N, int32_t H);
int dm_attention_split_bwd(const void *qkv_hi, const void *qkv_lo, const float *table, int32_t cube_s, int32_t cube_h,
                           int32_t cube_w, const float *out, const float *dout, void *dout_hi, void *dout_lo,
                           const float *lse, float *dqkv, float *delta, float *dbias_slab, int32_t B, int32_t N,
                           int32_t H, int32_t D, float scale, void *stream);
int dm_attention_split_bwd_pair(const void *qkv_hi, const void *qkv_lo, const float *table, int32_t cube_s, int32_t cube_h,
                                int32_t cube_w, const float *out, const float *dout, void *dout_hi, void *dout_lo,
                                const float *lse, void *dqkv_pair, float *delta, float *dbias_slab, int32_t B, int32_t N,
                                int32_t H, int32_t D, float scale, void *stream);
int32_t dm_attention_bwd_batch_chunks(int32_t B, int32_t N, int32_t H, int32_t dtype);

int dm_relpos_bias_gather(const float *table, const int32_t *index, float *bias, float *bias_t,
                          int32_t N, int32_t H, int32_t n_bins, void *stream);
int dm_relpos_bias_reduce(float *dbias_slab, const int32_t *positions, const int32_t *offsets, float *dtable,
                          int32_t chunks, int32_t H, int32_t N, int32_t n_bins, int32_t accumulate, void *stream);

int dm_layernorm_fwd(const float *x, const float *gamma, const float *beta, void *y, int32_t y_dtype,
                     float *mean, float *rstd, int32_t rows, int32_t cols, float eps, void *stream);
int dm_layernorm_bwd(const void *dy, int32_t dy_dtype, const float *x, const float *gamma,
                     const float *mean, const float *rstd, const float *dres, float *dx, void *dx_lp,
                     float *dgamma, float *dbeta, int32_t accumulate_params, float *partial,
                     int32_t rows, int32_t cols, void *stream);
int64_t dm_layernorm_bwd_partial_floats(int32_t cols);
int dm_layernorm_bwd_partials(const void *dy, int32_t dy_dtype, const float *x, const float *gamma,
                              const float *mean, const float *rstd, const float *dres, float *dx, void *dx_lp,
                              float *partial, int32_t rows, int32_t cols, int32_t *n_partial, void *stream);
int dm_layernorm_bwd_partials_pair(const void *dy, int32_t dy_dtype, const float *x, const float *gamma,
                                   const float *mean, const float *rstd, const float *dres, float *dx, void *dx_pair, float *partial,
                                   int32_t rows, int32_t cols, int32_t *n_partial, void *stream);
typedef struct DmReduceItem {
  const float *partial;
  float *out0, *out1;
  int32_t nrows, width, split, accumulate;
} DmReduceItem;
int dm_partial_reduce_batch(const DmReduceItem *items, int32_t n, void *stream);

int dm_token_pool_fwd(const float *x, float *y, int32_t B, int32_t S, int32_t side, int32_t C, void *stream);
int dm_token_pool_bwd(const float *dy, float *dx, int32_t B, int32_t S, int32_t side, int32_t C, void *stream);
int dm_group_mean_fwd(const float *x, float *y, int32_t rows, int32_t g, int32_t C, void *stream);
int dm_group_mean_bwd(const float *dy, float *dx, int32_t rows, int32_t g, int32_t C, void *stream);

int dm_colsum(const void *X, int32_t dtype, int64_t ldx, float *out, int32_t M, int32_t N,
              int32_t accumulate, float *partial, void *stream);
int64_t dm_colsum_partial_floats(int32_t N);

int dm_cast(const float *src, void *dst, int32_t dst_dtype, int64_t n, void *stream);

int dm_split_bf16(const float *src, int64_t ld, int64_t rows, int64_t cols, void *dst, int32_t stack, int32_t pattern, void *stream);
int64_t dm_split_colsum_partial_floats(int64_t rows, int64_t cols);
int dm_split_bf16_planes(const float *src, int64_t ld, int64_t rows, int64_t cols, void *dst, float *partial, int32_t *n_partial, void *stream);
int dm_split_bf16_colsum(const float *src, int64_t ld, int64_t rows, int64_t cols, void *dst, int32_t stack, int32_t pattern,
                         float *partial, int32_t *n_partial, void *stream);

int dm_patchify(const float *x, void *cols, int32_t dtype, int32_t B, int32_t C, int32_t side, int32_t p, void *stream);

int dm_contrastive_loss(const float *a, const float *b, const float *flag, float margin, float upstream,
                        float *loss, float *da, float *db, int32_t B, int32_t D, void *stream);

int dm_cross_entropy(const float *logits, const int64_t *target_index, const float *target_prob, float upstream,
                     float *loss, float *dlogits, int32_t B, int32_t K, void *stream);

int dm_adam_step(float *param, const float *grad, float *m, float *v, void *param_lp, int64_t n,
                 int32_t step, double lr, double beta1, double beta2, double eps, double grad_scale, void *stream);

int dm_adam_hyper(int32_t step, double lr, double beta1, double beta2, float *hyper_host);
int dm_adam_step_dev(float *param, const float *grad, float *m, float *v, void *param_lp, int64_t n, const float *hyper_dev,
                     double beta1, double beta2, double eps, double grad_scale, void *stream);
int dm_adam_step_dev_pair(float *param, const float *grad, float *m, float *v, void *param_hi, void *param_lo, int64_t n,
                          const float *hyper_dev, double beta1, double beta2, double eps, double grad_scale, void *stream);

int dm_segment_mean(const float *F, const int32_t *ptr, const int32_t *idx, float *pooled,
                    int32_t S, int32_t D, void *stream);
int dm_edge_similarity(const float *pooled, const int32_t *edges, float *simi, uint8_t *merge,
                       int32_t E, int32_t D, float margin, void *stream);
int dm_pairwise_distance(const void *X, const void *Y, void *D, int32_t n, int32_t m, int32_t p, int32_t dtype, void *stream);

#define DM_RESIZE_OPENCV 0
#define DM_RESIZE_EXACT_AREA 1
int dm_patch_pyramid(const uint8_t *tile, int32_t bands, int32_t H, int32_t W, const int32_t *xy, const int32_t *windows,
                     int32_t max_window, int32_t P, int32_t target, int32_t resize_rule, float *out, void *stream);
int dm_patch_pyramid_cols(const uint8_t *tile, int32_t bands, int32_t H, int32_t W, const int32_t *xy, const int32_t *windows,
                          int32_t max_window, int32_t P, int32_t target, int32_t grid, int32_t resize_rule, void *cols, int32_t dtype,
                          void *stream);

int dm_pair_batch_gather(const uint8_t *tiles, int32_t n_tiles, int32_t bands, int32_t H, int32_t W, const int32_t *tile_id,
                         const int32_t *xy, const int32_t *inner, const int32_t *obj, int32_t scale_index, int32_t max_window,
                         int32_t P, int32_t target, int32_t grid, int32_t resize_rule, void *out, int32_t dtype,
                         const float *region_features, float *designed, int32_t *error_flag, void *stream);

typedef struct {
  const int32_t *pairs, *pair_flag, *poly_off, *poly_pts;
  const int32_t *pt_tile, *pt_xy, *pt_inner, *pt_obj;
  const float *pt_region;
  int32_t *tile_id, *xy, *inner, *obj;
  float *region, *flag;
  int32_t *point_id;
  uint64_t seed;
  int32_t n_pairs, n_poly, n_poly_pts, n_pts, epoch, batch;
} DmPairDraw;
int dm_pair_epoch_draw(const DmPairDraw *args, void *stream);

int dm_contrastive_terms(const float *a, const float *b, const float *flag, float margin, float *d2, float *term, int32_t B, int32_t D,
                         void *stream);
int64_t dm_pair_eval_workspace_bytes(int64_t N, int32_t T);
int dm_pair_eval_summary(const float *term, const float *simi, const float *flag, int64_t N, const float *thresholds, int32_t T,
                         void *workspace, double *loss_sum, int64_t *merged, int64_t *n_pos, void *stream);

int dm_label_stats(const int32_t *labels, const uint8_t *tile, int32_t bands, int32_t H, int32_t W, int32_t S,
                   int64_t *count, int64_t *sum, int64_t *sumsq, int32_t *bbox, int64_t *peri, void *stream);
int dm_label_features(const int64_t *count, const int64_t *sum, const int64_t *sumsq, const int32_t *bbox, const int64_t *peri,
                      int32_t S, int32_t bands, float *features, void *stream);
int dm_rag_edges(const int32_t *labels, int32_t H, int32_t W, int32_t S, int64_t *table_keys, int32_t *table_counts,
                 int32_t capacity_log2, int64_t *edge_keys, int32_t *edge_counts, int32_t max_edges, int32_t *n_edges,
                 int32_t *overflow, void *stream);

int dm_seam_stitch(const int32_t *a, const int32_t *b, int64_t n, int64_t S, int64_t *peri, int64_t *table_keys,
                   int32_t *table_counts, int32_t capacity_log2, int64_t *edge_keys, int32_t *edge_counts, int32_t max_edges,
                   int32_t *n_edges, int32_t *overflow, void *stream);

int dm_merge_round(const int32_t *edges, const uint8_t *merge, int32_t E, int32_t S, int32_t *parent, int32_t *changed,
                   int32_t init, void *stream);

typedef struct {
  const int32_t *ptr, *idx, *edges, *root, *pick, *rep, *region_of;
  const float *simi;
  const int32_t *weights;
  const int64_t *count, *sum, *sumsq;
  const int32_t *bbox;
  const int64_t *peri;
  int32_t *new_id, *hist_rank, *new_ptr, *new_idx, *new_rep, *new_region_of, *n_regions;
  int64_t *new_count, *new_sum, *new_sumsq;
  int32_t *new_bbox;
  int64_t *new_peri;
  int32_t *history;
  float *history_simi;
  int32_t C, P, E, S0, bands, round, hist_base, hist_cap;
} DmMergeFold;
int dm_merge_best(const int32_t *edges, const float *simi, int32_t E, int32_t C, float margin, uint64_t *best, void *stream);
int dm_merge_match(const int32_t *edges, const uint64_t *best, int32_t E, int32_t C, uint8_t *picked, int32_t *root, int32_t *pick,
                   int32_t *n_picked, void *stream);
int dm_merge_fold_regions(const DmMergeFold *args, void *stream);
int dm_merge_edge_keys(const int32_t *edges, const int32_t *root, const int32_t *new_id, int32_t E, int32_t C, int64_t *keys,
                       void *stream);
int dm_merge_fold_edges(const int64_t *sorted_keys, const int64_t *order, const int32_t *weights, int32_t E, int32_t *new_edges,
                        int32_t *new_weights, int32_t *n_edges, void *stream);
int dm_relabel_raster(const int32_t *labels, const int32_t *map, int32_t *out, int64_t n, int32_t S, void *stream);

int dm_region_merge_cost(const int64_t *count, const int64_t *sum, const int64_t *sumsq, const int32_t *bbox, const int64_t *peri,
                         const int32_t *edges, const int32_t *weights, int32_t E, int32_t C, int32_t bands, double bw0, double bw1,
                         double bw2, double shape, double compactness, float *cost, void *stream);
int dm_pixel_regions(const uint8_t *tile, int32_t bands, int32_t H, int32_t W, int64_t *count, int64_t *sum, int64_t *sumsq,
                     int32_t *bbox, int64_t *peri, int32_t *edges, int32_t *weights, void *stream);

int dm_label_clearance(const int32_t *labels, int32_t H, int32_t W, int32_t max_window, uint64_t *bits, uint8_t *row_dist,
                       uint16_t *clearance, void *stream);
int dm_point_select_round(const int32_t *labels, const uint16_t *clearance, int32_t H, int32_t W, int32_t S, int32_t k, int32_t round,
                          uint64_t *best, int32_t *points, int32_t *point_clearance, int32_t *counts, int32_t *bbox, void *stream);
int dm_point_emit(const int32_t *counts, const int32_t *points, const int32_t *point_clearance, const int32_t *bbox, int32_t S, int32_t k,
                  int32_t max_window, int32_t capacity, int32_t *ptr, int32_t *xy, int32_t *label, int32_t *inner, int32_t *obj,
                  int32_t *round, void *stream);

int dm_label_overlap(const int32_t *labels, const int32_t *truth, int32_t H, int32_t W, int64_t S, int64_t G, int64_t *table_keys,
                     int32_t *table_counts, int32_t capacity_log2, int64_t *cell_keys, int32_t *cell_counts, int32_t max_cells,
                     int32_t *n_cells, int32_t *overflow, void *stream);
int dm_overlap_reduce(const int64_t *cell_keys, const int32_t *cell_counts, int32_t K, int64_t S, int64_t G, uint64_t *row_best,
                      int64_t *row_labelled, int64_t *area, int32_t *owner, int32_t *owner_count, int64_t *size, int32_t *cover,
                      int64_t *summary, void *stream);
int dm_pair_flags(const int32_t *edges, int32_t E, const int64_t *area, const int32_t *owner, const int32_t *owner_count, int32_t S,
                  int32_t purity_pm, int8_t *flags, void *stream);

int dm_slic_iterate(const uint8_t *tile, int32_t bands, int32_t H, int32_t W, int32_t cell, int32_t compactness, int32_t iters,
                    int32_t *centres, int64_t *sums, int32_t *labels, void *stream);
int dm_connected_labels(const int32_t *raster, int32_t H, int32_t W, int32_t use_background, int32_t background, int32_t *parent,
                        int32_t *chunk_counts, int32_t *labels, int32_t *n_labels, void *stream);
int dm_label_area(const int32_t *labels, int32_t H, int32_t W, int32_t S, int32_t *area, void *stream);
int dm_slic_absorb_pick(const int32_t *edges, const int32_t *weights, int32_t E, const int32_t *area, int32_t S, int32_t min_size,
                        uint64_t *best, uint8_t *merge, int32_t *n_picked, void *stream);

typedef struct DmVectorTrace {
  const int32_t *dart, *next, *lab, *other;
  const uint8_t *flags;
  const int64_t *key, *sum;
  const int32_t *ring_of_slot;
  const int64_t *ring_ptr;
  const int32_t *arc_base;
  int32_t *xy;
  int64_t *area2;
  int32_t *arc_first, *arc_left, *arc_right, *arc_vstart, *arc_count;
  const int32_t *arc_pos;
  const int64_t *arc_ptr;
  int32_t *arc_xy;
  int32_t W, D, R, n_arcs;
} DmVectorTrace;
int dm_vector_count(const int32_t *labels, int32_t H, int32_t W, uint8_t *mask, int32_t *tile_off, int32_t *n_darts, void *stream);
int dm_vector_emit(const uint8_t *mask, const int32_t *tile_off, int32_t H, int32_t W, int32_t *first_slot, int32_t *dart, void *stream);
int dm_vector_link(const int32_t *labels, const uint8_t *mask, const int32_t *first_slot, const int32_t *dart, int32_t H, int32_t W,
                   int32_t D, int32_t *next, int32_t *lab, int32_t *other, uint8_t *flags, int64_t *key, void *stream);
int dm_vector_head_round(const int64_t *key_in, const int32_t *jump_in, int64_t *key_out, int32_t *jump_out, int32_t D, int32_t *changed,
                         void *stream);
int dm_vector_rank_init(const int64_t *key, const int32_t *next, const uint8_t *flags, const int32_t *lab, int32_t D, int64_t *sum,
                        int32_t *nxt, int64_t *ring_key, int32_t *ring_slot, int32_t *n_rings, int32_t max_rings, void *stream);
int dm_vector_rank_round(const int64_t *sum_in, const int32_t *nxt_in, int64_t *sum_out, int32_t *nxt_out, int32_t D, int32_t *changed,
                         void *stream);
int dm_vector_ring_emit(const DmVectorTrace *t, void *stream);
int dm_vector_arc_emit(const DmVectorTrace *t, void *stream);

#define DM_SCENE_VECTOR_MAX_SIDE 2147483647LL
#define DM_SCENE_VECTOR_MAX_PIXELS (1LL << 60)
typedef struct DmSceneVectorTrace {
  const int64_t *dart;
  const int32_t *next, *lab, *other;
  const uint8_t *flags;
  const int64_t *key, *sum;
  const int32_t *ring_of_slot;
  const int64_t *ring_ptr;
  const int32_t *arc_base;
  int32_t *xy;
  int64_t *area2;
  int32_t *arc_first, *arc_left, *arc_right, *arc_vstart, *arc_count;
  const int32_t *arc_pos;
  const int64_t *arc_ptr;
  int32_t *arc_xy;
  int64_t W;
  int32_t D, R, n_arcs;
} DmSceneVectorTrace;
int dm_scene_vector_count(const int32_t *labels, int32_t H, int32_t W, int32_t cy0, int32_t cy1, int32_t cx0, int32_t cx1, uint8_t *mask,
                          uint8_t *core_mask, int32_t *tile_off, int32_t *n_darts, void *stream);
int dm_scene_vector_link(const int32_t *labels, const uint8_t *mask, const int32_t *dart, int32_t H, int32_t W, int32_t D, int64_t oy,
                         int64_t ox, int64_t scene_h, int64_t scene_w, int64_t *id, int64_t *succ, int32_t *lab, int32_t *other,
                         uint8_t *succ_flags, void *stream);
int dm_scene_vector_ring_emit(const DmSceneVectorTrace *t, void *stream);
int dm_scene_vector_arc_emit(const DmSceneVectorTrace *t, void *stream);

#define DM_RASTERIZE_SUBPIXEL 256
int dm_rasterize_count(const int32_t *xy, const int64_t *ring_ptr, const int32_t *vert_ring, int32_t V, int32_t R, int32_t H, int32_t W,
                       int32_t *count, void *stream);
int dm_rasterize_emit(const int32_t *xy, const int64_t *ring_ptr, const int32_t *vert_ring, const int32_t *ring_label, const int64_t *scan,
                      int32_t V, int32_t R, int64_t N, int32_t H, int32_t W, int64_t n_labels, int64_t *keys, void *stream);
int dm_rasterize_fill(const int64_t *keys, int64_t N, int32_t H, int32_t W, int32_t fill, int32_t *out, int32_t *error, void *stream);

#define DM_SIMPLIFY_MAX_SIDE 32768
#define DM_SIMPLIFY_MAX_Q (1 << 20)
int dm_simplify_nodes(const int32_t *labels, int32_t H, int32_t W, uint8_t *keep, void *stream);
int dm_simplify_chains(const int32_t *arc_xy, const int64_t *arc_ptr, int32_t A, int64_t Va, int32_t H, int32_t W, int32_t q, uint8_t *keep,
                       int64_t *stack, void *stream);
int dm_simplify_arc_count(const int32_t *arc_xy, const int64_t *arc_ptr, int32_t A, int64_t Va, int32_t H, int32_t W, const uint8_t *keep,
                          int32_t *count, void *stream);
int dm_simplify_arc_emit(const int32_t *arc_xy, const int64_t *arc_ptr, const int64_t *new_ptr, int32_t A, int64_t Va, int64_t Vn, int32_t H,
                         int32_t W, const uint8_t *keep, int32_t *out_xy, void *stream);
int dm_simplify_ring_count(const int32_t *xy, const int64_t *ring_ptr, const int32_t *vert_ring, int32_t V, int32_t R, int32_t H, int32_t W,
                           const uint8_t *keep, int32_t *count, void *stream);
int dm_simplify_ring_emit(const int32_t *xy, const int64_t *ring_ptr, const int32_t *vert_ring, const int64_t *scan, const int64_t *new_ring_ptr,
                          int32_t V, int32_t R, int64_t Vn, int32_t H, int32_t W, const uint8_t *keep, int32_t *out_xy, int64_t *area2,
                          void *stream);

int64_t dm_batchnorm_workspace_bytes(int32_t M, int32_t C);
int dm_batchnorm_fwd(const float *x, const float *gamma, const float *beta, float *running_mean, float *running_var,
                     const float *mask, int32_t rows_per_sample, float *y, float *save_mean, float *save_rstd, int32_t M,
                     int32_t C, float eps, float momentum, int32_t training, int32_t relu, void *workspace, void *stream);
int dm_batchnorm_bwd(const float *dy, const float *x, const float *y, const float *gamma, const float *mask, int32_t rows_per_sample,
                     const float *save_mean, const float *save_rstd, float *dx, float *dgamma, float *dbeta, int32_t accumulate,
                     int32_t M, int32_t C, int32_t training, int32_t relu, void *workspace, void *stream);

int dm_gru_cell_fwd(const float *gi, int64_t gi_stride, const float *gh, const float *h, float *h_new, float *saved,
                    int32_t B, int32_t H, void *stream);
int dm_gru_cell_bwd(const float *dh_new, const float *saved, const float *h, float *dgi, float *dgh, float *dh, int32_t B,
                    int32_t H, void *stream);

typedef struct {
  char name[64];
  int64_t launches;
  double total_ms;
  double total_flops;
  double total_bytes;
} DmProfRow;
int dm_prof_enable(int32_t on);
int32_t dm_prof_collect(DmProfRow *rows, int32_t max_rows);

#ifdef __cplusplus
}
#endif
#endif
```

Baseline: 6365 pairs/s.

## Add short-sequence bf16 attention kernels with in-kernel relpos bias and table gradient

Adds dedicated forward and backward attention kernels for short token counts in bf16. One block handles a head and loops over a chunk of batches, keeping all K/V (and Q/dO in backward) rows in LDS. The relative-position table is staged in LDS and looked up in-kernel, and the table gradient is accumulated through partials, so the dense bias gather and slab scatter are no longer needed. The path is on by default for eligible shapes. The cost is an extra code path and heavy LDS use in the backward kernel, which may limit occupancy.

```diff
diff --git a/deepmerge_amd/_lib.py b/deepmerge_amd/_lib.py
--- a/deepmerge_amd/_lib.py
+++ b/deepmerge_amd/_lib.py
@@ -117,6 +117,10 @@
     "dm_attention_bwd_relpos": (_I, [_P, _P, _I, _I, _I, _P, _P, _P, _P, _P, _P, _P, _P, _I, _I, _I, _I, _F, _I, _P]),
     "dm_attention_bwd": (_I, [_P, _P, _P, _P, _P, _P, _P, _P, _P, _I, _I, _I, _I, _F, _I, _P]),
     "dm_attention_bwd_batch_chunks": (_I, [_I, _I, _I, _I]),
+    "dm_attention_short_ok": (_I, [_I, _I, _I, _I, _I, _I]),
+    "dm_attention_short_partial_floats": (_L, [_I, _I, _I, _I]),
+    "dm_attention_short_fwd": (_I, [_P, _P, _P, _I, _P, _P, _I, _I, _I, _I, _F, _I, _P]),
+    "dm_attention_short_bwd": (_I, [_P, _P, _P, _P, _P, _I, _P, _P, _P, _P, _P, _I, _P, _L, _I, _I, _I, _I, _F, _I, _P]),
     "dm_relpos_bias_gather": (_I, [_P, _P, _P, _P, _I, _I, _I, _P]),
     "dm_relpos_bias_reduce": (_I, [_P, _P, _P, _P, _I, _I, _I, _I, _I, _P]),
     "dm_layernorm_fwd": (_I, [_P, _P, _P, _P, _I, _P, _P, _I, _I, _F, _P]),
diff --git a/deepmerge_amd/csrc/dm_attention.hip b/deepmerge_amd/csrc/dm_attention.hip
--- a/deepmerge_amd/csrc/dm_attention.hip
+++ b/deepmerge_amd/csrc/dm_attention.hip
@@ -1,111 +1,11 @@
 #include "dm_common.h"
 #include "dm_mfma.h"
+#include "dm_attention_tile.h"
 #include "dm_attention_pipe.h"
 #include "dm_attention_x3.h"
 #include "dm_prof.h"
 
 namespace {
-
-constexpr int HD = 64;
-constexpr int QB = 64;
-
-template <typename T> struct AL {
-  static constexpr int RB = HD * (int)sizeof(T);
-  static constexpr int CPRW = RB / 16;
-  static constexpr int KBD = RB / 64;
-  static constexpr int EPC = 16 / (int)sizeof(T);
-  static constexpr int TPB = (sizeof(T) == 2) ? 2 : 1;
-};
-
-template <typename T> __device__ __forceinline__ int swz(int row);
-template <> __device__ __forceinline__ int swz<bf16_t>(int row) {
-  const int t0 = (row >> 1) & 1, t1 = (row >> 2) & 1, t2 = (row >> 3) & 1;
-  return ((t1 ^ t2) << 2) | (t0 << 1) | t1;
-}
-template <> __device__ __forceinline__ int swz<float>(int row) { return row & 15; }
-
-template <typename T> __device__ __forceinline__ int img_off(int row, int chunk) {
-  return row * AL<T>::RB + ((chunk ^ swz<T>(row)) << 4);
-}
-
-template <typename T>
-__device__ __forceinline__ void tile_to_lds(char *lds, const T *g, long long ld, int nvalid, int nrows, int t) {
-  using L = AL<T>;
-  const int c = t % L::CPRW;
-  constexpr int RPI = 256 / L::CPRW;
-  for (int row = t / L::CPRW; row < nrows; row += RPI) {
-    u32x4 v = {0u, 0u, 0u, 0u};
-    if (row < nvalid) v = *reinterpret_cast<const u32x4 *>(g + (long long)row * ld + c * L::EPC);
-    *reinterpret_cast<u32x4 *>(lds + img_off<T>(row, c)) = v;
-  }
-}
-
-template <typename T> __device__ __forceinline__ u32x4 frag_row(const char *lds, int row, int kb, int lane) {
-  return *reinterpret_cast<const u32x4 *>(lds + img_off<T>(row, kb * 4 + (lane >> 4)));
-}
-template <typename T> __device__ __forceinline__ u32x4 frag_tr(const char *lds, int d0, int m, int lane);
-template <> __device__ __forceinline__ u32x4 frag_tr<bf16_t>(const char *lds, int d0, int m, int lane) {
-  const int g = lane >> 4, q = (lane >> 2) & 3, p = lane & 3;
-  const int d = d0 + 4 * p;
-  u32x4 out;
-#pragma unroll
-  for (int half = 0; half < 2; ++half) {
-    const int k = 32 * m + 4 * g + 16 * half + q;
-    const u32x2 w = dm_ds_read_tr16(lds + img_off<bf16_t>(k, d >> 3) + ((d & 7) << 1));
-    out[2 * half] = w[0];
-    out[2 * half + 1] = w[1];
-  }
-  return out;
-}
-template <> __device__ __forceinline__ u32x4 frag_tr<float>(const char *lds, int d0, int m, int lane) {
-  const int g = lane >> 4, d = d0 + (lane & 15);
-  u32x4 out;
-#pragma unroll
-  for (int j = 0; j < 4; ++j) {
-    const int k = 16 * m + 4 * g + j;
-    out[j] = *reinterpret_cast<const unsigned int *>(lds + img_off<float>(k, d >> 2) + ((d & 3) << 2));
-  }
-  return out;
-}
-template <typename T> __device__ __forceinline__ u32x4 gl_frag(const T *rowp, bool valid, int kb, int lane) {
-  u32x4 v = {0u, 0u, 0u, 0u};
-  if (valid) v = *reinterpret_cast<const u32x4 *>(rowp + (kb * 4 + (lane >> 4)) * AL<T>::EPC);
-  return v;
-}
-
-template <typename T, int NKT> __device__ __forceinline__ u32x4 acc_frag(const f32x4 (&s)[NKT], int m) {
-  if constexpr (sizeof(T) == 2) {
-    const f32x4 lo = s[2 * m], hi = s[2 * m + 1];
-    bf16x8 r = {(bf16_t)lo[0], (bf16_t)lo[1], (bf16_t)lo[2], (bf16_t)lo[3], (bf16_t)hi[0], (bf16_t)hi[1], (bf16_t)hi[2], (bf16_t)hi[3]};
-    return __builtin_bit_cast(u32x4, r);
-  } else {
-    return __builtin_bit_cast(u32x4, s[m]);
-  }
-}
-
-template <typename T, int NKT>
-__device__ __forceinline__ void contract_tokens(f32x4 (&o)[4], const f32x4 (&s)[NKT], const char *img, int lane) {
-#pragma unroll
-  for (int m = 0; m < NKT / AL<T>::TPB; ++m) {
-    const u32x4 fp = acc_frag<T, NKT>(s, m);
-#pragma unroll
-    for (int dt = 0; dt < 4; ++dt) mma<T>(o[dt], fp, frag_tr<T>(img, dt * 16, m, lane));
-    if ((m & 1) == 1) __builtin_amdgcn_sched_barrier(0);
-  }
-}
-
-__device__ __forceinline__ float row_max(float v) {
-  v = fmaxf(v, __shfl_xor(v, 16, 64));
-  return fmaxf(v, __shfl_xor(v, 32, 64));
-}
-__device__ __forceinline__ float row_sum(float v) {
-  v += __shfl_xor(v, 16, 64);
-  return v + __shfl_xor(v, 32, 64);
-}
-
-template <typename T> __device__ __forceinline__ float fast_exp(float x);
-template <> __device__ __forceinline__ float fast_exp<float>(float x) { return expf(x); }
-template <> __device__ __forceinline__ float fast_exp<bf16_t>(float x) { return __expf(x); }
 
 __device__ __forceinline__ f32x4 load4_guard(const float *p, int i, int n, bool vec) {
   if (vec) return (i < n) ? dm_load4(p + i) : (f32x4){0.f, 0.f, 0.f, 0.f};
@@ -143,40 +43,6 @@
   }
   return bv;
 }
-template <typename T>
-__device__ __forceinline__ f32x4 score_tile(const u32x4 (&fa)[AL<T>::KBD], const char *img, const f32x4 bv,
-                                            int N, int row, float scale, int lane, int kt) {
-  using L = AL<T>;
-  const int g = lane >> 4, li = lane & 15;
-  f32x4 a = {0.f, 0.f, 0.f, 0.f};
-#pragma unroll
-  for (int kb = 0; kb < L::KBD; ++kb) mma<T>(a, fa[kb], frag_row<T>(img, kt * 16 + li, kb, lane));
-  const int col = kt * 16 + 4 * g;
-#pragma unroll
-  for (int r = 0; r < 4; ++r) a[r] = (row < N && col + r < N) ? a[r] * scale + bv[r] : -INFINITY;
-  return a;
-}
-
-template <typename T> __device__ __forceinline__ u32x4 pack_tiles(const f32x4 (&tl)[AL<T>::TPB]) {
-  if constexpr (sizeof(T) == 2) {
-    bf16x8 r = {(bf16_t)tl[0][0], (bf16_t)tl[0][1], (bf16_t)tl[0][2], (bf16_t)tl[0][3],
-                (bf16_t)tl[1][0], (bf16_t)tl[1][1], (bf16_t)tl[1][2], (bf16_t)tl[1][3]};
-    return __builtin_bit_cast(u32x4, r);
-  } else {
-    return __builtin_bit_cast(u32x4, tl[0]);
-  }
-}
-
-template <typename T, int NB>
-__device__ __forceinline__ void contract_frags(f32x4 (&o)[4], const u32x4 (&f)[NB], const char *img, int lane) {
-#pragma unroll
-  for (int m = 0; m < NB; ++m) {
-#pragma unroll
-    for (int dt = 0; dt < 4; ++dt) mma<T>(o[dt], f[m], frag_tr<T>(img, dt * 16, m, lane));
-    if ((m & 1) == 1) __builtin_amdgcn_sched_barrier(0);
-  }
-}
-
 template <typename T, int NKT, bool FAST>
 __global__ __launch_bounds__(256, 2) void attn_fwd_kernel(const AttnParams p) {
   using L = AL<T>;
@@ -490,6 +356,7 @@
     if (const char *e = getenv("DM_ATTN_XCD")) v.xcd = atoi(e) != 0;
     if (const char *e = getenv("DM_ATTN_X3")) v.x3 = atoi(e) != 0;
     if (const char *e = getenv("DM_ATTN_X3_W8")) v.x3_w8 = atoi(e) != 0;
+    if (const char *e = getenv("DM_ATTN_SHORT")) v.short_attn = atoi(e) != 0;
     return v;
   }();
   return sw;
diff --git a/deepmerge_amd/csrc/dm_attention_plan.h b/deepmerge_amd/csrc/dm_attention_plan.h
--- a/deepmerge_amd/csrc/dm_attention_plan.h
+++ b/deepmerge_amd/csrc/dm_attention_plan.h
@@ -11,6 +11,7 @@
   bool xcd = true;
   bool x3 = true;
   bool x3_w8 = true;
+  bool short_attn = true;
 };
 const AttnSwitches &attn_switches();
 
@@ -30,6 +31,7 @@
   ATTN_Q32,
   ATTN_Q32_TABKV,
   ATTN_X3,
+  ATTN_SHORT,
 };
 enum AttnBias { ATTN_BIAS_NONE, ATTN_BIAS_DENSE, ATTN_BIAS_TABLE };
 enum AttnRefusal { ATTN_TAKEN = 0, ATTN_SHAPE_NOT_TAKEN, ATTN_TABLE_NEEDS_BF16, ATTN_TABLE_NOT_TAKEN };
@@ -56,6 +58,12 @@
 AttnFwdPlan attn_plan_fwd(const AttnCall &c, const AttnSwitches &sw);
 AttnBwdPlan attn_plan_bwd(const AttnCall &c, const AttnSwitches &sw);
 
+struct AttnShortPlan {
+  AttnRefusal refused;
+  AttnPass fwd, bwd;
+};
+AttnShortPlan attn_plan_short(const AttnCall &c, const AttnSwitches &sw);
+
 inline void attn_chunks(int B, int N, int H, int rows, int &nblk, int &chunks, int &bchunk) {
   nblk = (N + rows - 1) / rows;
   chunks = 256 / (H * nblk);
diff --git a/deepmerge_amd/csrc/dm_attention_short.hip b/deepmerge_amd/csrc/dm_attention_short.hip
--- /dev/null
+++ b/deepmerge_amd/csrc/dm_attention_short.hip
@@ -0,0 +1,423 @@
+#include "dm_common.h"
+#include "dm_mfma.h"
+#include "dm_attention_tile.h"
+#include "dm_attention_plan.h"
+#include "dm_prof.h"
+
+namespace {
+
+using T = bf16_t;
+constexpr int ROWB = AL<T>::RB;
+
+struct ShortParams {
+  const T *qkv;
+  const float *table;
+  const int *index;
+  const int *pos, *off;
+  T *out;
+  const T *dout;
+  float *lse;
+  T *dqkv;
+  float *partial;
+  int B, N, H, n_bins, bchunk;
+  float scale;
+};
+
+constexpr int TAB_MAX = 1024;
+
+template <int NT, int NROWS>
+__device__ __forceinline__ void rows_load(u32x4 (&r)[NROWS * 8 / NT], const T *g, long long ld, int nvalid, int t) {
+#pragma unroll
+  for (int i = 0; i < NROWS * 8 / NT; ++i) {
+    const int row = (t >> 3) + i * (NT / 8);
+    r[i] = (u32x4){0u, 0u, 0u, 0u};
+    if (row < nvalid) r[i] = *reinterpret_cast<const u32x4 *>(g + (long long)row * ld + (t & 7) * 8);
+  }
+}
+template <int NT, int NROWS>
+__device__ __forceinline__ void rows_store(char *lds, const u32x4 (&r)[NROWS * 8 / NT], int t) {
+#pragma unroll
+  for (int i = 0; i < NROWS * 8 / NT; ++i) *reinterpret_cast<u32x4 *>(lds + img_off<T>((t >> 3) + i * (NT / 8), t & 7)) = r[i];
+}
+
+template <int NKT>
+__device__ __forceinline__ void bias_bins(int (&bin)[NKT][4], const ShortParams &p, int q, int lane) {
+  const int g = lane >> 4;
+#pragma unroll
+  for (int kt = 0; kt < NKT; ++kt)
+#pragma unroll
+    for (int r = 0; r < 4; ++r) {
+      const int col = kt * 16 + 4 * g + r;
+      bin[kt][r] = -1;
+      if (p.table && q < p.N && col < p.N) bin[kt][r] = min(max(p.index[q * p.N + col], 0), p.n_bins - 1);
+    }
+}
+template <int NT>
+__device__ __forceinline__ void table_load(float (&tv)[TAB_MAX / NT], const ShortParams &p, int h, int t) {
+#pragma unroll
+  for (int i = 0; i < TAB_MAX / NT; ++i) {
+    const int b = t + i * NT;
+    tv[i] = (p.table && p.n_bins <= TAB_MAX && b < p.n_bins) ? p.table[(long long)b * p.H + h] : 0.f;
+  }
+}
+template <int NT>
+__device__ __forceinline__ void table_store(float *tabs, const float (&tv)[TAB_MAX / NT], int t) {
+#pragma unroll
+  for (int i = 0; i < TAB_MAX / NT; ++i) tabs[t + i * NT] = tv[i];
+}
+template <int NKT>
+__device__ __forceinline__ void bias_values(f32x4 (&bv)[NKT], const int (&bin)[NKT][4], const float *tabs, const ShortParams &p, int h) {
+  const bool in_lds = p.n_bins <= TAB_MAX;
+#pragma unroll
+  for (int kt = 0; kt < NKT; ++kt)
+#pragma unroll
+    for (int r = 0; r < 4; ++r) {
+      const int b = bin[kt][r];
+      bv[kt][r] = b < 0 ? 0.f : (in_lds ? tabs[b] : p.table[(long long)b * p.H + h]);
+    }
+}
+
+template <int NKT>
+__global__ __launch_bounds__(64 * NKT, 16 / NKT) void attn_short_fwd_kernel(const ShortParams p) {
+  constexpr int NT = 64 * NKT, NK = 16 * NKT, IMG = NK * ROWB;
+  __shared__ __attribute__((aligned(16))) char smem[2 * IMG];
+  __shared__ float tabs[TAB_MAX];
+  char *kimg = smem, *vimg = smem + IMG;
+  const int t = threadIdx.x, lane = t & 63, wave = t >> 6, g = lane >> 4, li = lane & 15;
+  const int h = blockIdx.x, chunk = blockIdx.y;
+  const int N = p.N, H = p.H;
+  const long long tok_stride = 3LL * H * HD;
+  const int q = wave * 16 + li;
+  const int b_first = chunk * p.bchunk, b_end = min(p.B, b_first + p.bchunk);
+  int bin[NKT][4];
+  float tv[TAB_MAX / NT];
+  f32x4 bv[NKT];
+  bias_bins<NKT>(bin, p, q, lane);
+  table_load<NT>(tv, p, h, t);
+
+  for (int b = b_first; b < b_end; ++b) {
+    const T *base = p.qkv + (long long)b * N * tok_stride + (long long)h * HD;
+    u32x4 rk[NK * 8 / NT], rv[NK * 8 / NT], fq[2];
+    if (b != b_first) __syncthreads();
+    rows_load<NT, NK>(rk, base + (long long)H * HD, tok_stride, N, t);
+    rows_load<NT, NK>(rv, base + 2LL * H * HD, tok_stride, N, t);
+#pragma unroll
+    for (int kb = 0; kb < 2; ++kb) fq[kb] = gl_frag<T>(base + (long long)q * tok_stride, q < N, kb, lane);
+    if (b == b_first) table_store<NT>(tabs, tv, t);
+    rows_store<NT, NK>(kimg, rk, t);
+    rows_store<NT, NK>(vimg, rv, t);
+    __syncthreads();
+    if (b == b_first) bias_values<NKT>(bv, bin, tabs, p, h);
+
+    f32x4 s[NKT];
+#pragma unroll
+    for (int kt = 0; kt < NKT; ++kt) s[kt] = score_tile<T>(fq, kimg, bv[kt], N, q, p.scale, lane, kt);
+    float m = -INFINITY;
+#pragma unroll
+    for (int kt = 0; kt < NKT; ++kt)
+#pragma unroll
+      for (int r = 0; r < 4; ++r) m = fmaxf(m, s[kt][r]);
+    m = row_max(m);
+    const float msafe = (m == -INFINITY) ? 0.f : m;
+    float l = 0.f;
+#pragma unroll
+    for (int kt = 0; kt < NKT; ++kt)
+#pragma unroll
+      for (int r = 0; r < 4; ++r) {
+        const float e = fast_exp<T>(s[kt][r] - msafe);
+        s[kt][r] = e;
+        l += e;
+      }
+    l = row_sum(l);
+    const float inv = (l > 0.f) ? 1.f / l : 0.f;
+    if (g == 0 && q < N) p.lse[((long long)b * H + h) * N + q] = msafe + logf(l);
+#pragma unroll
+    for (int kt = 0; kt < NKT; ++kt) s[kt] *= inv;
+
+    f32x4 o[4];
+#pragma unroll
+    for (int dt = 0; dt < 4; ++dt) o[dt] = (f32x4){0.f, 0.f, 0.f, 0.f};
+    contract_tokens<T, NKT>(o, s, vimg, lane);
+    if (q < N) {
+      T *orow = p.out + ((long long)b * N + q) * H * HD + (long long)h * HD;
+#pragma unroll
+      for (int dt = 0; dt < 4; ++dt) dm_store4(orow + dt * 16 + 4 * g, o[dt]);
+    }
+  }
+}
+
+template <int NKT>
+__global__ __launch_bounds__(64 * NKT) void attn_short_bwd_kernel(const ShortParams p) {
+  constexpr int NT = 64 * NKT, NK = 16 * NKT, IMG = NK * ROWB, NB = NKT / 2;
+  __shared__ __attribute__((aligned(16))) char smem[6 * IMG];
+  __shared__ float tabs[TAB_MAX];
+  char *kimg = smem, *vimg = smem + IMG, *qimg = smem + 2 * IMG, *doimg = smem + 3 * IMG, *pimg = smem + 4 * IMG, *dsimg = smem + 5 * IMG;
+  const int t = threadIdx.x, lane = t & 63, wave = t >> 6, g = lane >> 4, li = lane & 15;
+  const int h = blockIdx.x, chunk = blockIdx.y;
+  const int N = p.N, H = p.H;
+  const long long tok_stride = 3LL * H * HD, o_stride = (long long)H * HD;
+  const int q = wave * 16 + li;
+  const bool qok = q < N;
+  const int b_first = chunk * p.bchunk, b_end = min(p.B, b_first + p.bchunk);
+  int bin[NKT][4];
+  float tv[TAB_MAX / NT];
+  f32x4 bv[NKT], hacc[NKT];
+  bias_bins<NKT>(bin, p, q, lane);
+  table_load<NT>(tv, p, h, t);
+  int entries = 0, off0[2][2] = {{0, 0}, {0, 0}};
+  if (p.partial) {
+    entries = p.off[p.n_bins];
+#pragma unroll
+    for (int i = 0; i < 2; ++i)
+      if (t + i * NT < p.n_bins) { off0[i][0] = p.off[t + i * NT]; off0[i][1] = p.off[t + i * NT + 1]; }
+  }
+#pragma unroll
+  for (int kt = 0; kt < NKT; ++kt) hacc[kt] = (f32x4){0.f, 0.f, 0.f, 0.f};
+
+  for (int b = b_first; b < b_end; ++b) {
+    const T *base = p.qkv + (long long)b * N * tok_stride + (long long)h * HD;
+    const long long obase = (long long)b * N * o_stride + (long long)h * HD;
+    u32x4 rq[NK * 8 / NT], rk[NK * 8 / NT], rv[NK * 8 / NT], rdo[NK * 8 / NT];
+    if (b != b_first) __syncthreads();
+    rows_load<NT, NK>(rq, base, tok_stride, N, t);
+    rows_load<NT, NK>(rk, base + (long long)H * HD, tok_stride, N, t);
+    rows_load<NT, NK>(rv, base + 2LL * H * HD, tok_stride, N, t);
+    rows_load<NT, NK>(rdo, p.dout + obase, o_stride, N, t);
+    bf16x4 ov[4];
+#pragma unroll
+    for (int c = 0; c < 4; ++c) ov[c] = qok ? *reinterpret_cast<const bf16x4 *>(p.out + obase + (long long)q * o_stride + 16 * g + 4 * c) : (bf16x4){0, 0, 0, 0};
+    const float lse = qok ? p.lse[((long long)b * H + h) * N + q] : 0.f;
+    if (b == b_first) table_store<NT>(tabs, tv, t);
+    rows_store<NT, NK>(qimg, rq, t);
+    rows_store<NT, NK>(kimg, rk, t);
+    rows_store<NT, NK>(vimg, rv, t);
+    rows_store<NT, NK>(doimg, rdo, t);
+    __syncthreads();
+    if (b == b_first) bias_values<NKT>(bv, bin, tabs, p, h);
+
+    u32x4 fq[2], fdo[2];
+#pragma unroll
+    for (int kb = 0; kb < 2; ++kb) {
+      fq[kb] = frag_row<T>(qimg, q, kb, lane);
+      fdo[kb] = frag_row<T>(doimg, q, kb, lane);
+    }
+    float dl = 0.f;
+#pragma unroll
+    for (int c = 0; c < 4; ++c) {
+      const f32x4 d = dm_load4(reinterpret_cast<const T *>(doimg + img_off<T>(q, 2 * g + (c >> 1)) + (c & 1) * 8));
+      dl += ((float)ov[c][0] * d[0] + (float)ov[c][1] * d[1]) + ((float)ov[c][2] * d[2] + (float)ov[c][3] * d[3]);
+    }
+    dl = row_sum(dl);
+
+    u32x4 fds[NB];
+#pragma unroll
+    for (int m = 0; m < NB; ++m) {
+      f32x4 tp[2], td[2];
+#pragma unroll
+      for (int u = 0; u < 2; ++u) {
+        const int kt = 2 * m + u;
+        const f32x4 sc = score_tile<T>(fq, kimg, bv[kt], N, q, p.scale, lane, kt);
+        f32x4 a = {0.f, 0.f, 0.f, 0.f};
+#pragma unroll
+        for (int kb = 0; kb < 2; ++kb) mma<T>(a, fdo[kb], frag_row<T>(vimg, kt * 16 + li, kb, lane));
+#pragma unroll
+        for (int r = 0; r < 4; ++r) {
+          const float pv = fast_exp<T>(sc[r] - lse);
+          tp[u][r] = pv;
+          td[u][r] = pv * (a[r] - dl);
+        }
+        hacc[kt] += td[u];
+      }
+      const u32x4 fp = pack_tiles<T>(tp);
+      fds[m] = pack_tiles<T>(td);
+#pragma unroll
+      for (int u = 0; u < 2; ++u) {
+        const int o8 = img_off<T>(q, 2 * (2 * m + u) + (g >> 1)) + (g & 1) * 8;
+        *reinterpret_cast<u32x2 *>(pimg + o8) = (u32x2){fp[2 * u], fp[2 * u + 1]};
+        *reinterpret_cast<u32x2 *>(dsimg + o8) = (u32x2){fds[m][2 * u], fds[m][2 * u + 1]};
+      }
+    }
+    {
+      f32x4 o[4];
+#pragma unroll
+      for (int dt = 0; dt < 4; ++dt) o[dt] = (f32x4){0.f, 0.f, 0.f, 0.f};
+      contract_frags<T, NB>(o, fds, kimg, lane);
+      if (qok) {
+        T *dq = p.dqkv + ((long long)b * N + q) * tok_stride + (long long)h * HD;
+#pragma unroll
+        for (int dt = 0; dt < 4; ++dt) dm_store4(dq + dt * 16 + 4 * g, o[dt] * p.scale);
+      }
+    }
+    __syncthreads();
+
+    u32x4 fpt[NB], fdt[NB];
+#pragma unroll
+    for (int m = 0; m < NB; ++m) {
+      fpt[m] = frag_tr<T>(pimg, wave * 16, m, lane);
+      fdt[m] = frag_tr<T>(dsimg, wave * 16, m, lane);
+    }
+    T *dk = p.dqkv + ((long long)b * N + q) * tok_stride + (long long)(H + h) * HD;
+    f32x4 o[4];
+#pragma unroll
+    for (int dt = 0; dt < 4; ++dt) o[dt] = (f32x4){0.f, 0.f, 0.f, 0.f};
+    contract_frags<T, NB>(o, fpt, doimg, lane);
+    if (qok) {
+#pragma unroll
+      for (int dt = 0; dt < 4; ++dt) dm_store4(dk + o_stride + dt * 16 + 4 * g, o[dt]);
+    }
+#pragma unroll
+    for (int dt = 0; dt < 4; ++dt) o[dt] = (f32x4){0.f, 0.f, 0.f, 0.f};
+    contract_frags<T, NB>(o, fdt, qimg, lane);
+    if (qok) {
+#pragma unroll
+      for (int dt = 0; dt < 4; ++dt) dm_store4(dk + dt * 16 + 4 * g, o[dt] * p.scale);
+    }
+  }
+
+  if (p.partial == nullptr) return;
+  float *hs = reinterpret_cast<float *>(smem), *sorted = hs + NK * NK;
+  __syncthreads();
+  if (qok) {
+#pragma unroll
+    for (int kt = 0; kt < NKT; ++kt)
+#pragma unroll
+      for (int r = 0; r < 4; ++r) {
+        const int key = kt * 16 + 4 * g + r;
+        if (key < N) hs[q * N + key] = hacc[kt][r];
+      }
+  }
+  entries = min(max(entries, 0), N * N);
+  __syncthreads();
+  {
+    constexpr int PER = NK * NK / NT;
+    int at[PER];
+#pragma unroll
+    for (int i = 0; i < PER; ++i) at[i] = t + i * NT < entries ? p.pos[t + i * NT] : -1;
+#pragma unroll
+    for (int i = 0; i < PER; ++i)
+      if (t + i * NT < entries) sorted[t + i * NT] = (unsigned)at[i] < (unsigned)(N * N) ? hs[at[i]] : 0.f;
+  }
+  __syncthreads();
+  for (int bin0 = 0; bin0 < p.n_bins; bin0 += 2 * NT) {
+#pragma unroll
+    for (int i = 0; i < 2; ++i) {
+      const int b = bin0 + t + i * NT;
+      if (b >= p.n_bins) continue;
+      int beg = off0[i][0], end = off0[i][1];
+      if (bin0 != 0) { beg = p.off[b]; end = p.off[b + 1]; }
+      beg = min(max(beg, 0), entries);
+      end = min(max(end, beg), entries);
+      float acc = 0.f;
+#pragma unroll 4
+      for (int j = beg; j < end; ++j) acc += sorted[j];
+      p.partial[((long long)chunk * p.n_bins + b) * H + h] = acc;
+    }
+  }
+}
+
+__global__ void attn_short_table_kernel(const float *__restrict__ partial, float *__restrict__ dtable, int chunks, int elems, int accumulate) {
+  const int e = blockIdx.x * blockDim.x + threadIdx.x;
+  if (e >= elems) return;
+  float acc = 0.f;
+#pragma unroll 8
+  for (int c = 0; c < chunks; ++c) acc += partial[(long long)c * elems + e];
+  dtable[e] = accumulate ? dtable[e] + acc : acc;
+}
+
+bool short_shape(int B, int N, int H, int D, int dtype) {
+  return B > 0 && B <= 65535 && H > 0 && H <= 65535 && N >= 1 && N <= 64 && D == HD && dtype == DM_BF16;
+}
+
+}
+
+static AttnPass pass_short(const AttnCall &c, int per_cu) {
+  int chunks = 256 * per_cu / c.H;
+  chunks = chunks < 1 ? 1 : (chunks > c.B ? c.B : chunks);
+  const int bchunk = (c.B + chunks - 1) / chunks;
+  const int nkt = c.N <= 32 ? 2 : 4;
+  return AttnPass{ATTN_SHORT, nkt, c.N != 16 * nkt, c.table ? ATTN_BIAS_TABLE : ATTN_BIAS_NONE, nkt, 1, (c.B + bchunk - 1) / bchunk, bchunk};
+}
+
+AttnShortPlan attn_plan_short(const AttnCall &c, const AttnSwitches &sw) {
+  AttnShortPlan pl{};
+  if (!sw.short_attn || !short_shape(c.B, c.N, c.H, c.D, c.dtype) || c.dense || c.split) {
+    pl.refused = ATTN_SHAPE_NOT_TAKEN;
+    return pl;
+  }
+  pl.fwd = pass_short(c, 4);
+  pl.bwd = pass_short(c, 2);
+  return pl;
+}
+
+static AttnCall short_call(int32_t B, int32_t N, int32_t H, int32_t D, int32_t dtype, bool table) {
+  return AttnCall{B, N, H, D, dtype, false, table, 0, false, false};
+}
+
+extern "C" int32_t dm_attention_short_ok(int32_t B, int32_t N, int32_t H, int32_t D, int32_t dtype, int32_t has_table) {
+  return attn_plan_short(short_call(B, N, H, D, dtype, has_table != 0), attn_switches()).refused ? 0 : 1;
+}
+
+extern "C" int64_t dm_attention_short_partial_floats(int32_t B, int32_t N, int32_t H, int32_t n_bins) {
+  const AttnShortPlan pl = attn_plan_short(short_call(B, N, H, HD, DM_BF16, true), attn_switches());
+  return pl.refused || n_bins <= 0 ? 0 : (int64_t)pl.bwd.chunks * n_bins * H;
+}
+
+extern "C" int dm_attention_short_fwd(const void *qkv, const float *table, const int32_t *index32, int32_t n_bins, void *out, float *lse,
+                                      int32_t B, int32_t N, int32_t H, int32_t D, float scale, int32_t dtype, void *stream) {
+  const AttnShortPlan pl = attn_plan_short(short_call(B, N, H, D, dtype, table != nullptr), attn_switches());
+  DM_REQUIRE(!pl.refused, DM_ERR_UNSUPPORTED, "dm_attention_short_fwd: shape not taken (B=%d N=%d H=%d D=%d dtype=%d; bf16, D = 64, N <= 64, DM_ATTN_SHORT); call dm_attention_fwd",
+             B, N, H, D, dtype);
+  DM_REQUIRE(qkv && out && lse, DM_ERR_BAD_SHAPE, "dm_attention_short_fwd: null pointer");
+  DM_REQUIRE(!table || (index32 && n_bins > 0), DM_ERR_BAD_SHAPE, "dm_attention_short_fwd: a table needs its index and n_bins > 0");
+  DM_REQUIRE(dm_aligned16(qkv) && dm_aligned(out, 8) && dm_aligned(lse, 4) && dm_aligned(table, 4) && dm_aligned(index32, 4), DM_ERR_BAD_ALIGN,
+             "dm_attention_short_fwd: qkv must be 16-byte aligned, out 8-byte");
+  hipStream_t s = reinterpret_cast<hipStream_t>(stream);
+  {
+    DmProfScope prof("attn_fwd_bf16", s, 4.0 * B * H * (double)N * N * HD, 2.0 * 4.0 * B * H * (double)N * HD);
+    ShortParams p{};
+    p.qkv = reinterpret_cast<const T *>(qkv); p.table = table; p.index = index32; p.out = reinterpret_cast<T *>(out); p.lse = lse;
+    p.B = B; p.N = N; p.H = H; p.n_bins = n_bins; p.bchunk = pl.fwd.bchunk; p.scale = scale;
+    const dim3 grid(H, pl.fwd.chunks);
+    if (pl.fwd.nkt == 2) hipLaunchKernelGGL(attn_short_fwd_kernel<2>, grid, dim3(128), 0, s, p);
+    else hipLaunchKernelGGL(attn_short_fwd_kernel<4>, grid, dim3(256), 0, s, p);
+  }
+  DM_LAUNCH_CHECK("dm_attention_short_fwd");
+  return DM_OK;
+}
+
+extern "C" int dm_attention_short_bwd(const void *qkv, const float *table, const int32_t *index32, const int32_t *positions, const int32_t *offsets,
+                                      int32_t n_bins, const void *out, const void *dout, const float *lse, void *dqkv, float *dtable,
+                                      int32_t accumulate, float *partial, int64_t partial_floats, int32_t B, int32_t N, int32_t H, int32_t D,
+                                      float scale, int32_t dtype, void *stream) {
+  const AttnShortPlan pl = attn_plan_short(short_call(B, N, H, D, dtype, table != nullptr), attn_switches());
+  DM_REQUIRE(!pl.refused, DM_ERR_UNSUPPORTED, "dm_attention_short_bwd: shape not taken (B=%d N=%d H=%d D=%d dtype=%d; bf16, D = 64, N <= 64, DM_ATTN_SHORT); call dm_attention_bwd",
+             B, N, H, D, dtype);
+  DM_REQUIRE(qkv && out && dout && lse && dqkv, DM_ERR_BAD_SHAPE, "dm_attention_short_bwd: null pointer");
+  DM_REQUIRE(!table || (index32 && n_bins > 0), DM_ERR_BAD_SHAPE, "dm_attention_short_bwd: a table needs its index and n_bins > 0");
+  DM_REQUIRE(!dtable || (table && positions && offsets && partial), DM_ERR_BAD_SHAPE,
+             "dm_attention_short_bwd: the table gradient needs the table, the index CSR and the partial workspace");
+  DM_REQUIRE(!dtable || partial_floats >= (int64_t)pl.bwd.chunks * n_bins * H, DM_ERR_BAD_SHAPE,
+             "dm_attention_short_bwd: partial workspace of %lld floats, need %lld (dm_attention_short_partial_floats)", (long long)partial_floats,
+             (long long)pl.bwd.chunks * n_bins * H);
+  DM_REQUIRE(dm_aligned16(qkv) && dm_aligned16(dout) && dm_aligned(out, 8) && dm_aligned(dqkv, 8) && dm_aligned(lse, 4) && dm_aligned(table, 4) &&
+             dm_aligned(index32, 4) && dm_aligned(positions, 4) && dm_aligned(offsets, 4) && dm_aligned(dtable, 4) && dm_aligned(partial, 4),
+             DM_ERR_BAD_ALIGN, "dm_attention_short_bwd: qkv / dout must be 16-byte aligned, out / dqkv 8-byte");
+  hipStream_t s = reinterpret_cast<hipStream_t>(stream);
+  {
+    DmProfScope prof("attn_bwd_bf16", s, 10.0 * B * H * (double)N * N * HD, 2.0 * 8.0 * B * H * (double)N * HD);
+    ShortParams p{};
+    p.qkv = reinterpret_cast<const T *>(qkv); p.table = table; p.index = index32; p.pos = positions; p.off = offsets;
+    p.out = reinterpret_cast<T *>(const_cast<void *>(out)); p.dout = reinterpret_cast<const T *>(dout); p.lse = const_cast<float *>(lse);
+    p.dqkv = reinterpret_cast<T *>(dqkv); p.partial = dtable ? partial : nullptr;
+    p.B = B; p.N = N; p.H = H; p.n_bins = n_bins; p.bchunk = pl.bwd.bchunk; p.scale = scale;
+    const dim3 grid(H, pl.bwd.chunks);
+    if (pl.bwd.nkt == 2) hipLaunchKernelGGL(attn_short_bwd_kernel<2>, grid, dim3(128), 0, s, p);
+    else hipLaunchKernelGGL(attn_short_bwd_kernel<4>, grid, dim3(256), 0, s, p);
+    if (dtable) {
+      const int elems = n_bins * H;
+      hipLaunchKernelGGL(attn_short_table_kernel, dim3((elems + 255) / 256), dim3(256), 0, s, partial, dtable, pl.bwd.chunks, elems, accumulate);
+    }
+  }
+  DM_LAUNCH_CHECK("dm_attention_short_bwd");
+  return DM_OK;
+}
diff --git a/deepmerge_amd/csrc/dm_attention_tile.h b/deepmerge_amd/csrc/dm_attention_tile.h
--- /dev/null
+++ b/deepmerge_amd/csrc/dm_attention_tile.h
@@ -0,0 +1,142 @@
+#pragma once
+#include "dm_common.h"
+#include "dm_mfma.h"
+
+namespace {
+
+constexpr int HD = 64;
+constexpr int QB = 64;
+
+template <typename T> struct AL {
+  static constexpr int RB = HD * (int)sizeof(T);
+  static constexpr int CPRW = RB / 16;
+  static constexpr int KBD = RB / 64;
+  static constexpr int EPC = 16 / (int)sizeof(T);
+  static constexpr int TPB = (sizeof(T) == 2) ? 2 : 1;
+};
+
+template <typename T> __device__ __forceinline__ int swz(int row);
+template <> __device__ __forceinline__ int swz<bf16_t>(int row) {
+  const int t0 = (row >> 1) & 1, t1 = (row >> 2) & 1, t2 = (row >> 3) & 1;
+  return ((t1 ^ t2) << 2) | (t0 << 1) | t1;
+}
+template <> __device__ __forceinline__ int swz<float>(int row) { return row & 15; }
+
+template <typename T> __device__ __forceinline__ int img_off(int row, int chunk) {
+  return row * AL<T>::RB + ((chunk ^ swz<T>(row)) << 4);
+}
+
+template <typename T>
+__device__ __forceinline__ void tile_to_lds(char *lds, const T *g, long long ld, int nvalid, int nrows, int t) {
+  using L = AL<T>;
+  const int c = t % L::CPRW;
+  constexpr int RPI = 256 / L::CPRW;
+  for (int row = t / L::CPRW; row < nrows; row += RPI) {
+    u32x4 v = {0u, 0u, 0u, 0u};
+    if (row < nvalid) v = *reinterpret_cast<const u32x4 *>(g + (long long)row * ld + c * L::EPC);
+    *reinterpret_cast<u32x4 *>(lds + img_off<T>(row, c)) = v;
+  }
+}
+
+template <typename T> __device__ __forceinline__ u32x4 frag_row(const char *lds, int row, int kb, int lane) {
+  return *reinterpret_cast<const u32x4 *>(lds + img_off<T>(row, kb * 4 + (lane >> 4)));
+}
+template <typename T> __device__ __forceinline__ u32x4 frag_tr(const char *lds, int d0, int m, int lane);
+template <> __device__ __forceinline__ u32x4 frag_tr<bf16_t>(const char *lds, int d0, int m, int lane) {
+  const int g = lane >> 4, q = (lane >> 2) & 3, p = lane & 3;
+  const int d = d0 + 4 * p;
+  u32x4 out;
+#pragma unroll
+  for (int half = 0; half < 2; ++half) {
+    const int k = 32 * m + 4 * g + 16 * half + q;
+    const u32x2 w = dm_ds_read_tr16(lds + img_off<bf16_t>(k, d >> 3) + ((d & 7) << 1));
+    out[2 * half] = w[0];
+    out[2 * half + 1] = w[1];
+  }
+  return out;
+}
+template <> __device__ __forceinline__ u32x4 frag_tr<float>(const char *lds, int d0, int m, int lane) {
+  const int g = lane >> 4, d = d0 + (lane & 15);
+  u32x4 out;
+#pragma unroll
+  for (int j = 0; j < 4; ++j) {
+    const int k = 16 * m + 4 * g + j;
+    out[j] = *reinterpret_cast<const unsigned int *>(lds + img_off<float>(k, d >> 2) + ((d & 3) << 2));
+  }
+  return out;
+}
+template <typename T> __device__ __forceinline__ u32x4 gl_frag(const T *rowp, bool valid, int kb, int lane) {
+  u32x4 v = {0u, 0u, 0u, 0u};
+  if (valid) v = *reinterpret_cast<const u32x4 *>(rowp + (kb * 4 + (lane >> 4)) * AL<T>::EPC);
+  return v;
+}
+
+template <typename T, int NKT> __device__ __forceinline__ u32x4 acc_frag(const f32x4 (&s)[NKT], int m) {
+  if constexpr (sizeof(T) == 2) {
+    const f32x4 lo = s[2 * m], hi = s[2 * m + 1];
+    bf16x8 r = {(bf16_t)lo[0], (bf16_t)lo[1], (bf16_t)lo[2], (bf16_t)lo[3], (bf16_t)hi[0], (bf16_t)hi[1], (bf16_t)hi[2], (bf16_t)hi[3]};
+    return __builtin_bit_cast(u32x4, r);
+  } else {
+    return __builtin_bit_cast(u32x4, s[m]);
+  }
+}
+
+template <typename T, int NKT>
+__device__ __forceinline__ void contract_tokens(f32x4 (&o)[4], const f32x4 (&s)[NKT], const char *img, int lane) {
+#pragma unroll
+  for (int m = 0; m < NKT / AL<T>::TPB; ++m) {
+    const u32x4 fp = acc_frag<T, NKT>(s, m);
+#pragma unroll
+    for (int dt = 0; dt < 4; ++dt) mma<T>(o[dt], fp, frag_tr<T>(img, dt * 16, m, lane));
+    if ((m & 1) == 1) __builtin_amdgcn_sched_barrier(0);
+  }
+}
+
+__device__ __forceinline__ float row_max(float v) {
+  v = fmaxf(v, __shfl_xor(v, 16, 64));
+  return fmaxf(v, __shfl_xor(v, 32, 64));
+}
+__device__ __forceinline__ float row_sum(float v) {
+  v += __shfl_xor(v, 16, 64);
+  return v + __shfl_xor(v, 32, 64);
+}
+
+template <typename T> __device__ __forceinline__ float fast_exp(float x);
+template <> __device__ __forceinline__ float fast_exp<float>(float x) { return expf(x); }
+template <> __device__ __forceinline__ float fast_exp<bf16_t>(float x) { return __expf(x); }
+
+template <typename T> __device__ __forceinline__ u32x4 pack_tiles(const f32x4 (&tl)[AL<T>::TPB]) {
+  if constexpr (sizeof(T) == 2) {
+    bf16x8 r = {(bf16_t)tl[0][0], (bf16_t)tl[0][1], (bf16_t)tl[0][2], (bf16_t)tl[0][3],
+                (bf16_t)tl[1][0], (bf16_t)tl[1][1], (bf16_t)tl[1][2], (bf16_t)tl[1][3]};
+    return __builtin_bit_cast(u32x4, r);
+  } else {
+    return __builtin_bit_cast(u32x4, tl[0]);
+  }
+}
+
+template <typename T, int NB>
+__device__ __forceinline__ void contract_frags(f32x4 (&o)[4], const u32x4 (&f)[NB], const char *img, int lane) {
+#pragma unroll
+  for (int m = 0; m < NB; ++m) {
+#pragma unroll
+    for (int dt = 0; dt < 4; ++dt) mma<T>(o[dt], f[m], frag_tr<T>(img, dt * 16, m, lane));
+    if ((m & 1) == 1) __builtin_amdgcn_sched_barrier(0);
+  }
+}
+
+template <typename T>
+__device__ __forceinline__ f32x4 score_tile(const u32x4 (&fa)[AL<T>::KBD], const char *img, const f32x4 bv,
+                                            int N, int row, float scale, int lane, int kt) {
+  using L = AL<T>;
+  const int g = lane >> 4, li = lane & 15;
+  f32x4 a = {0.f, 0.f, 0.f, 0.f};
+#pragma unroll
+  for (int kb = 0; kb < L::KBD; ++kb) mma<T>(a, fa[kb], frag_row<T>(img, kt * 16 + li, kb, lane));
+  const int col = kt * 16 + 4 * g;
+#pragma unroll
+  for (int r = 0; r < 4; ++r) a[r] = (row < N && col + r < N) ? a[r] * scale + bv[r] : -INFINITY;
+  return a;
+}
+
+}
diff --git a/deepmerge_amd/ops.py b/deepmerge_amd/ops.py
--- a/deepmerge_amd/ops.py
+++ b/deepmerge_amd/ops.py
@@ -610,6 +610,48 @@
     return dtable
 
 
+def attention_short_ok(B: int, N: int, H: int, D: int, dtype: torch.dtype, has_table: bool = True) -> bool:
+    return bool(_lib.lib().dm_attention_short_ok(B, N, H, D, DM_BF16 if dtype == torch.bfloat16 else DM_F32, int(has_table)))
+
+
+def attention_fwd_short(qkv: torch.Tensor, table: Optional[torch.Tensor], index32: Optional[torch.Tensor], B: int, N: int, H: int, D: int, scale: float):
+    _need_cuda(qkv, table, index32)
+    n_bins = _short_table(table, index32, N, H, "attention_fwd_short")
+    out = torch.empty((B, N, H * D), dtype=qkv.dtype, device=qkv.device)
+    lse = torch.empty((B, H, N), dtype=torch.float32, device=qkv.device)
+    check(_lib.lib().dm_attention_short_fwd(qkv.data_ptr(), _ptr(table), _ptr(index32) if table is not None else None, n_bins, out.data_ptr(),
+                                            lse.data_ptr(), B, N, H, D, scale, _dt(qkv), _stream()), "dm_attention_short_fwd")
+    return out, lse
+
+
+def attention_bwd_short(qkv, table, index32, out, dout, lse, B, N, H, D, scale, dtable=None, accumulate=False):
+    _need_cuda(qkv, table, index32, out, dout, lse, dtable)
+    n_bins = _short_table(table, index32, N, H, "attention_bwd_short")
+    dqkv = torch.empty_like(qkv)
+    pos = off = part = None
+    floats = 0
+    if dtable is not None:
+        if table is None or dtable.dtype != torch.float32 or not dtable.is_contiguous() or dtable.numel() != n_bins * H:
+            raise ValueError("attention_bwd_short: dtable must be contiguous fp32 [n_bins, H] and needs the table")
+        pos, off = relpos_index_csr(index32, n_bins)
+        floats = int(_lib.lib().dm_attention_short_partial_floats(B, N, H, n_bins))
+        part = torch.empty((max(floats, 1),), dtype=torch.float32, device=qkv.device)
+    check(_lib.lib().dm_attention_short_bwd(qkv.data_ptr(), _ptr(table), _ptr(index32) if table is not None else None, _ptr(pos), _ptr(off), n_bins,
+                                            out.data_ptr(), dout.data_ptr(), lse.data_ptr(), dqkv.data_ptr(), _ptr(dtable), int(accumulate),
+                                            _ptr(part), floats, B, N, H, D, scale, _dt(qkv), _stream()), "dm_attention_short_bwd")
+    return dqkv
+
+
+def _short_table(table, index32, N, H, who) -> int:
+    if table is None:
+        return 0
+    if table.dtype != torch.float32 or not table.is_contiguous() or table.dim() != 2 or table.shape[1] != H:
+        raise ValueError(f"{who}: table must be contiguous fp32 [n_bins, H], got {tuple(table.shape)} {table.dtype}")
+    if index32 is None or index32.dtype != torch.int32 or not index32.is_contiguous() or index32.numel() != N * N:
+        raise ValueError(f"{who}: index32 must be a contiguous int32 [N, N] tensor")
+    return int(table.shape[0])
+
+
 def patchify(x: torch.Tensor, patch: int, dtype: torch.dtype) -> torch.Tensor:
     _need_cuda(x)
     B, Cc, H, W = x.shape
@@ -1059,11 +1101,14 @@
             return out
         elif cube is not None:
             out, lse = attention_fwd_relpos(qkv, table.contiguous(), cube, B, N, H, D, scale)
+        elif qkv.dtype == torch.bfloat16 and attention_short_ok(B, N, H, D, qkv.dtype, table is not None):
+            ctx.short = True
+            out, lse = attention_fwd_short(qkv, None if table is None else table.contiguous(), index32, B, N, H, D, scale)
         else:
             if table is not None:
                 bias, bias_t = relpos_bias_gather(table.contiguous(), index32, N, transposed=True)
             out, lse = attention_fwd(qkv, bias, B, N, H, D, scale)
-        ctx.save_for_backward(qkv, out, lse, bias, bias_t, index32, table if cube is not None else None)
+        ctx.save_for_backward(qkv, out, lse, bias, bias_t, index32, table if (cube is not None or getattr(ctx, "short", False)) else None)
         ctx.dims = (B, N, H, D, scale, None if table is None else table.shape[0])
         return out
 
@@ -1081,6 +1126,14 @@
                 relpos_bias_scatter(slab, dtable, B, H, rows, n_bins)
             return dqkv, dtable, None, None, None, None, None, None
         qkv, out, lse, bias, bias_t, index32, table = ctx.saved_tensors
+        if getattr(ctx, "short", False):
+            dtable = None
+            if table is not None:
+                table = table.detach().contiguous()
+                if ctx.needs_input_grad[1]:
+                    dtable = torch.empty((n_bins, H), dtype=torch.float32, device=qkv.device)
+            dqkv = attention_bwd_short(qkv, table, index32, out, _as_operand(dout, qkv.dtype), lse, B, N, H, D, scale, dtable=dtable)
+            return dqkv, dtable, None, None, None, None, None, None
         cube = None
         if table is not None:
             table, cube = table.contiguous(), index32._dm_cube
@@ -1416,6 +1469,7 @@
         gemm(DM_NT, y1, wq, qkv, M, 3 * Cc, Cc, lda=Cc, ldb=Cc, ldc=3 * Cc, bias=qkv_b)
         bias = bias_t = None
         cube = _inkernel_cube(table, index32, B, N, heads, D, dtype)
+        short = not split and cube is None and dtype == torch.bfloat16 and attention_short_ok(B, N, heads, D, dtype, table is not None)
         split_imgs = None
         if split:
             o_op = None
@@ -1426,6 +1480,8 @@
             split_imgs = (hi, lo, scube)
         elif cube is not None:
             o, lse = attention_fwd_relpos(qkv, table.contiguous(), cube, B, N, heads, D, scale)
+        elif short:
+            o, lse = attention_fwd_short(qkv, None if table is None else table.contiguous(), index32, B, N, heads, D, scale)
         else:
             if table is not None:
                 bias, bias_t = relpos_bias_gather(table.contiguous(), index32, N, transposed=True)
@@ -1453,6 +1509,7 @@
                               wq, wp, w1, w2, n1w, n2w, o_op if planes else None)
         ctx.dims = (B, N, Cc, heads, D, Hd, scale, None if table is None else table.shape[0])
         ctx.table_in_kernel = cube is not None
+        ctx.short = short
         ctx.split_imgs = split_imgs
         ctx.params = (n1w, n1b, table, qkv_w, qkv_b, proj_w, proj_b, n2w, n2b, fc1_w, fc1_b, fc2_w, fc2_b)
         return x2.view(B, N, Cc)
@@ -1532,6 +1589,7 @@
         do = torch.empty((M, Cc), dtype=dtype, device=dev)
         gemm(DM_NN, dx1_op, wp, do, M, Cc, Cc, lda=Cc, ldb=Cc, ldc=Cc)
         tab, cube = None, None
+        dtable, k_t = None, False
         if ctx.split_imgs is not None:
             hi, lo, scube = ctx.split_imgs
             ctx.split_imgs = None
@@ -1539,14 +1597,21 @@
             dqkv, slab, rows = attention_bwd_split(hi, lo, None if P_table is None else P_table.detach().contiguous(), scube, o.view(B, N, Cc),
                                                    do.view(B, N, Cc), lse, B, N, heads, D, scale, index32 if want_table else None, n_bins or 0,
                                                    pair=planes)
+        elif ctx.short:
+            want_table = P_table is not None
+            if want_table:
+                tab = P_table.detach().contiguous()
+                dtable, k_t = _grad_out(P_table, (n_bins, heads), dev)
+            dqkv = attention_bwd_short(qkv, tab, index32, o, do, lse, B, N, heads, D, scale, dtable=dtable,
+                                       accumulate=want_table and _acc(P_table, k_t))
+            slab = None
         else:
             if ctx.table_in_kernel:
                 tab, cube = P_table.detach().contiguous(), index32._dm_cube
             want_table = bias is not None or tab is not None
             dqkv, slab, rows = attention_bwd(qkv, bias, o, do, lse, B, N, heads, D, scale,
                                              index32 if want_table else None, n_bins or 0, bias_t=bias_t, table=tab, cube=cube)
-        dtable, k_t = None, False
-        if want_table:
+        if want_table and slab is not None:
             dtable, k_t = _grad_out(P_table, (n_bins, heads), dev)
             relpos_bias_scatter(slab, dtable, B, heads, rows, n_bins, accumulate=_acc(P_table, k_t))
         dqkv2 = dqkv if isinstance(dqkv, Planes) else dqkv.view(M, 3 * Cc)
diff --git a/include/deepmerge_hip.h b/include/deepmerge_hip.h
--- a/include/deepmerge_hip.h
+++ b/include/deepmerge_hip.h
@@ -89,6 +89,15 @@
                                 int32_t H, int32_t D, float scale, void *stream);
 int32_t dm_attention_bwd_batch_chunks(int32_t B, int32_t N, int32_t H, int32_t dtype);
 
+int32_t dm_attention_short_ok(int32_t B, int32_t N, int32_t H, int32_t D, int32_t dtype, int32_t has_table);
+int64_t dm_attention_short_partial_floats(int32_t B, int32_t N, int32_t H, int32_t n_bins);
+int dm_attention_short_fwd(const void *qkv, const float *table, const int32_t *index32, int32_t n_bins, void *out, float *lse,
+                           int32_t B, int32_t N, int32_t H, int32_t D, float scale, int32_t dtype, void *stream);
+int dm_attention_short_bwd(const void *qkv, const float *table, const int32_t *index32, const int32_t *positions, const int32_t *offsets,
+                           int32_t n_bins, const void *out, const void *dout, const float *lse, void *dqkv, float *dtable,
+                           int32_t accumulate, float *partial, int64_t partial_floats, int32_t B, int32_t N, int32_t H, int32_t D,
+                           float scale, int32_t dtype, void *stream);
+
 int dm_relpos_bias_gather(const float *table, const int32_t *index, float *bias, float *bias_t,
                           int32_t N, int32_t H, int32_t n_bins, void *stream);
 int dm_relpos_bias_reduce(float *dbias_slab, const int32_t *positions, const int32_t *offsets, float *dtable,
```

Measured after the change: 6399 pairs/s (median of 6 runs). Within noise of the previous version (+0.5%).
